# maciejkula/spotlight

Hardware: NVIDIA B200
Metric: interactions/sec (BPR MF, 1Mx100Kx64) (higher is better)
Workload: dtype f32

## Files before the change

### include/spotlight_b200.h

```cpp
#ifndef SPOTLIGHT_B200_H
#define SPOTLIGHT_B200_H

#include <stddef.h>
#include <stdint.h>

#ifdef __cplusplus
extern "C" {
#endif

#define SLB_VERSION 100

#define SLB_OK 0
#define SLB_EINVAL (-1)
#define SLB_ECUDA (-2)
#define SLB_ENOSPC (-3)

#define SLB_LOSS_POINTWISE 0
#define SLB_LOSS_BPR 1
#define SLB_LOSS_HINGE 2
#define SLB_LOSS_ADAPTIVE_HINGE 3

#define SLB_GRAD_DENSE 0
#define SLB_GRAD_COMPACT 1

#define SLB_OPT_NONE 0
#define SLB_OPT_SGD 1
#define SLB_OPT_ADAGRAD 2
#define SLB_OPT_ADAM 3

typedef void* slb_stream_t;

int slb_version(void);
const char* slb_last_error(void);
int slb_sm_count(void);


int slb_mt19937_fill(uint32_t* blocks, int64_t nblocks, slb_stream_t stream);

int slb_mt19937_fill_parallel(uint32_t* blocks, int64_t nblocks, const uint32_t* jump_table,
                              int32_t table_rows, uint32_t* states, slb_stream_t stream);

int64_t slb_mt19937_direct_slots(int64_t nblocks, int32_t j0_log2);
int slb_mt19937_fill_direct(uint32_t* blocks, int64_t nblocks, const uint32_t* jump_table,
                            int32_t table_rows, const uint32_t* direct_table, int32_t direct_rows,
                            int32_t j0_log2, uint32_t* states, int64_t state_slots, slb_stream_t stream);

size_t slb_sample_workspace_bytes(int64_t nwords);

int slb_sample_bounded(const uint32_t* blocks, int64_t nwords, int64_t* cursor,
                       uint32_t rng, int64_t count, int64_t* out,
                       void* workspace, size_t workspace_bytes, slb_stream_t stream);

int slb_sample_bounded_chain(uint32_t* blocks, int64_t nwords, int64_t* cursor,
                             uint32_t rng, int64_t count, int64_t* out,
                             void* workspace, size_t workspace_bytes, slb_stream_t stream);

int slb_host_shuffle_order(uint32_t* key, int32_t* pos, int64_t n, int32_t elem_bytes,
                           void* order_out);

size_t slb_shuffle_workspace_bytes(int64_t n, int64_t nwords);
int slb_shuffle_order(const uint32_t* blocks, int64_t nwords, int64_t* cursor, int64_t first_word,
                      int64_t n, int32_t rounds, int32_t resume, int64_t* order,
                      void* workspace, size_t workspace_bytes, slb_stream_t stream);

int slb_permute_ids(const int64_t* order, int64_t n, const void* users, const void* items,
                    int32_t elem_bytes, int64_t* users_out, int64_t* items_out, slb_stream_t stream);


int slb_embedding_forward(const float* W, int64_t rows, int32_t dim,
                          const int64_t* ids, int64_t n,
                          int32_t hash_count, const uint32_t* seeds ,
                          int64_t padding_idx, float* out, slb_stream_t stream);

int slb_bloom_rows(const int64_t* ids, int64_t n, int32_t hash_count,
                   const uint32_t* seeds , int64_t rows, int64_t padding_idx,
                   int64_t* rows_out, slb_stream_t stream);

size_t slb_embedding_backward_workspace_bytes(int64_t n_terms, int64_t rows);

int slb_embedding_backward(const float* dout, const int64_t* ids, int64_t n,
                           int32_t hash_count, const uint32_t* seeds ,
                           int64_t rows, int32_t dim, int64_t frozen_row,
                           float* dW, void* workspace, size_t workspace_bytes,
                           slb_stream_t stream);

int slb_workspace_init(void* workspace, size_t workspace_bytes, slb_stream_t stream);

int slb_mf_scores(const float* Wu, const float* Wi, const float* bu, const float* bi,
                  int32_t dim, const int64_t* users, const int64_t* items, int64_t n,
                  int32_t user_broadcast, float* scores, slb_stream_t stream);

int slb_mf_scores_backward(const float* gscores, const int64_t* users, const int64_t* items,
                           int64_t n, int32_t user_broadcast, const float* Wu, const float* Wi,
                           int64_t num_users, int64_t num_items, int32_t dim,
                           float* dWu, float* dWi, float* dbu, float* dbi,
                           void* workspace, size_t workspace_bytes, slb_stream_t stream);

int slb_rank_pairs(const float* scores, int64_t n_rows, int64_t n_items, const int64_t* pair_row,
                   const int64_t* pair_item, int64_t n_pairs, float* ranks, slb_stream_t stream);

typedef struct slb_mf_step_args {
    int64_t batch;
    const int64_t* users;
    const int64_t* items;
    const int64_t* negs;
    int32_t loss;
    int32_t n_neg;
    int64_t num_users, num_items;
    int32_t dim;
    float* Wu; float* Wi;
    float* bu; float* bi;
    float* loss_out;
    float* pos_out;
    float* neg_out;
    int32_t grad_mode;
    float* dWu; float* dWi; float* dbu; float* dbi;
    int64_t* urows; float* gWu; float* gbu;
    int64_t* irows; float* gWi; float* gbi;
    int32_t* compact_counts;
    int32_t opt;
    float lr;
    float weight_decay;
    float eps;
    float* state_Wu; float* state_Wi; float* state_bu; float* state_bi;
    int64_t norm_batch;
    int32_t opt_users_only;
    void* workspace; size_t workspace_bytes;
    void* fused_workspace; size_t fused_workspace_bytes;
    slb_stream_t plan_stream;
    float beta1, beta2;
    float one_minus_beta1, one_minus_beta2;
    float* state2_Wu; float* state2_Wi; float* state2_bu; float* state2_bi;
    int32_t* last_u; int32_t* last_i;
    const float* adam_sched;
    int64_t adam_step;
} slb_mf_step_args;

size_t slb_mf_step_workspace_bytes(int64_t batch, int32_t n_neg, int32_t loss,
                                   int64_t num_users, int64_t num_items);
size_t slb_mf_fused_workspace_bytes(int64_t batch, int64_t num_users, int64_t num_items, int32_t dim);
int64_t slb_mf_compact_rows(int64_t batch, int32_t n_neg, int32_t loss, int32_t which );

int slb_mf_train_step(const slb_mf_step_args* args, slb_stream_t stream);

int slb_mf_train_step_phases(const slb_mf_step_args* args, int32_t phases, slb_stream_t stream);

typedef struct slb_mf_bloom_args {
    slb_mf_step_args base;
    int64_t user_rows, item_rows;
    int32_t user_hashes, item_hashes;
    uint32_t user_seeds[24], item_seeds[24];
    int64_t user_padding_idx, item_padding_idx;
    int64_t* pair_ids_u; float* pair_g_u;
    int64_t* pair_ids_i; float* pair_g_i;
} slb_mf_bloom_args;

size_t slb_mf_bloom_workspace_bytes(const slb_mf_bloom_args* args);

size_t slb_bias_sparse_workspace_bytes(int64_t n);
int slb_bias_sparse_apply(const int64_t* ids, const float* g, int64_t n, float* bias, float* state,
                          int32_t opt, float lr, float weight_decay, float eps,
                          void* workspace, size_t workspace_bytes, slb_stream_t stream);
int slb_mf_bloom_train_step(const slb_mf_bloom_args* args, slb_stream_t stream);

int slb_mf_fit_epoch(const slb_mf_step_args* step, const int64_t* users, const int64_t* items,
                     const int64_t* negs, int64_t n, float* losses_out, slb_stream_t stream);

int slb_mf_fit_epoch_events(const slb_mf_step_args* step, const int64_t* users, const int64_t* items,
                            const int64_t* negs, int64_t n, float* losses_out, slb_stream_t stream,
                            const int64_t* wait_steps, void* const* wait_events, int32_t n_waits);

int slb_adam_flush(float* W, float* exp_avg, float* exp_avg_sq, float* bias, float* bias_avg, float* bias_avg_sq,
                   int32_t* last, int64_t rows, int32_t dim, const float* sched, int64_t step,
                   float beta1, float beta2, float one_minus_beta1, float one_minus_beta2, float eps,
                   float weight_decay, slb_stream_t stream);

size_t slb_unique_workspace_bytes(int64_t n, int64_t rows);
int slb_unique_bucket(const int64_t* ids, int64_t n, int64_t rows, int64_t chunk, int32_t nparts,
                      int64_t* uniq , int64_t* inverse ,
                      int64_t* counts_out, void* workspace, size_t workspace_bytes,
                      slb_stream_t stream);

int slb_shard_gather_batch(const int64_t* pos, int64_t m, const int64_t* users, const int64_t* items,
                           const int64_t* negs, int64_t neg_base, int32_t n_neg, int64_t user_lo,
                           int64_t* users_out, int64_t* items_out, int64_t* negs_out, slb_stream_t stream);

int slb_adagrad_dense(float* W, float* state, const float* grad, int64_t n, float lr, float eps,
                      slb_stream_t stream);

size_t slb_loss_workspace_bytes(int64_t n);
int slb_pairwise_loss(int32_t loss, const float* pos, const float* neg, const uint8_t* mask,
                      int64_t n, int32_t n_neg, float* loss_out, float* gpos, float* gneg,
                      void* workspace, size_t workspace_bytes, slb_stream_t stream);

typedef struct slb_seq_step_args {
    int64_t batch;
    int32_t seq_len;
    const int64_t* seqs;
    const int64_t* negs;
    int32_t loss; int32_t n_neg;
    int64_t num_items; int32_t dim;
    float* E; float* bias;
    int32_t n_layers;
    const int32_t* kernel_width; const int32_t* dilation;
    int32_t nonlinearity;
    int32_t residual;
    float* const* conv_w;
    float* const* conv_b;
    float* const* dconv_w;
    float* const* dconv_b;
    float* loss_out; float* pos_out; float* neg_out;
    float* dE; float* dbias;
    const int32_t* norm_count;
    void* workspace; size_t workspace_bytes;
    int32_t opt; float lr; float weight_decay; float eps;
    float* state_E; float* state_bias;
} slb_seq_step_args;

size_t slb_seq_step_workspace_bytes(const slb_seq_step_args* args);
int slb_seq_train_step(const slb_seq_step_args* args, slb_stream_t stream);

int slb_seq_representation(const slb_seq_step_args* args, float* rep_out, slb_stream_t stream);

#ifdef __cplusplus
}
#endif
#endif
```

### spotlight_b200/_lib.py

```python

import ctypes
import os

_HERE = os.path.dirname(os.path.abspath(__file__))
LIB_PATH = os.environ.get('SLB_LIBRARY') or os.path.join(_HERE, 'libspotlight_b200.so')

c_i32, c_i64, c_f32 = ctypes.c_int32, ctypes.c_int64, ctypes.c_float
c_vp, c_sz = ctypes.c_void_p, ctypes.c_size_t

LOSS_KIND = {'pointwise': 0, 'bpr': 1, 'hinge': 2, 'adaptive_hinge': 3}
GRAD_DENSE, GRAD_COMPACT = 0, 1
OPT_NONE, OPT_SGD, OPT_ADAGRAD, OPT_ADAM = 0, 1, 2, 3

EXPORTS = (
    'slb_version', 'slb_last_error', 'slb_sm_count', 'slb_workspace_init',
    'slb_mt19937_fill', 'slb_mt19937_fill_parallel', 'slb_mt19937_direct_slots',
    'slb_mt19937_fill_direct', 'slb_host_shuffle_order',
    'slb_sample_workspace_bytes', 'slb_sample_bounded', 'slb_sample_bounded_chain',
    'slb_shuffle_workspace_bytes', 'slb_shuffle_order', 'slb_permute_ids',
    'slb_embedding_forward', 'slb_bloom_rows',
    'slb_embedding_backward_workspace_bytes', 'slb_embedding_backward',
    'slb_mf_scores', 'slb_mf_scores_backward', 'slb_rank_pairs', 'slb_mf_step_workspace_bytes', 'slb_mf_fused_workspace_bytes', 'slb_mf_compact_rows',
    'slb_mf_train_step', 'slb_mf_train_step_phases', 'slb_mf_fit_epoch', 'slb_mf_fit_epoch_events', 'slb_adam_flush',
    'slb_mf_bloom_workspace_bytes', 'slb_mf_bloom_train_step',
    'slb_bias_sparse_workspace_bytes', 'slb_bias_sparse_apply',
    'slb_unique_workspace_bytes', 'slb_unique_bucket', 'slb_shard_gather_batch', 'slb_adagrad_dense',
    'slb_loss_workspace_bytes', 'slb_pairwise_loss',
    'slb_seq_step_workspace_bytes', 'slb_seq_train_step', 'slb_seq_representation',
)


class MfStepArgs(ctypes.Structure):
    _fields_ = [
        ('batch', c_i64), ('users', c_vp), ('items', c_vp), ('negs', c_vp),
        ('loss', c_i32), ('n_neg', c_i32),
        ('num_users', c_i64), ('num_items', c_i64), ('dim', c_i32),
        ('Wu', c_vp), ('Wi', c_vp), ('bu', c_vp), ('bi', c_vp),
        ('loss_out', c_vp), ('pos_out', c_vp), ('neg_out', c_vp),
        ('grad_mode', c_i32),
        ('dWu', c_vp), ('dWi', c_vp), ('dbu', c_vp), ('dbi', c_vp),
        ('urows', c_vp), ('gWu', c_vp), ('gbu', c_vp),
        ('irows', c_vp), ('gWi', c_vp), ('gbi', c_vp),
        ('compact_counts', c_vp),
        ('opt', c_i32), ('lr', c_f32), ('weight_decay', c_f32), ('eps', c_f32),
        ('state_Wu', c_vp), ('state_Wi', c_vp), ('state_bu', c_vp), ('state_bi', c_vp),
        ('norm_batch', c_i64), ('opt_users_only', c_i32),
        ('workspace', c_vp), ('workspace_bytes', c_sz),
        ('fused_workspace', c_vp), ('fused_workspace_bytes', c_sz), ('plan_stream', c_vp),
        ('beta1', c_f32), ('beta2', c_f32), ('one_minus_beta1', c_f32), ('one_minus_beta2', c_f32),
        ('state2_Wu', c_vp), ('state2_Wi', c_vp), ('state2_bu', c_vp), ('state2_bi', c_vp),
        ('last_u', c_vp), ('last_i', c_vp), ('adam_sched', c_vp), ('adam_step', c_i64),
    ]


class MfBloomArgs(ctypes.Structure):
    _fields_ = [
        ('base', MfStepArgs),
        ('user_rows', c_i64), ('item_rows', c_i64),
        ('user_hashes', c_i32), ('item_hashes', c_i32),
        ('user_seeds', ctypes.c_uint32 * 24), ('item_seeds', ctypes.c_uint32 * 24),
        ('user_padding_idx', c_i64), ('item_padding_idx', c_i64),
        ('pair_ids_u', c_vp), ('pair_g_u', c_vp), ('pair_ids_i', c_vp), ('pair_g_i', c_vp),
    ]


class SeqStepArgs(ctypes.Structure):
    _fields_ = [
        ('batch', c_i64), ('seq_len', c_i32), ('seqs', c_vp), ('negs', c_vp),
        ('loss', c_i32), ('n_neg', c_i32),
        ('num_items', c_i64), ('dim', c_i32),
        ('E', c_vp), ('bias', c_vp),
        ('n_layers', c_i32), ('kernel_width', c_vp), ('dilation', c_vp),
        ('nonlinearity', c_i32), ('residual', c_i32),
        ('conv_w', c_vp), ('conv_b', c_vp), ('dconv_w', c_vp), ('dconv_b', c_vp),
        ('loss_out', c_vp), ('pos_out', c_vp), ('neg_out', c_vp),
        ('dE', c_vp), ('dbias', c_vp),
        ('norm_count', c_vp),
        ('workspace', c_vp), ('workspace_bytes', c_sz),
        ('opt', c_i32), ('lr', c_f32), ('weight_decay', c_f32), ('eps', c_f32),
        ('state_E', c_vp), ('state_bias', c_vp),
    ]


_lib = None


class LibraryError(RuntimeError):
    pass


def _declare(lib):
    P = ctypes.POINTER
    lib.slb_version.restype = c_i32
    lib.slb_last_error.restype = ctypes.c_char_p
    lib.slb_sm_count.restype = c_i32
    lib.slb_workspace_init.argtypes = [c_vp, c_sz, c_vp]
    lib.slb_mt19937_fill.argtypes = [c_vp, c_i64, c_vp]
    lib.slb_mt19937_fill_parallel.argtypes = [c_vp, c_i64, c_vp, c_i32, c_vp, c_vp]
    lib.slb_mt19937_direct_slots.argtypes = [c_i64, c_i32]
    lib.slb_mt19937_direct_slots.restype = c_i64
    lib.slb_mt19937_fill_direct.argtypes = [c_vp, c_i64, c_vp, c_i32, c_vp, c_i32, c_i32, c_vp, c_i64, c_vp]
    lib.slb_sample_bounded_chain.argtypes = [c_vp, c_i64, c_vp, ctypes.c_uint32, c_i64, c_vp, c_vp, c_sz, c_vp]
    lib.slb_host_shuffle_order.argtypes = [c_vp, c_vp, c_i64, c_i32, c_vp]
    lib.slb_shuffle_workspace_bytes.argtypes = [c_i64, c_i64]
    lib.slb_shuffle_workspace_bytes.restype = c_sz
    lib.slb_shuffle_order.argtypes = [c_vp, c_i64, c_vp, c_i64, c_i64, c_i32, c_i32, c_vp, c_vp, c_sz, c_vp]
    lib.slb_permute_ids.argtypes = [c_vp, c_i64, c_vp, c_vp, c_i32, c_vp, c_vp, c_vp]
    lib.slb_sample_workspace_bytes.argtypes = [c_i64]
    lib.slb_sample_workspace_bytes.restype = c_sz
    lib.slb_sample_bounded.argtypes = [c_vp, c_i64, c_vp, ctypes.c_uint32, c_i64, c_vp, c_vp, c_sz, c_vp]
    lib.slb_embedding_forward.argtypes = [c_vp, c_i64, c_i32, c_vp, c_i64, c_i32, c_vp, c_i64, c_vp, c_vp]
    lib.slb_bloom_rows.argtypes = [c_vp, c_i64, c_i32, c_vp, c_i64, c_i64, c_vp, c_vp]
    lib.slb_embedding_backward_workspace_bytes.argtypes = [c_i64, c_i64]
    lib.slb_embedding_backward_workspace_bytes.restype = c_sz
    lib.slb_embedding_backward.argtypes = [c_vp, c_vp, c_i64, c_i32, c_vp, c_i64, c_i32, c_i64,
                                           c_vp, c_vp, c_sz, c_vp]
    lib.slb_mf_scores.argtypes = [c_vp, c_vp, c_vp, c_vp, c_i32, c_vp, c_vp, c_i64, c_i32, c_vp, c_vp]
    lib.slb_mf_scores_backward.argtypes = [c_vp, c_vp, c_vp, c_i64, c_i32, c_vp, c_vp, c_i64, c_i64, c_i32,
                                           c_vp, c_vp, c_vp, c_vp, c_vp, c_sz, c_vp]
    lib.slb_rank_pairs.argtypes = [c_vp, c_i64, c_i64, c_vp, c_vp, c_i64, c_vp, c_vp]
    lib.slb_mf_step_workspace_bytes.argtypes = [c_i64, c_i32, c_i32, c_i64, c_i64]
    lib.slb_mf_step_workspace_bytes.restype = c_sz
    lib.slb_mf_fused_workspace_bytes.argtypes = [c_i64, c_i64, c_i64, c_i32]
    lib.slb_mf_fused_workspace_bytes.restype = c_sz
    lib.slb_mf_compact_rows.argtypes = [c_i64, c_i32, c_i32, c_i32]
    lib.slb_mf_compact_rows.restype = c_i64
    lib.slb_mf_train_step.argtypes = [P(MfStepArgs), c_vp]
    lib.slb_mf_train_step_phases.argtypes = [P(MfStepArgs), c_i32, c_vp]
    lib.slb_mf_bloom_workspace_bytes.argtypes = [P(MfBloomArgs)]
    lib.slb_mf_bloom_workspace_bytes.restype = c_sz
    lib.slb_mf_bloom_train_step.argtypes = [P(MfBloomArgs), c_vp]
    lib.slb_bias_sparse_workspace_bytes.argtypes = [c_i64]
    lib.slb_bias_sparse_workspace_bytes.restype = c_sz
    lib.slb_bias_sparse_apply.argtypes = [c_vp, c_vp, c_i64, c_vp, c_vp, c_i32, c_f32, c_f32, c_f32, c_vp, c_sz, c_vp]
    lib.slb_mf_fit_epoch.argtypes = [P(MfStepArgs), c_vp, c_vp, c_vp, c_i64, c_vp, c_vp]
    lib.slb_mf_fit_epoch_events.argtypes = [P(MfStepArgs), c_vp, c_vp, c_vp, c_i64, c_vp, c_vp, c_vp, c_vp, c_i32]
    lib.slb_adam_flush.argtypes = [c_vp, c_vp, c_vp, c_vp, c_vp, c_vp, c_vp, c_i64, c_i32, c_vp, c_i64,
                                   c_f32, c_f32, c_f32, c_f32, c_f32, c_f32, c_vp]
    lib.slb_unique_workspace_bytes.argtypes = [c_i64, c_i64]
    lib.slb_unique_workspace_bytes.restype = c_sz
    lib.slb_unique_bucket.argtypes = [c_vp, c_i64, c_i64, c_i64, c_i32, c_vp, c_vp, c_vp, c_vp, c_sz, c_vp]
    lib.slb_shard_gather_batch.argtypes = [c_vp, c_i64, c_vp, c_vp, c_vp, c_i64, c_i32, c_i64, c_vp, c_vp, c_vp, c_vp]
    lib.slb_adagrad_dense.argtypes = [c_vp, c_vp, c_vp, c_i64, c_f32, c_f32, c_vp]
    lib.slb_loss_workspace_bytes.argtypes = [c_i64]
    lib.slb_loss_workspace_bytes.restype = c_sz
    lib.slb_pairwise_loss.argtypes = [c_i32, c_vp, c_vp, c_vp, c_i64, c_i32, c_vp, c_vp, c_vp,
                                      c_vp, c_sz, c_vp]
    lib.slb_seq_step_workspace_bytes.argtypes = [P(SeqStepArgs)]
    lib.slb_seq_step_workspace_bytes.restype = c_sz
    lib.slb_seq_train_step.argtypes = [P(SeqStepArgs), c_vp]
    lib.slb_seq_representation.argtypes = [P(SeqStepArgs), c_vp, c_vp]
    for name in EXPORTS:
        fn = getattr(lib, name)
        if fn.restype is ctypes.c_int:
            fn.restype = c_i32


def load():
    global _lib
    if _lib is None:
        if not os.path.exists(LIB_PATH):
            raise LibraryError(
                'spotlight_b200: %s not found. Build it with '
                '`python -c "import __graft_entry__ as g; g.build()"` (needs nvcc, sm_100a). '
                'There is no CPU fallback.' % LIB_PATH)
        lib = ctypes.CDLL(LIB_PATH)
        missing = [n for n in EXPORTS if not hasattr(lib, n)]
        if missing:
            raise LibraryError('spotlight_b200: library lacks symbols %s' % missing)
        _declare(lib)
        if lib.slb_version() != 100:
            raise LibraryError('spotlight_b200: ABI version mismatch')
        _lib = lib
    return _lib


def check(rc, what=''):
    if rc != 0:
        msg = load().slb_last_error().decode('utf-8', 'replace')
        if rc == -1:
            raise ValueError('%s: %s' % (what or 'spotlight_b200', msg))
        raise LibraryError('%s failed (%d): %s' % (what or 'spotlight_b200', rc, msg))
```

### spotlight_b200/csrc/common.cuh

```cuda
#pragma once

#include <cuda_runtime.h>
#include <stdint.h>
#include <stdio.h>

#include "../../include/spotlight_b200.h"

void slb_set_error(const char* fmt, ...);
int slb_sms();

#define SLB_REQUIRE(cond, ...)                 \
    do {                                       \
        if (!(cond)) {                         \
            slb_set_error(__VA_ARGS__);        \
            return SLB_EINVAL;                 \
        }                                      \
    } while (0)

#define SLB_LAUNCH_CHECK(name)                                                   \
    do {                                                                         \
        cudaError_t e__ = cudaGetLastError();                                    \
        if (e__ != cudaSuccess) {                                                \
            slb_set_error("%s: launch failed: %s", name, cudaGetErrorString(e__)); \
            return SLB_ECUDA;                                                    \
        }                                                                        \
    } while (0)

static inline size_t slb_align_up(size_t x, size_t a) { return (x + a - 1) / a * a; }

struct WsCarver {
    char* base;
    size_t off;
    explicit WsCarver(void* p) : base(static_cast<char*>(p)), off(0) {}
    template <typename T>
    T* take(size_t count) {
        off = slb_align_up(off, 256);
        T* p = base ? reinterpret_cast<T*>(base + off) : nullptr;
        off += count * sizeof(T);
        return p;
    }
    size_t bytes() const { return slb_align_up(off, 256); }
};

#ifdef __CUDACC__

__device__ __forceinline__ float4 ldg4(const float* p) {
    return __ldg(reinterpret_cast<const float4*>(p));
}
__device__ __forceinline__ float4 ld4(const float* p) {
    return *reinterpret_cast<const float4*>(p);
}
__device__ __forceinline__ void st4(float* p, float4 v) { *reinterpret_cast<float4*>(p) = v; }

__device__ __forceinline__ float dot4(float4 a, float4 b) {
    return a.x * b.x + a.y * b.y + a.z * b.z + a.w * b.w;
}
__device__ __forceinline__ void fma4(float4& acc, float g, float4 v) {
    acc.x = fmaf(g, v.x, acc.x);
    acc.y = fmaf(g, v.y, acc.y);
    acc.z = fmaf(g, v.z, acc.z);
    acc.w = fmaf(g, v.w, acc.w);
}

template <int LPR>
__device__ __forceinline__ float group_sum(float v, unsigned mask) {
#pragma unroll
    for (int o = LPR / 2; o > 0; o >>= 1) v += __shfl_xor_sync(mask, v, o);
    return v;
}

__device__ __forceinline__ unsigned group_mask(int lpr) {
    const int lane = threadIdx.x & 31;
    const unsigned m = lpr == 32 ? 0xffffffffu : ((1u << lpr) - 1u);
    return m << (lane & ~(lpr - 1));
}

__device__ __forceinline__ float sigmoidf_(float x) { return 1.0f / (1.0f + expf(-x)); }

template <int THREADS>
__device__ __forceinline__ float block_sum(float v, float* smem ) {
#pragma unroll
    for (int o = 16; o > 0; o >>= 1) v += __shfl_down_sync(0xffffffffu, v, o);
    const int w = threadIdx.x >> 5, l = threadIdx.x & 31;
    if (l == 0) smem[w] = v;
    __syncthreads();
    if (w == 0) {
        v = l < THREADS / 32 ? smem[l] : 0.f;
#pragma unroll
        for (int o = 16; o > 0; o >>= 1) v += __shfl_down_sync(0xffffffffu, v, o);
    }
    return v;
}

__device__ __forceinline__ uint32_t murmur3_32(uint32_t k, uint32_t seed) {
    k *= 0xcc9e2d51u;
    k = (k << 15) | (k >> 17);
    k *= 0x1b873593u;
    uint32_t h = seed ^ k;
    h = (h << 13) | (h >> 19);
    h = h * 5u + 0xe6546b64u;
    h ^= 4u;
    h ^= h >> 16;
    h *= 0x85ebca6bu;
    h ^= h >> 13;
    h *= 0xc2b2ae35u;
    h ^= h >> 16;
    return h;
}

__device__ __forceinline__ int64_t bloom_row(int64_t id, uint32_t seed, int64_t rows,
                                             int64_t padding_idx) {
    if (id == padding_idx) return 0;
    const int64_t h = static_cast<int32_t>(murmur3_32(static_cast<uint32_t>(id), seed));
    int64_t m = h % rows;
    if (m < 0) m += rows;
    return m;
}

__device__ __forceinline__ float adagrad_delta(float lr, float g, float s, float eps) {
    const float root = s > 0.f ? s * rsqrtf(s) : 0.f;
    return __fdividef(lr * g, root + eps);
}

struct OptV2 { int32_t opt; float lr, wd, eps; };

__device__ __forceinline__ void row_update(const OptV2& o, float4& w, float4& s, const float4& g0) {
    float gv[4] = {g0.x + o.wd * w.x, g0.y + o.wd * w.y, g0.z + o.wd * w.z, g0.w + o.wd * w.w};
    float wv[4] = {w.x, w.y, w.z, w.w};
    if (o.opt == SLB_OPT_SGD) {
#pragma unroll
        for (int q = 0; q < 4; ++q) wv[q] -= o.lr * gv[q];
    } else {
        float sv[4] = {s.x, s.y, s.z, s.w};
#pragma unroll
        for (int q = 0; q < 4; ++q) {
            sv[q] += gv[q] * gv[q];
            wv[q] -= adagrad_delta(o.lr, gv[q], sv[q], o.eps);
        }
        s = make_float4(sv[0], sv[1], sv[2], sv[3]);
    }
    w = make_float4(wv[0], wv[1], wv[2], wv[3]);
}

__device__ __forceinline__ void bias_update(const OptV2& o, float* bw, float* bs, float g) {
    const float gb = g + o.wd * *bw;
    if (o.opt == SLB_OPT_SGD) {
        *bw -= o.lr * gb;
    } else {
        const float sv = *bs + gb * gb;
        *bs = sv;
        *bw -= adagrad_delta(o.lr, gb, sv, o.eps);
    }
}

#endif
```

### spotlight_b200/csrc/mf.cu

```cuda
#include <stdlib.h>

#include "segindex.cuh"

namespace {

constexpr int MF_THREADS = 256;

struct MfDev {
    int64_t B;
    int64_t NB;
    int64_t T;
    const int64_t* users; const int64_t* items; const int64_t* negs;
    int32_t loss; int32_t n_neg;
    int64_t U, I; int32_t D;
    float* Wu; float* Wi; float* bu; float* bi;
    float* loss_out; float* pos_out; float* neg_out;
    int32_t* t_a; int32_t* t_b; float* t_g;
    float* partial; int32_t* done;
    int32_t* err;
    SegIndex seg;
    int32_t grad_mode;
    float* dWu; float* dWi; float* dbu; float* dbi;
    int64_t* urows; float* gWu; float* gbu;
    int64_t* irows; float* gWi; float* gbi;
    int32_t* compact_counts;
    int32_t opt; float lr, wd, eps;
    float* sWu; float* sWi; float* sbu; float* sbi;
    int32_t no_bias;
    int64_t frozen_a, frozen_b;
};

template <int LPR>
__device__ __forceinline__ float row_dot(const float* __restrict__ a, const float* __restrict__ b,
                                         int D, int gl, unsigned gmask) {
    float acc = 0.f;
    for (int c = gl * 4; c < D; c += LPR * 4) acc += dot4(ldg4(a + c), ldg4(b + c));
    return group_sum<LPR>(acc, gmask);
}

__device__ __forceinline__ void pair_loss(int loss, float p, float n, float& per, float& gp, float& gn) {
    if (loss == SLB_LOSS_BPR) {
        const float s = sigmoidf_(p - n);
        per = 1.0f - s;
        gp = -s * (1.0f - s);
        gn = -gp;
    } else if (loss == SLB_LOSS_POINTWISE) {
        const float sp = sigmoidf_(p), sn = sigmoidf_(n);
        per = (1.0f - sp) + sn;
        gp = -sp * (1.0f - sp);
        gn = sn * (1.0f - sn);
    } else {
        const float z = n - p + 1.0f;
        per = fmaxf(z, 0.0f);
        const float act = z >= 0.0f ? 1.0f : 0.0f;
        gp = -act;
        gn = act;
    }
}

template <int LPR>
__global__ void __launch_bounds__(MF_THREADS) mf_fwd_kernel(MfDev a) {
    __shared__ float sh_red[MF_THREADS / 32];
    const int gl = threadIdx.x & (LPR - 1);
    const unsigned gmask = group_mask(LPR);
    constexpr int GROUPS = MF_THREADS / LPR;
    const int64_t gid = static_cast<int64_t>(blockIdx.x) * GROUPS + threadIdx.x / LPR;
    const int64_t gstride = static_cast<int64_t>(gridDim.x) * GROUPS;
    const float invB = 1.0f / static_cast<float>(a.NB);
    const int D = a.D;
    float lsum = 0.f;
    if (blockIdx.x == 0 && threadIdx.x == 0) a.seg.totals[3] = 0;

    const int64_t iters = (a.B + gstride - 1) / gstride;
    for (int64_t it = 0; it < iters; ++it) {
        const int64_t b = gid + it * gstride;
        const bool valid = b < a.B;
        const int64_t bb = valid ? b : 0;
        const int64_t u = a.users[bb], i = a.items[bb];
        bool bad = u < 0 || u >= a.U || i < 0 || i >= a.I;
        const int64_t uc = bad ? 0 : u, ic = bad ? 0 : i;
        const float* urow = a.Wu + uc * D;
        float p, n;
        int64_t nu, nj;
        if (a.loss != SLB_LOSS_ADAPTIVE_HINGE) {
            int64_t j = a.negs[bb];
            if (j < 0 || j >= a.I) { bad = true; j = 0; }
            const float* qi = a.Wi + ic * D;
            const float* qj = a.Wi + j * D;
            float dp = 0.f, dn = 0.f;
            for (int c = gl * 4; c < D; c += LPR * 4) {
                const float4 u4 = ldg4(urow + c), i4 = ldg4(qi + c), j4 = ldg4(qj + c);
                dp += dot4(u4, i4);
                dn += dot4(u4, j4);
            }
            const float ub = __ldg(a.bu + uc);
            p = group_sum<LPR>(dp, gmask) + ub + __ldg(a.bi + ic);
            n = group_sum<LPR>(dn, gmask) + ub + __ldg(a.bi + j);
            nu = uc; nj = j;
            if (valid && gl == 0 && a.neg_out) a.neg_out[bb] = n;
        } else {
            p = row_dot<LPR>(urow, a.Wi + ic * D, D, gl, gmask) + __ldg(a.bu + uc) + __ldg(a.bi + ic);
            n = -INFINITY; nu = 0; nj = 0;
            for (int k = 0; k < a.n_neg; ++k) {
                const int64_t f = static_cast<int64_t>(k) * a.B + bb;
                int64_t u2 = a.users[f / a.n_neg], j = a.negs[f];
                if (u2 < 0 || u2 >= a.U || j < 0 || j >= a.I) { bad = true; u2 = 0; j = 0; }
                const float nk = row_dot<LPR>(a.Wu + u2 * D, a.Wi + j * D, D, gl, gmask) +
                                 __ldg(a.bu + u2) + __ldg(a.bi + j);
                if (valid && gl == 0 && a.neg_out) a.neg_out[f] = nk;
                if (nk > n || k == 0) { n = nk; nu = u2; nj = j; }
            }
        }
        if (valid && gl == 0) {
            if (bad) atomicExch(a.err, 1);
            float per, gp, gn;
            pair_loss(a.loss, p, n, per, gp, gn);
            lsum += per;
            gp *= invB; gn *= invB;
            if (bad) { gp = 0.f; gn = 0.f; }
            if (a.pos_out) a.pos_out[bb] = p;
            const int32_t t = static_cast<int32_t>(2 * bb);
            a.t_a[t] = static_cast<int32_t>(uc); a.t_b[t] = static_cast<int32_t>(ic); a.t_g[t] = gp;
            a.t_a[t + 1] = static_cast<int32_t>(nu); a.t_b[t + 1] = static_cast<int32_t>(nj); a.t_g[t + 1] = gn;
            if (gp != 0.f) { atomicAdd(a.seg.cnt + uc, 1); atomicAdd(a.seg.cnt + a.U + ic, 1); }
            if (gn != 0.f) { atomicAdd(a.seg.cnt + nu, 1); atomicAdd(a.seg.cnt + a.U + nj, 1); }
        }
    }

    const float bsum = block_sum<MF_THREADS>(lsum, sh_red);
    __shared__ bool is_last;
    if (threadIdx.x == 0) {
        a.partial[blockIdx.x] = bsum;
        __threadfence();
        is_last = atomicAdd(a.done, 1) == static_cast<int>(gridDim.x) - 1;
    }
    __syncthreads();
    if (is_last && threadIdx.x < 32) {
        __threadfence();
        float v = 0.f;
        for (int k = threadIdx.x; k < static_cast<int>(gridDim.x); k += 32)
            v += *reinterpret_cast<volatile float*>(a.partial + k);
#pragma unroll
        for (int o = 16; o > 0; o >>= 1) v += __shfl_down_sync(0xffffffffu, v, o);
        if (threadIdx.x == 0) { *a.loss_out = v * invB; *a.done = 0; }
    }
}

constexpr int MF_TILE_THREADS = 128;

template <int LPR, int LOSS, int TI, bool EX>
__global__ void __launch_bounds__(MF_TILE_THREADS) mf_fwd_tile_kernel(MfDev a) {
    __shared__ float sh_red[MF_TILE_THREADS / 32];
    __shared__ bool is_last;
    constexpr int GPW = 32 / LPR;
    constexpr int ITERS = TI / GPW > 0 ? TI / GPW : 1;
    const int lane = threadIdx.x & 31;
    const int gl = lane & (LPR - 1);
    const int grp = lane / LPR;
    const int D = EX ? LPR * 4 : a.D;
    const float invB = 1.0f / static_cast<float>(a.NB);
    const int64_t ntiles = (a.B + TI - 1) / TI;
    const int64_t wstride = static_cast<int64_t>(gridDim.x) * (MF_TILE_THREADS / 32);
    float lsum = 0.f;
    if (blockIdx.x == 0 && threadIdx.x == 0) a.seg.totals[3] = 0;

    for (int64_t tile = static_cast<int64_t>(blockIdx.x) * (MF_TILE_THREADS / 32) + (threadIdx.x >> 5);
         tile < ntiles; tile += wstride) {
        const int64_t b = tile * TI + lane;
        const bool valid = lane < TI && b < a.B;
        int64_t u64 = 0, i64 = 0, j64 = 0;
        if (valid) { u64 = a.users[b]; i64 = a.items[b]; j64 = a.negs[b]; }
        const bool bad = u64 < 0 || u64 >= a.U || i64 < 0 || i64 >= a.I || j64 < 0 || j64 >= a.I;
        if (bad) { u64 = 0; i64 = 0; j64 = 0; }
        const int u = static_cast<int>(u64), i = static_cast<int>(i64), j = static_cast<int>(j64);
        const float ub = __ldg(a.bu + u), ib = __ldg(a.bi + i), jb = __ldg(a.bi + j);
        float dpm = 0.f, dnm = 0.f;
#pragma unroll 4
        for (int s = 0; s < ITERS; ++s) {
            const int src = (s * GPW + grp) % TI;
            const int uu = __shfl_sync(0xffffffffu, u, src);
            const int ii = __shfl_sync(0xffffffffu, i, src);
            const int jj = __shfl_sync(0xffffffffu, j, src);
            const float* ur = a.Wu + static_cast<int64_t>(uu) * D;
            const float* qi = a.Wi + static_cast<int64_t>(ii) * D;
            const float* qj = a.Wi + static_cast<int64_t>(jj) * D;
            float dp = 0.f, dn = 0.f;
            for (int c = gl * 4; c < D; c += LPR * 4) {
                const float4 u4 = ldg4(ur + c), i4 = ldg4(qi + c), j4 = ldg4(qj + c);
                dp += dot4(u4, i4);
                dn += dot4(u4, j4);
            }
            dp = group_sum<LPR>(dp, 0xffffffffu);
            dn = group_sum<LPR>(dn, 0xffffffffu);
            const float tp = __shfl_sync(0xffffffffu, dp, (lane % GPW) * LPR);
            const float tn = __shfl_sync(0xffffffffu, dn, (lane % GPW) * LPR);
            if (lane / GPW == s) { dpm = tp; dnm = tn; }
        }
        if (valid) {
            const float p = dpm + ub + ib, n = dnm + ub + jb;
            float per, gp, gn;
            pair_loss(LOSS, p, n, per, gp, gn);
            lsum += per;
            gp *= invB; gn *= invB;
            if (bad) { atomicExch(a.err, 1); gp = 0.f; gn = 0.f; }
            if (a.pos_out) a.pos_out[b] = p;
            if (a.neg_out) a.neg_out[b] = n;
            *reinterpret_cast<int2*>(a.t_a + 2 * b) = make_int2(u, u);
            *reinterpret_cast<int2*>(a.t_b + 2 * b) = make_int2(i, j);
            *reinterpret_cast<float2*>(a.t_g + 2 * b) = make_float2(gp, gn);
            const int nu = (gp != 0.f) + (gn != 0.f);
            if (nu) atomicAdd(a.seg.cnt + u, nu);
            if (gp != 0.f) atomicAdd(a.seg.cnt + a.U + i, 1);
            if (gn != 0.f) atomicAdd(a.seg.cnt + a.U + j, 1);
        }
    }
    const float bsum = block_sum<MF_TILE_THREADS>(lsum, sh_red);
    if (threadIdx.x == 0) {
        a.partial[blockIdx.x] = bsum;
        __threadfence();
        is_last = atomicAdd(a.done, 1) == static_cast<int>(gridDim.x) - 1;
    }
    __syncthreads();
    if (is_last && threadIdx.x < 32) {
        __threadfence();
        float v = 0.f;
        for (int k = threadIdx.x; k < static_cast<int>(gridDim.x); k += 32)
            v += *reinterpret_cast<volatile float*>(a.partial + k);
#pragma unroll
        for (int o = 16; o > 0; o >>= 1) v += __shfl_down_sync(0xffffffffu, v, o);
        if (threadIdx.x == 0) { *a.loss_out = v * invB; *a.done = 0; }
    }
}

__device__ __forceinline__ void cswap(int& x, int& y) {
    const int lo = x < y ? x : y, hi = x < y ? y : x;
    x = lo; y = hi;
}

#ifndef GEN_CHUNK
#define GEN_CHUNK 8
#endif
__device__ __forceinline__ void pf_row_l2(const float* row, int D) {
    const char* p = reinterpret_cast<const char*>(row);
    for (int o = 0; o < D * 4; o += 128) asm volatile("prefetch.global.L2 [%0];" ::"l"(p + o));
}

#ifndef BWD_BULK
#define BWD_BULK 0
#endif
#if BWD_BULK
__device__ __forceinline__ uint32_t bulk_smem_u32(const void* p) {
    return static_cast<uint32_t>(__cvta_generic_to_shared(p));
}
__device__ __forceinline__ void bulk_bar_init(uint64_t* bar) {
    asm volatile("mbarrier.init.shared::cta.b64 [%0], 1;" ::"r"(bulk_smem_u32(bar)));
    asm volatile("fence.mbarrier_init.release.cluster;" ::: "memory");
}
__device__ __forceinline__ void bulk_bar_expect(uint64_t* bar, uint32_t bytes) {
    asm volatile("mbarrier.arrive.expect_tx.shared::cta.b64 _, [%0], %1;" ::"r"(bulk_smem_u32(bar)), "r"(bytes)
                 : "memory");
}
__device__ __forceinline__ void bulk_g2s(void* dst, const void* src, uint32_t bytes, uint64_t* bar) {
    asm volatile("cp.async.bulk.shared::cluster.global.mbarrier::complete_tx::bytes [%0], [%1], %2, [%3];"
                 ::"r"(bulk_smem_u32(dst)), "l"(src), "r"(bytes), "r"(bulk_smem_u32(bar)) : "memory");
}
__device__ __forceinline__ void bulk_bar_wait(uint64_t* bar, uint32_t parity) {
    for (int spin = 0; spin < (1 << 26); ++spin) {
        uint32_t ok;
        asm volatile("{\n\t.reg .pred p;\n\t"
                     "mbarrier.try_wait.parity.shared::cta.b64 p, [%1], %2;\n\t"
                     "selp.u32 %0, 1, 0, p;\n\t}"
                     : "=r"(ok) : "r"(bulk_smem_u32(bar)), "r"(parity) : "memory");
        if (ok) return;
    }
    __trap();
}
#endif

#ifndef BWD_MINB
#define BWD_MINB 6
#endif
#ifndef BWD_MINB1
#define BWD_MINB1 BWD_MINB
#endif
#ifndef BWD_FAST
#define BWD_FAST 4
#endif
template <int LPR, int MODE, int TI, bool EX>
__global__ void __launch_bounds__(MF_TILE_THREADS, MODE == 1 ? BWD_MINB1 : BWD_MINB) mf_bwd_tile_kernel(MfDev a) {
    constexpr int GPW = 32 / LPR;
    constexpr int ITERS = TI / GPW > 0 ? TI / GPW : 1;
    constexpr int WARPS = MF_TILE_THREADS / 32;
    constexpr int CAP = seg_sort_cap(LPR);
    __shared__ int32_t sh_all[WARPS * GPW * 4 * CAP];
    const int lane = threadIdx.x & 31;
    const int gl = lane & (LPR - 1);
    const int grp = lane / LPR;
    const unsigned gmask = group_mask(LPR);
    int32_t* sh = sh_all + ((threadIdx.x >> 5) * GPW + grp) * 4 * CAP;
    const int D = EX ? LPR * 4 : a.D;
#if defined(BWD_OPT_CT)
    a.opt = BWD_OPT_CT;
    a.wd = 0.f;
#endif
#if BWD_BULK
    constexpr bool BULK = MODE == 2 && EX && TI == 32;
    constexpr int RB = LPR * 16;
    extern __shared__ __align__(128) unsigned char bulk_rows[];
    __shared__ uint64_t bulk_bar[WARPS];
    unsigned char* my_rows = bulk_rows + (threadIdx.x >> 5) * (TI * 2 * RB);
    uint64_t* my_bar = &bulk_bar[threadIdx.x >> 5];
    uint32_t bulk_phase = 0;
    if (BULK) {
        if (lane == 0) bulk_bar_init(my_bar);
        __syncwarp();
    }
#endif
    const int nseg = a.seg.totals[0];
    const int nsegA = a.seg.totals[2];
    if (MODE != 2 && blockIdx.x == 0 && threadIdx.x == 0 && a.compact_counts) {
        a.compact_counts[0] = nsegA;
        a.compact_counts[1] = nseg - nsegA;
    }
    const int seg_lo = MODE == 1 ? nsegA : 0;
    const int seg_hi = MODE == 2 ? nsegA : nseg;
    const int32_t* __restrict__ t_a = a.t_a;
    const int32_t* __restrict__ t_b = a.t_b;
    const float* __restrict__ t_g = a.t_g;
    const int32_t* __restrict__ members = a.seg.members;
    const int ntiles = (seg_hi - seg_lo + TI - 1) / TI;
    const int wstride = gridDim.x * WARPS;

    for (int tile = blockIdx.x * WARPS + (threadIdx.x >> 5); tile < ntiles; tile += wstride) {
        const int sidx = seg_lo + tile * TI + lane;
        const bool valid = lane < TI && sidx < seg_hi;
        int start = 0, len = 0, row = 0;
        int p[BWD_FAST] = {};
        float g[BWD_FAST] = {};
#if BWD_BULK
        if (valid) {
            start = a.seg.seg_start[sidx];
            len = a.seg.seg_start[sidx + 1] - start;
            row = a.seg.seg_row[sidx];
        }
        if (BULK) {
            const bool stage = valid && len <= CAP && row != a.frozen_a;
            const unsigned who = __ballot_sync(0xffffffffu, stage);
            const uint32_t per = a.opt == SLB_OPT_ADAGRAD ? 2u * RB : 1u * RB;
            if (lane == 0) bulk_bar_expect(my_bar, __popc(who) * per);
            __syncwarp();
            if (stage) {
                bulk_g2s(my_rows + lane * 2 * RB, a.Wu + static_cast<int64_t>(row) * D, RB, my_bar);
                if (a.opt == SLB_OPT_ADAGRAD)
                    bulk_g2s(my_rows + lane * 2 * RB + RB, a.sWu + static_cast<int64_t>(row) * D, RB, my_bar);
            }
        }
#endif
        if (valid) {
            const bool isA = sidx < nsegA;
#if !BWD_BULK
            start = a.seg.seg_start[sidx];
            len = a.seg.seg_start[sidx + 1] - start;
            row = a.seg.seg_row[sidx];
#endif
            if (len <= BWD_FAST) {
                int m[BWD_FAST];
#pragma unroll
                for (int k = 0; k < BWD_FAST; ++k) m[k] = k < len ? members[start + k] : 0x7fffffff;
                cswap(m[0], m[1]);
                if (BWD_FAST == 4) { cswap(m[BWD_FAST - 2], m[BWD_FAST - 1]); cswap(m[0], m[BWD_FAST - 2]); cswap(m[1], m[BWD_FAST - 1]); cswap(m[1], m[BWD_FAST - 2]); }
                const int32_t* pidx = isA ? t_b : t_a;
#pragma unroll
                for (int k = 0; k < BWD_FAST; ++k)
                    if (k < len) { g[k] = t_g[m[k]]; p[k] = pidx[m[k]]; }
            }
        }
#if BWD_BULK
        if (BULK) { bulk_bar_wait(my_bar, bulk_phase); bulk_phase ^= 1u; }
#endif
        for (int it = 0; it < ITERS; ++it) {
            const int src = it * GPW + grp;
            const int s_len = __shfl_sync(0xffffffffu, len, src & 31);
            const int s_row = __shfl_sync(0xffffffffu, row, src & 31);
            const int s_start = __shfl_sync(0xffffffffu, start, src & 31);
            int sp[BWD_FAST];
            float sg[BWD_FAST];
#pragma unroll
            for (int k = 0; k < BWD_FAST; ++k) {
                sp[k] = __shfl_sync(0xffffffffu, p[k], src & 31);
                sg[k] = __shfl_sync(0xffffffffu, g[k], src & 31);
            }
            const int s = seg_lo + tile * TI + src;
            if (src >= TI || s >= seg_hi) continue;
            const bool sA = s < nsegA;
            const float* ptab = sA ? a.Wi : a.Wu;
            const int64_t orow = sA ? s_row : s_row - a.U;
            if (orow == (sA ? a.frozen_a : a.frozen_b)) {
                if (MODE != 2 && gl == 0 && a.grad_mode == SLB_GRAD_COMPACT) {
                    if (sA) a.urows[s] = -1; else a.irows[s - nsegA] = -1;
                }
                continue;
            }
            if (s_len > CAP) continue;
            float* out = nullptr;
            if (MODE != 2) {
                if (a.grad_mode == SLB_GRAD_DENSE) out = (sA ? a.dWu : a.dWi) + orow * D;
                else out = sA ? a.gWu + static_cast<int64_t>(s) * D : a.gWi + static_cast<int64_t>(s - nsegA) * D;
            }
            float* wrow = MODE == 2 ? a.Wu + orow * D : nullptr;
            float* srow = (MODE == 2 && a.opt == SLB_OPT_ADAGRAD) ? a.sWu + orow * D : nullptr;
            float bacc = 0.f;

            int n_gen = 0;
            if (s_len > BWD_FAST && s_len <= CAP) {
                int32_t* in = sh;
                int32_t* srt = sh + CAP;
                float* pg = reinterpret_cast<float*>(sh + 2 * CAP);
                int32_t* pp = sh + 3 * CAP;
                for (int i = gl; i < s_len; i += LPR) in[i] = members[s_start + i];
                __syncwarp(gmask);
                for (int i = gl; i < s_len; i += LPR) {
                    const int32_t m = in[i];
                    int r = 0;
                    for (int j = 0; j < s_len; ++j) r += in[j] < m;
                    srt[r] = m;
                }
                __syncwarp(gmask);
                const int32_t* pidx = sA ? t_b : t_a;
                for (int i = gl; i < s_len; i += LPR) {
                    const int32_t pr = pidx[srt[i]];
                    pg[i] = t_g[srt[i]];
                    pp[i] = pr;
                    if (!sA) pf_row_l2(ptab + static_cast<int64_t>(pr) * D, D);
                }
                __syncwarp(gmask);
                n_gen = s_len;
            }

            for (int c = gl * 4; c < D; c += LPR * 4) {
                float4 acc = make_float4(0.f, 0.f, 0.f, 0.f);
                float b2 = 0.f;
                float4 w4 = make_float4(0.f, 0.f, 0.f, 0.f), s4 = w4;
#if BWD_BULK
                if (BULK) {
                    const unsigned char* staged = my_rows + src * 2 * RB + c * 4;
                    w4 = *reinterpret_cast<const float4*>(staged);
                    if (srow) s4 = *reinterpret_cast<const float4*>(staged + RB);
                } else
#endif
                if (MODE == 2) { w4 = ld4(wrow + c); if (srow) s4 = ld4(srow + c); }
                if (s_len <= BWD_FAST) {
                    float4 v[BWD_FAST];
#pragma unroll
                    for (int k = 0; k < BWD_FAST; ++k)
                        if (k < s_len) v[k] = ldg4(ptab + static_cast<int64_t>(sp[k]) * D + c);
#pragma unroll
                    for (int k = 0; k < BWD_FAST; ++k)
                        if (k < s_len) { fma4(acc, sg[k], v[k]); b2 += sg[k]; }
                } else if (n_gen) {
                    const float* pg = reinterpret_cast<const float*>(sh + 2 * CAP);
                    const int32_t* pp = sh + 3 * CAP;
                    int i = 0;
                    for (; i + GEN_CHUNK <= n_gen; i += GEN_CHUNK) {
                        float4 v[GEN_CHUNK];
#pragma unroll
                        for (int k = 0; k < GEN_CHUNK; ++k) v[k] = ldg4(ptab + static_cast<int64_t>(pp[i + k]) * D + c);
#pragma unroll
                        for (int k = 0; k < GEN_CHUNK; ++k) { fma4(acc, pg[i + k], v[k]); b2 += pg[i + k]; }
                    }
                    for (; i < n_gen; ++i) {
                        fma4(acc, pg[i], ldg4(ptab + static_cast<int64_t>(pp[i]) * D + c));
                        b2 += pg[i];
                    }
                }
                bacc = b2;
                if (MODE == 2) {
                    float gv[4] = {acc.x + a.wd * w4.x, acc.y + a.wd * w4.y, acc.z + a.wd * w4.z, acc.w + a.wd * w4.w};
                    float wv[4] = {w4.x, w4.y, w4.z, w4.w};
                    if (a.opt == SLB_OPT_SGD) {
#pragma unroll
                        for (int q = 0; q < 4; ++q) wv[q] -= a.lr * gv[q];
                    } else {
                        float sv[4] = {s4.x, s4.y, s4.z, s4.w};
#pragma unroll
                        for (int q = 0; q < 4; ++q) {
                            sv[q] += gv[q] * gv[q];
                            wv[q] -= adagrad_delta(a.lr, gv[q], sv[q], a.eps);
                        }
                        st4(srow + c, make_float4(sv[0], sv[1], sv[2], sv[3]));
                    }
                    st4(wrow + c, make_float4(wv[0], wv[1], wv[2], wv[3]));
                } else {
                    st4(out + c, acc);
                }
            }
            if (n_gen) __syncwarp(gmask);
            if (gl == 0 && MODE != 2 && a.grad_mode == SLB_GRAD_COMPACT) {
                if (sA) a.urows[s] = orow; else a.irows[s - nsegA] = orow;
            }
            if (gl == 0 && !a.no_bias) {
                if (MODE == 2) {
                    float* bw = a.bu + orow;
                    const float gb = bacc + a.wd * *bw;
                    if (a.opt == SLB_OPT_SGD) {
                        *bw -= a.lr * gb;
                    } else {
                        float* bs = a.sbu + orow;
                        const float sv = *bs + gb * gb;
                        *bs = sv;
                        *bw -= adagrad_delta(a.lr, gb, sv, a.eps);
                    }
                } else if (a.grad_mode == SLB_GRAD_DENSE) {
                    if (sA) a.dbu[orow] = bacc; else a.dbi[orow] = bacc;
                } else {
                    if (sA) a.gbu[s] = bacc; else a.gbi[s - nsegA] = bacc;
                }
            }
        }
#if BWD_BULK
        if (BULK) __syncwarp();
#endif
    }
}

template <int LPR, int MODE>
__global__ void __launch_bounds__(256) mf_bwd_long_kernel(MfDev a) {
    constexpr int GROUPS = 256 / LPR;
    extern __shared__ float sh_part[];
    const int gl = threadIdx.x & (LPR - 1);
    const int gq = threadIdx.x / LPR;
    const int D = a.D;
    const int PS = D + 4;
    const int nlong = a.seg.totals[3];
    const int nsegA = a.seg.totals[2];
    const int32_t* __restrict__ members = a.seg.members;
    for (int li = blockIdx.x; li < nlong; li += gridDim.x) {
        const int s = a.seg.long_list[li];
        const bool sA = s < nsegA;
        if ((MODE == 1 && sA) || (MODE == 2 && !sA)) continue;
        const int start = a.seg.seg_start[s];
        const int len = a.seg.seg_start[s + 1] - start;
        const int row = a.seg.seg_row[s];
        const int64_t orow = sA ? row : row - a.U;
        if (orow == (sA ? a.frozen_a : a.frozen_b)) {
            if (MODE != 2 && threadIdx.x == 0 && a.grad_mode == SLB_GRAD_COMPACT) {
                if (sA) a.urows[s] = -1; else a.irows[s - nsegA] = -1;
            }
            continue;
        }
        const float* ptab = sA ? a.Wi : a.Wu;
        const int32_t* pidx = sA ? a.t_b : a.t_a;
        const int chunk = (len + GROUPS - 1) / GROUPS;
        const int lo = min(gq * chunk, len), hi = min(lo + chunk, len);
        for (int c0 = 0; c0 < D; c0 += LPR * 4) {
            const int c = c0 + gl * 4;
            float4 acc = make_float4(0.f, 0.f, 0.f, 0.f);
            float b2 = 0.f;
            int i = lo;
            for (; i + 4 <= hi; i += 4) {
                int t[4]; float g[4]; float4 v[4];
#pragma unroll
                for (int k = 0; k < 4; ++k) t[k] = members[start + i + k];
#pragma unroll
                for (int k = 0; k < 4; ++k) {
                    g[k] = a.t_g[t[k]];
                    v[k] = c < D ? ldg4(ptab + static_cast<int64_t>(pidx[t[k]]) * D + c) : make_float4(0, 0, 0, 0);
                }
#pragma unroll
                for (int k = 0; k < 4; ++k) { fma4(acc, g[k], v[k]); b2 += g[k]; }
            }
            for (; i < hi; ++i) {
                const int t = members[start + i];
                const float g = a.t_g[t];
                if (c < D) fma4(acc, g, ldg4(ptab + static_cast<int64_t>(pidx[t]) * D + c));
                b2 += g;
            }
            if (c < D) st4(sh_part + gq * PS + c, acc);
            if (gl == 0 && c0 == 0) sh_part[gq * PS + D] = b2;
        }
        __syncthreads();
        if (gq == 0) {
            float bacc = 0.f;
            for (int q = 0; q < GROUPS; ++q) bacc += sh_part[q * PS + D];
            for (int c = gl * 4; c < D; c += LPR * 4) {
                float4 acc = make_float4(0.f, 0.f, 0.f, 0.f);
                for (int q = 0; q < GROUPS; ++q) {
                    const float4 p = ld4(sh_part + q * PS + c);
                    acc.x += p.x; acc.y += p.y; acc.z += p.z; acc.w += p.w;
                }
                if (MODE == 2) {
                    float* wrow = a.Wu + orow * D;
                    float4 w4 = ld4(wrow + c);
                    float gv[4] = {acc.x + a.wd * w4.x, acc.y + a.wd * w4.y, acc.z + a.wd * w4.z, acc.w + a.wd * w4.w};
                    float wv[4] = {w4.x, w4.y, w4.z, w4.w};
                    if (a.opt == SLB_OPT_SGD) {
#pragma unroll
                        for (int q = 0; q < 4; ++q) wv[q] -= a.lr * gv[q];
                    } else {
                        float* srow = a.sWu + orow * D;
                        float4 s4 = ld4(srow + c);
                        float sv[4] = {s4.x, s4.y, s4.z, s4.w};
#pragma unroll
                        for (int q = 0; q < 4; ++q) { sv[q] += gv[q] * gv[q]; wv[q] -= adagrad_delta(a.lr, gv[q], sv[q], a.eps); }
                        st4(srow + c, make_float4(sv[0], sv[1], sv[2], sv[3]));
                    }
                    st4(wrow + c, make_float4(wv[0], wv[1], wv[2], wv[3]));
                } else {
                    float* out;
                    if (a.grad_mode == SLB_GRAD_DENSE) out = (sA ? a.dWu : a.dWi) + orow * D;
                    else out = sA ? a.gWu + static_cast<int64_t>(s) * D : a.gWi + static_cast<int64_t>(s - nsegA) * D;
                    st4(out + c, acc);
                }
            }
            if (gl == 0 && MODE != 2 && a.grad_mode == SLB_GRAD_COMPACT) {
                if (sA) a.urows[s] = orow; else a.irows[s - nsegA] = orow;
            }
            if (gl == 0 && !a.no_bias) {
                if (MODE == 2) {
                    float* bw = a.bu + orow;
                    const float gb = bacc + a.wd * *bw;
                    if (a.opt == SLB_OPT_SGD) {
                        *bw -= a.lr * gb;
                    } else {
                        float* bs = a.sbu + orow;
                        const float sv = *bs + gb * gb;
                        *bs = sv;
                        *bw -= adagrad_delta(a.lr, gb, sv, a.eps);
                    }
                } else if (a.grad_mode == SLB_GRAD_DENSE) {
                    if (sA) a.dbu[orow] = bacc; else a.dbi[orow] = bacc;
                } else {
                    if (sA) a.gbu[s] = bacc; else a.gbi[s - nsegA] = bacc;
                }
            }
        }
        __syncthreads();
    }
}

__global__ void __launch_bounds__(256) mf_fill_kernel(MfDev a) {
    seg_rearm(a.seg);
    const int64_t T = a.T;
    const int64_t nth = static_cast<int64_t>(gridDim.x) * blockDim.x;
    for (int64_t t = static_cast<int64_t>(blockIdx.x) * blockDim.x + threadIdx.x; t < T; t += nth) {
        if (a.t_g[t] != 0.f) {
            seg_place(a.seg, a.t_a[t], static_cast<int32_t>(t));
            seg_place(a.seg, a.U + a.t_b[t], static_cast<int32_t>(t));
        }
    }
}

template <int LPR, int ITEMS_ONLY>
__global__ void __launch_bounds__(MF_THREADS) mf_apply_kernel(MfDev a) {
    constexpr int GROUPS = MF_THREADS / LPR;
    const int gl = threadIdx.x & (LPR - 1);
    const int gib = threadIdx.x / LPR;
    const int D = a.D;
    const int nseg = a.seg.totals[0];
    const int nsegA = a.seg.totals[2];
    for (int64_t s = (ITEMS_ONLY ? nsegA : 0) + static_cast<int64_t>(blockIdx.x) * GROUPS + gib; s < nseg;
         s += static_cast<int64_t>(gridDim.x) * GROUPS) {
        const bool isA = s < nsegA;
        const int64_t k = isA ? s : s - nsegA;
        const int64_t row = isA ? a.urows[k] : a.irows[k];
        if (row < 0) continue;
        float* W = (isA ? a.Wu : a.Wi) + row * D;
        const float* G = (isA ? a.gWu : a.gWi) + k * D;
        float* S = a.opt == SLB_OPT_ADAGRAD ? (isA ? a.sWu : a.sWi) + row * D : nullptr;
        for (int c = gl * 4; c < D; c += LPR * 4) {
            float4 w = ld4(W + c);
            const float4 g0 = ld4(G + c);
            float gv[4] = {g0.x + a.wd * w.x, g0.y + a.wd * w.y, g0.z + a.wd * w.z, g0.w + a.wd * w.w};
            float wv[4] = {w.x, w.y, w.z, w.w};
            if (a.opt == SLB_OPT_SGD) {
#pragma unroll
                for (int q = 0; q < 4; ++q) wv[q] -= a.lr * gv[q];
            } else {
                float4 st = ld4(S + c);
                float sv[4] = {st.x, st.y, st.z, st.w};
#pragma unroll
                for (int q = 0; q < 4; ++q) {
                    sv[q] += gv[q] * gv[q];
                    wv[q] -= adagrad_delta(a.lr, gv[q], sv[q], a.eps);
                }
                st4(S + c, make_float4(sv[0], sv[1], sv[2], sv[3]));
            }
            st4(W + c, make_float4(wv[0], wv[1], wv[2], wv[3]));
        }
        if (gl == 0 && !a.no_bias) {
            float* bw = (isA ? a.bu : a.bi) + row;
            float g = (isA ? a.gbu : a.gbi)[k] + a.wd * *bw;
            if (a.opt == SLB_OPT_SGD) {
                *bw -= a.lr * g;
            } else {
                float* bs = (isA ? a.sbu : a.sbi) + row;
                const float sv = *bs + g * g;
                *bs = sv;
                *bw -= adagrad_delta(a.lr, g, sv, a.eps);
            }
        }
    }
}

constexpr int MF_MAX_GRID = 148 * 16;

#include "mf_v2.cuh"
#include "mf_adam.cuh"

template <int LPR>
__global__ void __launch_bounds__(MF_THREADS)
mf_scores_kernel(const float* __restrict__ Wu, const float* __restrict__ Wi,
                 const float* __restrict__ bu, const float* __restrict__ bi, int D,
                 const int64_t* __restrict__ users, const int64_t* __restrict__ items, int64_t n,
                 int user_broadcast, float* __restrict__ scores) {
    const int gl = threadIdx.x & (LPR - 1);
    const unsigned gmask = group_mask(LPR);
    constexpr int GROUPS = MF_THREADS / LPR;
    const int64_t gid = static_cast<int64_t>(blockIdx.x) * GROUPS + threadIdx.x / LPR;
    const int64_t gstride = static_cast<int64_t>(gridDim.x) * GROUPS;
    const int64_t iters = (n + gstride - 1) / gstride;
    for (int64_t it = 0; it < iters; ++it) {
        const int64_t b = gid + it * gstride;
        const bool valid = b < n;
        const int64_t bb = valid ? b : 0;
        const int64_t u = users[user_broadcast ? 0 : bb], i = items[bb];
        const float p = row_dot<LPR>(Wu + u * D, Wi + i * D, D, gl, gmask) + __ldg(bu + u) + __ldg(bi + i);
        if (valid && gl == 0) scores[bb] = p;
    }
}

__global__ void __launch_bounds__(256)
mf_terms_kernel(MfDev a, const float* __restrict__ gscores, int user_broadcast) {
    const int64_t nth = static_cast<int64_t>(gridDim.x) * blockDim.x;
    if (blockIdx.x == 0 && threadIdx.x == 0) a.seg.totals[3] = 0;
    for (int64_t t = static_cast<int64_t>(blockIdx.x) * blockDim.x + threadIdx.x; t < a.T; t += nth) {
        int64_t u = a.users[user_broadcast ? 0 : t], i = a.items[t];
        float g = gscores[t];
        if (u < 0 || u >= a.U || i < 0 || i >= a.I) { atomicExch(a.err, 1); u = 0; i = 0; g = 0.f; }
        a.t_a[t] = static_cast<int32_t>(u); a.t_b[t] = static_cast<int32_t>(i); a.t_g[t] = g;
        if (g != 0.f) { atomicAdd(a.seg.cnt + u, 1); atomicAdd(a.seg.cnt + a.U + i, 1); }
    }
}

struct BloomSpec {
    int Hu, Hi;
    int64_t pad_u, pad_i;
    uint32_t su[24], si[24];
    int64_t num_users, num_items;
    int64_t* ids_u2; int64_t* ids_i2;
    float* g_u2; float* g_i2;
};

__device__ __forceinline__ int64_t hashed_row(int64_t id, int k, int H, const uint32_t* seeds,
                                              int64_t rows, int64_t pad) {
    return H == 0 ? id : bloom_row(id, seeds[k], rows, pad);
}

template <int LPR>
__device__ __forceinline__ float bloom_dot(const MfDev& a, const BloomSpec& h, int64_t u, int64_t i,
                                           int gl, unsigned gmask) {
    const int D = a.D;
    const int nu = h.Hu ? h.Hu : 1, ni = h.Hi ? h.Hi : 1;
    float acc = 0.f;
    for (int c = gl * 4; c < D; c += LPR * 4) {
        float4 us = make_float4(0, 0, 0, 0), is = make_float4(0, 0, 0, 0);
        for (int k = 0; k < nu; ++k) {
            const float4 v = ldg4(a.Wu + hashed_row(u, k, h.Hu, h.su, a.U, h.pad_u) * D + c);
            us.x += v.x; us.y += v.y; us.z += v.z; us.w += v.w;
        }
        for (int k = 0; k < ni; ++k) {
            const float4 v = ldg4(a.Wi + hashed_row(i, k, h.Hi, h.si, a.I, h.pad_i) * D + c);
            is.x += v.x; is.y += v.y; is.z += v.z; is.w += v.w;
        }
        acc += dot4(us, is);
    }
    return group_sum<LPR>(acc, gmask);
}

template <int LPR>
__global__ void __launch_bounds__(MF_THREADS) mf_fwd_bloom_kernel(MfDev a, const __grid_constant__ BloomSpec h) {
    __shared__ float sh_red[MF_THREADS / 32];
    __shared__ bool is_last;
    const int gl = threadIdx.x & (LPR - 1);
    const unsigned gmask = group_mask(LPR);
    constexpr int GROUPS = MF_THREADS / LPR;
    const int64_t gid = static_cast<int64_t>(blockIdx.x) * GROUPS + threadIdx.x / LPR;
    const int64_t gstride = static_cast<int64_t>(gridDim.x) * GROUPS;
    const float invB = 1.0f / static_cast<float>(a.NB);
    const int nu = h.Hu ? h.Hu : 1, ni = h.Hi ? h.Hi : 1;
    const int pairs = nu * ni;
    float lsum = 0.f;
    if (blockIdx.x == 0 && threadIdx.x == 0) a.seg.totals[3] = 0;
    const int64_t iters = (a.B + gstride - 1) / gstride;
    for (int64_t it = 0; it < iters; ++it) {
        const int64_t b = gid + it * gstride;
        const bool valid = b < a.B;
        const int64_t bb = valid ? b : 0;
        int64_t u = a.users[bb], i = a.items[bb];
        bool bad = u < 0 || u >= h.num_users || i < 0 || i >= h.num_items;
        if (bad) { u = 0; i = 0; }
        const float p = bloom_dot<LPR>(a, h, u, i, gl, gmask) + __ldg(a.bu + u) + __ldg(a.bi + i);
        float n = -INFINITY;
        int64_t nuid = u, njid = 0;
        for (int k = 0; k < a.n_neg; ++k) {
            const int64_t f = static_cast<int64_t>(k) * a.B + bb;
            int64_t u2 = a.loss == SLB_LOSS_ADAPTIVE_HINGE ? a.users[f / a.n_neg] : u;
            int64_t j = a.negs[f];
            if (u2 < 0 || u2 >= h.num_users || j < 0 || j >= h.num_items) { bad = true; u2 = 0; j = 0; }
            const float nk = bloom_dot<LPR>(a, h, u2, j, gl, gmask) + __ldg(a.bu + u2) + __ldg(a.bi + j);
            if (valid && gl == 0 && a.neg_out) a.neg_out[f] = nk;
            if (k == 0 || nk > n) { n = nk; nuid = u2; njid = j; }
        }
        if (valid && gl == 0) {
            if (bad) atomicExch(a.err, 1);
            float per, gp, gn;
            pair_loss(a.loss, p, n, per, gp, gn);
            lsum += per;
            gp *= invB; gn *= invB;
            if (bad) { gp = 0.f; gn = 0.f; }
            if (a.pos_out) a.pos_out[bb] = p;
            if (nuid == u) {
                h.ids_u2[bb] = u; h.g_u2[bb] = gp + gn;
                h.ids_u2[a.B + bb] = u; h.g_u2[a.B + bb] = 0.f;
            } else {
                h.ids_u2[bb] = u; h.g_u2[bb] = gp;
                h.ids_u2[a.B + bb] = nuid; h.g_u2[a.B + bb] = gn;
            }
            h.ids_i2[bb] = i; h.g_i2[bb] = gp;
            h.ids_i2[a.B + bb] = njid; h.g_i2[a.B + bb] = gn;
            const int64_t t0 = bb * 2 * pairs;
            for (int side = 0; side < 2; ++side) {
                const float g = side ? gn : gp;
                const int64_t uu = side ? nuid : u, ii = side ? njid : i;
                for (int ku = 0; ku < nu; ++ku) {
                    const int32_t ra = static_cast<int32_t>(hashed_row(uu, ku, h.Hu, h.su, a.U, h.pad_u));
                    for (int ki = 0; ki < ni; ++ki) {
                        const int32_t rb = static_cast<int32_t>(hashed_row(ii, ki, h.Hi, h.si, a.I, h.pad_i));
                        const int64_t t = t0 + side * pairs + ku * ni + ki;
                        a.t_a[t] = ra; a.t_b[t] = rb; a.t_g[t] = g;
                        if (g != 0.f) { atomicAdd(a.seg.cnt + ra, 1); atomicAdd(a.seg.cnt + a.U + rb, 1); }
                    }
                }
            }
        }
    }
    const float bsum = block_sum<MF_THREADS>(lsum, sh_red);
    if (threadIdx.x == 0) {
        a.partial[blockIdx.x] = bsum;
        __threadfence();
        is_last = atomicAdd(a.done, 1) == static_cast<int>(gridDim.x) - 1;
    }
    __syncthreads();
    if (is_last && threadIdx.x < 32) {
        __threadfence();
        float v = 0.f;
        for (int k = threadIdx.x; k < static_cast<int>(gridDim.x); k += 32)
            v += *reinterpret_cast<volatile float*>(a.partial + k);
#pragma unroll
        for (int o = 16; o > 0; o >>= 1) v += __shfl_down_sync(0xffffffffu, v, o);
        if (threadIdx.x == 0) { *a.loss_out = v * invB; *a.done = 0; }
    }
}

struct MfLayout {
    int32_t* t_a; int32_t* t_b; float* t_g; float* partial; int32_t* done; int32_t* err;
    SegIndex seg;
    size_t bytes;
};

MfLayout mf_layout(void* base, int64_t B, int64_t U, int64_t I) {
    WsCarver ws(base);
    MfLayout l;
    l.done = ws.take<int32_t>(8);
    l.err = l.done + 4;
    l.seg = seg_index_carve(ws, U + I, 4 * B);
    l.t_a = ws.take<int32_t>(2 * B);
    l.t_b = ws.take<int32_t>(2 * B);
    l.t_g = ws.take<float>(2 * B);
    l.partial = ws.take<float>(MF_MAX_GRID);
    l.bytes = ws.bytes();
    return l;
}

int lpr_for_dim(int D) {
    int l = D / 4;
    if (l >= 32) return 32;
    int p = 1;
    while (p < l) p <<= 1;
    return p;
}

#define DISPATCH_LPR(lpr, KERNEL, grid, block, stream, ...)                                   \
    switch (lpr) {                                                                           \
        case 1: KERNEL<1><<<grid, block, 0, stream>>>(__VA_ARGS__); break;                   \
        case 2: KERNEL<2><<<grid, block, 0, stream>>>(__VA_ARGS__); break;                   \
        case 4: KERNEL<4><<<grid, block, 0, stream>>>(__VA_ARGS__); break;                   \
        case 8: KERNEL<8><<<grid, block, 0, stream>>>(__VA_ARGS__); break;                   \
        case 16: KERNEL<16><<<grid, block, 0, stream>>>(__VA_ARGS__); break;                 \
        default: KERNEL<32><<<grid, block, 0, stream>>>(__VA_ARGS__); break;                 \
    }

#define DISPATCH_LPR2(lpr, KERNEL, P2, grid, block, stream, ...)                               \
    switch (lpr) {                                                                           \
        case 1: KERNEL<1, P2><<<grid, block, 0, stream>>>(__VA_ARGS__); break;               \
        case 2: KERNEL<2, P2><<<grid, block, 0, stream>>>(__VA_ARGS__); break;               \
        case 4: KERNEL<4, P2><<<grid, block, 0, stream>>>(__VA_ARGS__); break;               \
        case 8: KERNEL<8, P2><<<grid, block, 0, stream>>>(__VA_ARGS__); break;               \
        case 16: KERNEL<16, P2><<<grid, block, 0, stream>>>(__VA_ARGS__); break;             \
        default: KERNEL<32, P2><<<grid, block, 0, stream>>>(__VA_ARGS__); break;             \
    }

#define DISPATCH_LPR3_EX(L, KERNEL, P2, P3, grid, block, stream, a)                              \
    if ((a).D == (L) * 4) KERNEL<L, P2, P3, true><<<grid, block, 0, stream>>>(a);                \
    else KERNEL<L, P2, P3, false><<<grid, block, 0, stream>>>(a);
#define DISPATCH_LPR3(lpr, KERNEL, P2, P3, grid, block, stream, a)                               \
    switch (lpr) {                                                                               \
        case 1: KERNEL<1, P2, P3, false><<<grid, block, 0, stream>>>(a); break;                  \
        case 2: KERNEL<2, P2, P3, false><<<grid, block, 0, stream>>>(a); break;                  \
        case 4: KERNEL<4, P2, P3, false><<<grid, block, 0, stream>>>(a); break;                  \
        case 8: DISPATCH_LPR3_EX(8, KERNEL, P2, P3, grid, block, stream, a) break;               \
        case 16: DISPATCH_LPR3_EX(16, KERNEL, P2, P3, grid, block, stream, a) break;             \
        default: DISPATCH_LPR3_EX(32, KERNEL, P2, P3, grid, block, stream, a) break;             \
    }

template <int MODE>
void launch_long(int lpr, cudaStream_t st, const MfDev& a) {
    const size_t smem = static_cast<size_t>(256 / lpr) * (a.D + 4) * sizeof(float);
    switch (lpr) {
        case 1: mf_bwd_long_kernel<1, MODE><<<SEG_LONG_CTAS * 4, 256, smem, st>>>(a); break;
        case 2: mf_bwd_long_kernel<2, MODE><<<SEG_LONG_CTAS * 4, 256, smem, st>>>(a); break;
        case 4: mf_bwd_long_kernel<4, MODE><<<SEG_LONG_CTAS * 4, 256, smem, st>>>(a); break;
        case 8: mf_bwd_long_kernel<8, MODE><<<SEG_LONG_CTAS * 4, 256, smem, st>>>(a); break;
        case 16: mf_bwd_long_kernel<16, MODE><<<SEG_LONG_CTAS * 4, 256, smem, st>>>(a); break;
        default: mf_bwd_long_kernel<32, MODE><<<SEG_LONG_CTAS * 4, 256, smem, st>>>(a); break;
    }
}

bool v2_eligible(const slb_mf_step_args* x);

int validate(const slb_mf_step_args* x) {
    SLB_REQUIRE(x != nullptr, "mf_train_step: null args");
    SLB_REQUIRE(x->batch > 0, "mf_train_step: batch must be > 0");
    SLB_REQUIRE(x->dim >= 4 && x->dim % 4 == 0, "mf_train_step: dim must be a positive multiple of 4 (got %d)", x->dim);
    SLB_REQUIRE(x->loss >= 0 && x->loss <= 3, "mf_train_step: bad loss kind %d", x->loss);
    SLB_REQUIRE(x->n_neg >= 1, "mf_train_step: n_neg must be >= 1");
    SLB_REQUIRE(x->loss == SLB_LOSS_ADAPTIVE_HINGE || x->n_neg == 1, "mf_train_step: n_neg > 1 only for adaptive hinge");
    SLB_REQUIRE(x->num_users > 0 && x->num_items > 0, "mf_train_step: empty tables");
    SLB_REQUIRE(x->num_users + x->num_items < (1ll << 31) - SEG_SCAN_TILE, "mf_train_step: num_users + num_items must be < 2^31");
    SLB_REQUIRE(x->batch * 4 < (1ll << 31), "mf_train_step: batch too large");
    SLB_REQUIRE(x->users && x->items && x->negs && x->Wu && x->Wi && x->bu && x->bi && x->loss_out,
                "mf_train_step: null pointer");
    SLB_REQUIRE(x->workspace != nullptr, "mf_train_step: null workspace");
    if (x->grad_mode == SLB_GRAD_DENSE) {
        if (x->opt != SLB_OPT_NONE) {
            SLB_REQUIRE(x->opt_users_only, "mf_train_step: a fully fused optimizer needs compact grads");
            SLB_REQUIRE(x->dWi && x->dbi, "mf_train_step: users-only optimizer needs dWi/dbi for the item side");
        } else {
            SLB_REQUIRE(x->dWu && x->dWi && x->dbu && x->dbi, "mf_train_step: dense mode needs dWu/dWi/dbu/dbi");
        }
    } else {
        SLB_REQUIRE(x->grad_mode == SLB_GRAD_COMPACT, "mf_train_step: bad grad_mode");
        SLB_REQUIRE(v2_eligible(x) || (x->urows && x->gWu && x->gbu && x->irows && x->gWi && x->gbi && x->compact_counts),
                    "mf_train_step: compact mode needs urows/gWu/gbu/irows/gWi/gbi/compact_counts");
    }
    SLB_REQUIRE(x->opt >= SLB_OPT_NONE && x->opt <= SLB_OPT_ADAM, "mf_train_step: bad optimizer");
    if (x->opt == SLB_OPT_ADAM) {
        SLB_REQUIRE(x->grad_mode == SLB_GRAD_COMPACT && !x->opt_users_only, "mf_train_step: fused Adam needs compact grads");
        SLB_REQUIRE(x->state_Wu && x->state_Wi && x->state_bu && x->state_bi && x->state2_Wu && x->state2_Wi &&
                    x->state2_bu && x->state2_bi && x->last_u && x->last_i && x->adam_sched && x->adam_step >= 1,
                    "mf_train_step: fused Adam needs exp_avg / exp_avg_sq / last / schedule and adam_step >= 1");
    }
    if (x->opt == SLB_OPT_ADAGRAD) {
        SLB_REQUIRE(x->state_Wu && x->state_bu, "mf_train_step: adagrad needs state");
        SLB_REQUIRE(x->opt_users_only || (x->state_Wi && x->state_bi), "mf_train_step: adagrad needs item state");
    }
#if defined(BWD_OPT_CT)
    SLB_REQUIRE(x->opt == SLB_OPT_NONE || (x->opt == BWD_OPT_CT && x->weight_decay == 0.f),
                "mf_train_step: this build was compiled with -DBWD_OPT_CT=%d and weight_decay 0", BWD_OPT_CT);
#endif
    const size_t need = slb_mf_step_workspace_bytes(x->batch, x->n_neg, x->loss, x->num_users, x->num_items);
    if (x->workspace_bytes < need) {
        slb_set_error("mf_train_step: workspace too small (%zu < %zu)", x->workspace_bytes, need);
        return SLB_ENOSPC;
    }
    return SLB_OK;
}

int launch_step(const slb_mf_step_args* x, const int64_t* users, const int64_t* items,
                const int64_t* negs, int64_t B, float* loss_out, cudaStream_t st,
                int phases = 0x1f, int64_t step_idx = 0) {
    MfLayout l = mf_layout(x->workspace, x->batch, x->num_users, x->num_items);
    MfDev a;
    a.B = B; a.NB = x->norm_batch > 0 ? x->norm_batch : B; a.T = 2 * B; a.users = users; a.items = items; a.negs = negs;
    a.loss = x->loss; a.n_neg = x->n_neg;
    a.U = x->num_users; a.I = x->num_items; a.D = x->dim;
    a.Wu = x->Wu; a.Wi = x->Wi; a.bu = x->bu; a.bi = x->bi;
    a.loss_out = loss_out; a.pos_out = x->pos_out; a.neg_out = x->neg_out;
    a.t_a = l.t_a; a.t_b = l.t_b; a.t_g = l.t_g; a.partial = l.partial; a.done = l.done; a.err = l.err;
    a.seg = l.seg;
    a.seg.long_cap = seg_sort_cap(lpr_for_dim(x->dim));
    a.no_bias = 0; a.frozen_a = -1; a.frozen_b = -1;
    a.grad_mode = x->grad_mode;
    a.dWu = x->dWu; a.dWi = x->dWi; a.dbu = x->dbu; a.dbi = x->dbi;
    a.urows = x->urows; a.gWu = x->gWu; a.gbu = x->gbu;
    a.irows = x->irows; a.gWi = x->gWi; a.gbi = x->gbi;
    a.compact_counts = x->compact_counts;
    a.opt = x->opt; a.lr = x->lr; a.wd = x->weight_decay; a.eps = x->eps;
    a.sWu = x->state_Wu; a.sWi = x->state_Wi; a.sbu = x->state_bu; a.sbi = x->state_bi;

    const int lpr = lpr_for_dim(x->dim);
    const int groups = MF_THREADS / lpr;
    const int sms = slb_sms();
    int64_t want = (B + groups - 1) / groups;
    int grid = static_cast<int>(want < static_cast<int64_t>(sms) * 8 ? want : static_cast<int64_t>(sms) * 8);
    if (grid < 1) grid = 1;
    if (grid > MF_MAX_GRID) grid = MF_MAX_GRID;
    if ((phases & 1) && x->opt == SLB_OPT_ADAM) {
        AdamDev o = {x->beta1, x->beta2, x->one_minus_beta1, x->one_minus_beta2, x->eps, x->weight_decay, x->adam_sched,
                     static_cast<int32_t>(x->adam_step + step_idx)};
        const int64_t refs = (2 + x->n_neg) * B;
        const int64_t pw = (refs + groups - 1) / groups;
        const int pgrid = static_cast<int>(pw < static_cast<int64_t>(sms) * 8 ? (pw < 1 ? 1 : pw) : static_cast<int64_t>(sms) * 8);
        DISPATCH_LPR(lpr, mf_adam_prepass_kernel, pgrid, MF_THREADS, st, a, o, x->state2_Wu, x->state2_Wi,
                     x->state2_bu, x->state2_bi, x->last_u, x->last_i);
        SLB_LAUNCH_CHECK("mf_adam_prepass_kernel");
    }
    if (phases & 1) {
        if (x->loss == SLB_LOSS_ADAPTIVE_HINGE) {
            DISPATCH_LPR(lpr, mf_fwd_kernel, grid, MF_THREADS, st, a);
        } else {
            const bool small = B < static_cast<int64_t>(sms) * 36 * 32;
            const int ti = small ? 8 : 32;
            int64_t tw = ((B + ti - 1) / ti + 3) / 4;
            int tgrid = static_cast<int>(tw < MF_MAX_GRID ? tw : MF_MAX_GRID);
#define FWD_TILE(L)                                                                             \
    if (small) { DISPATCH_LPR3(lpr, mf_fwd_tile_kernel, L, 8, tgrid, MF_TILE_THREADS, st, a); } \
    else { DISPATCH_LPR3(lpr, mf_fwd_tile_kernel, L, 32, tgrid, MF_TILE_THREADS, st, a); }
            switch (x->loss) {
                case SLB_LOSS_POINTWISE: FWD_TILE(SLB_LOSS_POINTWISE); break;
                case SLB_LOSS_BPR: FWD_TILE(SLB_LOSS_BPR); break;
                default: FWD_TILE(SLB_LOSS_HINGE); break;
            }
        }
        SLB_LAUNCH_CHECK("mf_fwd_kernel");
    }
    if (phases & 2) {
        seg_scan_launch(a.seg, a.U, st);
        SLB_LAUNCH_CHECK("seg_scan_kernel");
    }
    int fgrid = static_cast<int>((2 * B + 255) / 256);
    if (fgrid > sms * 8) fgrid = sms * 8;
    if (phases & 4) {
        mf_fill_kernel<<<fgrid, 256, 0, st>>>(a);
        SLB_LAUNCH_CHECK("mf_fill_kernel");
        seg_sort_long_kernel<<<SEG_LONG_CTAS, 256, 0, st>>>(a.seg);
        SLB_LAUNCH_CHECK("seg_sort_long_kernel");
    }
    int64_t bwant = (2 * B + groups - 1) / groups;
    int bgrid = static_cast<int>(bwant < static_cast<int64_t>(sms) * 8 ? bwant : static_cast<int64_t>(sms) * 8);
    const bool bsmall = 2 * B < static_cast<int64_t>(sms) * 24 * 32;
    const int bti = bsmall ? 8 : 32;
    const int64_t tw = ((2 * B + bti - 1) / bti + 3) / 4;
    const int tgrid = static_cast<int>(tw < static_cast<int64_t>(sms) * 16 ? tw : static_cast<int64_t>(sms) * 16);
    const int blpr = lpr;
#define BWD_TILE(MODE)                                                                               \
    if (bsmall) { DISPATCH_LPR3(blpr, mf_bwd_tile_kernel, MODE, 8, tgrid, MF_TILE_THREADS, st, a); } \
    else { DISPATCH_LPR3(blpr, mf_bwd_tile_kernel, MODE, 32, tgrid, MF_TILE_THREADS, st, a); }
    if (x->opt == SLB_OPT_NONE || x->opt == SLB_OPT_ADAM) {
        if (phases & 8) {
            BWD_TILE(0);
            SLB_LAUNCH_CHECK("mf_bwd_tile_kernel");
            launch_long<0>(lpr, st, a);
            SLB_LAUNCH_CHECK("mf_bwd_long_kernel");
        }
        if (x->opt == SLB_OPT_ADAM && (phases & 16)) {
            AdamDev o = {x->beta1, x->beta2, x->one_minus_beta1, x->one_minus_beta2, x->eps, x->weight_decay, x->adam_sched,
                         static_cast<int32_t>(x->adam_step + step_idx)};
            DISPATCH_LPR(lpr, mf_adam_apply_kernel, bgrid, MF_THREADS, st, a, o, x->state2_Wu, x->state2_Wi,
                         x->state2_bu, x->state2_bi, x->last_u, x->last_i);
            SLB_LAUNCH_CHECK("mf_adam_apply_kernel");
        }
    } else {
        if (phases & 8) {
            BWD_TILE(1);
            SLB_LAUNCH_CHECK("mf_bwd_tile_kernel<items>");
            launch_long<1>(lpr, st, a);
            SLB_LAUNCH_CHECK("mf_bwd_long_kernel<items>");
#if BWD_BULK
            if (lpr == 16 && a.D == 64 && !bsmall) {
                auto kern = mf_bwd_tile_kernel<16, 2, 32, true>;
                constexpr int BULK_SMEM = (MF_TILE_THREADS / 32) * 32 * 2 * 256;
                static bool configured = false;
                if (!configured) {
                    cudaFuncSetAttribute(kern, cudaFuncAttributeMaxDynamicSharedMemorySize, BULK_SMEM);
                    configured = true;
                }
                kern<<<tgrid, MF_TILE_THREADS, BULK_SMEM, st>>>(a);
            } else
#endif
            { BWD_TILE(2); }
            SLB_LAUNCH_CHECK("mf_bwd_tile_kernel<users+opt>");
            launch_long<2>(lpr, st, a);
            SLB_LAUNCH_CHECK("mf_bwd_long_kernel<users+opt>");
        }
        if ((phases & 16) && !x->opt_users_only) {
            DISPATCH_LPR2(lpr, mf_apply_kernel, 1, bgrid, MF_THREADS, st, a);
            SLB_LAUNCH_CHECK("mf_apply_kernel<items>");
        }
    }
    return SLB_OK;
}


struct V2Layout {
    PlanDev plan[2];
    StepV2 st;
    size_t bytes;
};

V2Layout v2_layout(void* base, int64_t B, int64_t U, int64_t I, int D) {
    WsCarver ws(base);
    V2Layout l;
    const int64_t R = U + I;
    const int64_t Rpad = (R + SEG_SCAN_TILE - 1) / SEG_SCAN_TILE * SEG_SCAN_TILE;
    l.st.done = ws.take<int32_t>(8);
    int32_t* cnt[2] = {ws.take<int32_t>(Rpad), ws.take<int32_t>(Rpad)};
    for (int k = 0; k < 2; ++k) {
        PlanDev& p = l.plan[k];
        SegIndex& s = p.seg;
        s.R = R;
        s.Rpad = Rpad;
        s.ntiles = s.Rpad / SEG_SCAN_TILE;
        s.Tmax = 3 * B;
        s.cnt = cnt[k];
        s.off = ws.take<int32_t>(s.Rpad);
        s.sid = ws.take<int32_t>(s.Rpad);
        s.status = ws.take<unsigned long long>(s.ntiles);
        s.ticket = ws.take<int32_t>(8);
        s.totals = s.ticket + 4;
        s.seg_row = ws.take<int32_t>(3 * B + 1);
        s.seg_start = ws.take<int32_t>(3 * B + 2);
        s.long_list = ws.take<int32_t>(3 * B / 16 + 2);
        s.members = nullptr; s.long_tmp = nullptr; s.long_bits = nullptr; s.long_words = 0;
        s.long_cap = 0;
        p.mu = ws.take<URec>(B + 1);
        p.mi = ws.take<IRec>(2 * B + 1);
        p.mu_tmp = ws.take<URec>(B + 1);
        p.mi_tmp = ws.take<IRec>(2 * B + 1);
        p.words = (2 * B + 31) / 32;
        p.bits = ws.take<uint32_t>(static_cast<size_t>(SEG_LONG_CTAS) * 2 * p.words);
        p.B = B; p.U = U; p.I = I;
        p.err = nullptr; p.users = nullptr; p.items = nullptr; p.negs = nullptr;
    }
    l.st.t_g = ws.take<float>(2 * B);
    l.st.stash = ws.take<float>(static_cast<size_t>(B) * D);
    l.st.partial = ws.take<float>(MF_MAX_GRID);
    l.st.partial_long = ws.take<float>(SEG_LONG_CTAS * 4);
    l.bytes = ws.bytes();
    return l;
}

bool v2_dim_ok(int D) { return D == 8 || D == 16 || D == 32 || D == 64 || D == 128; }

bool v2_eligible(const slb_mf_step_args* x) {
    if (x->fused_workspace == nullptr || x->loss == SLB_LOSS_ADAPTIVE_HINGE || x->opt == SLB_OPT_NONE ||
        x->opt == SLB_OPT_ADAM ||
        !v2_dim_ok(x->dim) || x->pos_out != nullptr || x->neg_out != nullptr)
        return false;
    if (x->opt_users_only) return x->grad_mode == SLB_GRAD_DENSE && x->dWi != nullptr && x->dbi != nullptr;
    return x->grad_mode == SLB_GRAD_COMPACT;
}

int v2_launch_plan(const slb_mf_step_args* x, PlanDev p, int32_t* err, const int64_t* users, const int64_t* items,
                   const int64_t* negs, int64_t B, cudaStream_t st) {
    p.B = B; p.users = users; p.items = items; p.negs = negs; p.err = err;
    p.seg.long_cap = seg_sort_cap(lpr_for_dim(x->dim));
    const int sms = slb_sms();
    int g = static_cast<int>((B + 255) / 256);
    if (g > sms * 8) g = sms * 8;
    plan_count_kernel<<<g, 256, 0, st>>>(p);
    SLB_LAUNCH_CHECK("plan_count_kernel");
    seg_scan_launch(p.seg, p.U, st);
    SLB_LAUNCH_CHECK("seg_scan_kernel");
    plan_fill_kernel<<<g, 256, 0, st>>>(p);
    SLB_LAUNCH_CHECK("plan_fill_kernel");
    int64_t tiles = ((3 * B + 31) / 32 + 3) / 4;
    int sg = static_cast<int>(tiles < static_cast<int64_t>(sms) * 16 ? tiles : static_cast<int64_t>(sms) * 16);
    plan_sort_kernel<<<sg, 128, 0, st>>>(p, p.seg.long_cap);
    SLB_LAUNCH_CHECK("plan_sort_kernel");
    plan_sort_long_kernel<<<SEG_LONG_CTAS, 256, 0, st>>>(p);
    SLB_LAUNCH_CHECK("plan_sort_long_kernel");
    return SLB_OK;
}

MfDev v2_dev(const slb_mf_step_args* x, int64_t B, float* loss_out) {
    MfDev a = {};
    a.B = B; a.NB = x->norm_batch > 0 ? x->norm_batch : B; a.T = 2 * B;
    a.loss = x->loss; a.n_neg = 1;
    a.U = x->num_users; a.I = x->num_items; a.D = x->dim;
    a.Wu = x->Wu; a.Wi = x->Wi; a.bu = x->bu; a.bi = x->bi;
    a.loss_out = loss_out;
    a.opt = x->opt; a.lr = x->lr; a.wd = x->weight_decay; a.eps = x->eps;
    a.sWu = x->state_Wu; a.sWi = x->state_Wi; a.sbu = x->state_bu; a.sbi = x->state_bi;
    a.frozen_a = -1; a.frozen_b = -1;
    if (x->opt_users_only) { a.dWi = x->dWi; a.dbi = x->dbi; }
    return a;
}

template <int LPR, int LOSS>
void v2_user_launch(const MfDev& a, const PlanDev& p, const StepV2& v, bool small, int grid, cudaStream_t st) {
    const size_t smem = static_cast<size_t>(256 / LPR) * (LPR * 4 + 4) * sizeof(float);
    mf_user_long_kernel<LPR, LOSS><<<SEG_LONG_CTAS * 4, 256, smem, st>>>(a, p, v);
    if (small) mf_user_kernel<LPR, 1, LOSS, 8><<<grid, MF_TILE_THREADS, 0, st>>>(a, p, v, SEG_LONG_CTAS * 4);
    else if (V2_UVPL == 2 && LPR >= 16) {
        mf_user_kernel<LPR / 2, 2, LOSS, 32><<<grid, MF_TILE_THREADS, 0, st>>>(a, p, v, SEG_LONG_CTAS * 4);
    } else mf_user_kernel<LPR, 1, LOSS, 32><<<grid, MF_TILE_THREADS, 0, st>>>(a, p, v, SEG_LONG_CTAS * 4);
}

template <int LPR>
void v2_user_dispatch(const MfDev& a, const PlanDev& p, const StepV2& v, bool small, int grid, cudaStream_t st) {
    switch (a.loss) {
        case SLB_LOSS_POINTWISE: v2_user_launch<LPR, SLB_LOSS_POINTWISE>(a, p, v, small, grid, st); break;
        case SLB_LOSS_BPR: v2_user_launch<LPR, SLB_LOSS_BPR>(a, p, v, small, grid, st); break;
        default: v2_user_launch<LPR, SLB_LOSS_HINGE>(a, p, v, small, grid, st); break;
    }
}

template <int LPR>
void v2_item_launch(const MfDev& a, const PlanDev& p, const StepV2& v, bool small, int grid, cudaStream_t st) {
    const size_t smem = static_cast<size_t>(256 / LPR) * (LPR * 4 + 4) * sizeof(float);
    mf_item_long_kernel<LPR><<<SEG_LONG_CTAS * 4, 256, smem, st>>>(a, p, v);
    if (small) mf_item_kernel<LPR, 8><<<grid, MF_TILE_THREADS, 0, st>>>(a, p, v);
    else mf_item_kernel<LPR, 32><<<grid, MF_TILE_THREADS, 0, st>>>(a, p, v);
}

int v2_launch_step(const slb_mf_step_args* x, const V2Layout& l, int slot, int32_t* err, const int64_t* users,
                   const int64_t* items, const int64_t* negs, int64_t B, float* loss_out, cudaStream_t st,
                   int phases) {
    if (phases & 1) {
        const int rc = v2_launch_plan(x, l.plan[slot], err, users, items, negs, B, st);
        if (rc != SLB_OK) return rc;
    }
    PlanDev p = l.plan[slot];
    p.B = B; p.users = users; p.items = items; p.negs = negs; p.err = err;
    p.seg.long_cap = seg_sort_cap(lpr_for_dim(x->dim));
    const MfDev a = v2_dev(x, B, loss_out);
    const int sms = slb_sms();
    const int lpr = x->dim / 4;
    if (phases & 2) {
        const bool small = B < static_cast<int64_t>(sms) * 24 * 32;
        const int64_t tw = ((B + (small ? 8 : 32) - 1) / (small ? 8 : 32) + 3) / 4;
        const int grid = static_cast<int>(tw < MF_MAX_GRID ? (tw < 1 ? 1 : tw) : MF_MAX_GRID);
        switch (lpr) {
            case 2: v2_user_dispatch<2>(a, p, l.st, small, grid, st); break;
            case 4: v2_user_dispatch<4>(a, p, l.st, small, grid, st); break;
            case 8: v2_user_dispatch<8>(a, p, l.st, small, grid, st); break;
            case 16: v2_user_dispatch<16>(a, p, l.st, small, grid, st); break;
            default: v2_user_dispatch<32>(a, p, l.st, small, grid, st); break;
        }
        SLB_LAUNCH_CHECK("mf_user_kernel");
    }
    if (phases & 4) {
        const bool small = 2 * B < static_cast<int64_t>(sms) * 24 * 32;
        const int64_t tw = ((2 * B + (small ? 8 : 32) - 1) / (small ? 8 : 32) + 3) / 4;
        const int grid = static_cast<int>(tw < static_cast<int64_t>(sms) * 16 ? (tw < 1 ? 1 : tw) : static_cast<int64_t>(sms) * 16);
        switch (lpr) {
            case 2: v2_item_launch<2>(a, p, l.st, small, grid, st); break;
            case 4: v2_item_launch<4>(a, p, l.st, small, grid, st); break;
            case 8: v2_item_launch<8>(a, p, l.st, small, grid, st); break;
            case 16: v2_item_launch<16>(a, p, l.st, small, grid, st); break;
            default: v2_item_launch<32>(a, p, l.st, small, grid, st); break;
        }
        SLB_LAUNCH_CHECK("mf_item_kernel");
    }
    return SLB_OK;
}

int v2_check_ws(const slb_mf_step_args* x) {
    const size_t need = v2_layout(nullptr, x->batch, x->num_users, x->num_items, x->dim).bytes;
    if (x->fused_workspace_bytes < need) {
        slb_set_error("mf_train_step: fused workspace too small (%zu < %zu)", x->fused_workspace_bytes, need);
        return SLB_ENOSPC;
    }
    return SLB_OK;
}

}

extern "C" {

size_t slb_mf_step_workspace_bytes(int64_t batch, int32_t n_neg, int32_t loss,
                                   int64_t num_users, int64_t num_items) {
    (void)n_neg; (void)loss;
    return mf_layout(nullptr, batch, num_users, num_items).bytes;
}

int64_t slb_mf_compact_rows(int64_t batch, int32_t n_neg, int32_t loss, int32_t which) {
    (void)n_neg; (void)loss; (void)which;
    return 2 * batch;
}

size_t slb_mf_fused_workspace_bytes(int64_t batch, int64_t num_users, int64_t num_items, int32_t dim) {
    if (batch <= 0 || !v2_dim_ok(dim)) return 0;
    return v2_layout(nullptr, batch, num_users, num_items, dim).bytes;
}

int slb_mf_train_step(const slb_mf_step_args* x, slb_stream_t stream) {
    const int rc = validate(x);
    if (rc != SLB_OK) return rc;
    if (v2_eligible(x)) {
        const int r2 = v2_check_ws(x);
        if (r2 != SLB_OK) return r2;
        const V2Layout l = v2_layout(x->fused_workspace, x->batch, x->num_users, x->num_items, x->dim);
        MfLayout old = mf_layout(x->workspace, x->batch, x->num_users, x->num_items);
        return v2_launch_step(x, l, 0, old.err, x->users, x->items, x->negs, x->batch, x->loss_out,
                              static_cast<cudaStream_t>(stream), 7);
    }
    return launch_step(x, x->users, x->items, x->negs, x->batch, x->loss_out,
                       static_cast<cudaStream_t>(stream));
}

int slb_mf_train_step_phases(const slb_mf_step_args* x, int32_t phases, slb_stream_t stream) {
    const int rc = validate(x);
    if (rc != SLB_OK) return rc;
    if (v2_eligible(x)) {
        const int r2 = v2_check_ws(x);
        if (r2 != SLB_OK) return r2;
        const V2Layout l = v2_layout(x->fused_workspace, x->batch, x->num_users, x->num_items, x->dim);
        MfLayout old = mf_layout(x->workspace, x->batch, x->num_users, x->num_items);
        return v2_launch_step(x, l, (phases >> 8) & 1, old.err, x->users, x->items, x->negs, x->batch, x->loss_out,
                              static_cast<cudaStream_t>(stream), phases & 7);
    }
    return launch_step(x, x->users, x->items, x->negs, x->batch, x->loss_out,
                       static_cast<cudaStream_t>(stream), phases);
}

static int fit_epoch_impl(const slb_mf_step_args* x, const int64_t* users, const int64_t* items,
                          const int64_t* negs, int64_t n, float* losses_out, slb_stream_t stream,
                          const int64_t* wait_steps, void* const* wait_events, int32_t n_waits) {
    slb_mf_step_args tmp = *x;
    tmp.users = users; tmp.items = items; tmp.negs = negs; tmp.loss_out = losses_out;
    const int rc = validate(&tmp);
    if (rc != SLB_OK) return rc;
    SLB_REQUIRE(x->grad_mode == SLB_GRAD_COMPACT && x->opt != SLB_OPT_NONE,
                "mf_fit_epoch: needs compact grads and a fused optimizer");
    SLB_REQUIRE(n > 0, "mf_fit_epoch: n must be > 0");
    cudaStream_t main_st = static_cast<cudaStream_t>(stream);
    if (v2_eligible(&tmp)) {
        const int r2 = v2_check_ws(&tmp);
        if (r2 != SLB_OK) return r2;
        const V2Layout l = v2_layout(x->fused_workspace, x->batch, x->num_users, x->num_items, x->dim);
        MfLayout old = mf_layout(x->workspace, x->batch, x->num_users, x->num_items);
        cudaStream_t plan_st = x->plan_stream ? static_cast<cudaStream_t>(x->plan_stream) : main_st;
        const bool two = plan_st != main_st;
        const int64_t nsteps = (n + x->batch - 1) / x->batch;
        cudaEvent_t ev_plan[2] = {nullptr, nullptr}, ev_done[2] = {nullptr, nullptr}, ev_in = nullptr;
        int rc2 = SLB_OK;
        if (two) {
            bool ok = cudaEventCreateWithFlags(&ev_in, cudaEventDisableTiming) == cudaSuccess;
            for (int k = 0; k < 2 && ok; ++k)
                ok = cudaEventCreateWithFlags(&ev_plan[k], cudaEventDisableTiming) == cudaSuccess &&
                     cudaEventCreateWithFlags(&ev_done[k], cudaEventDisableTiming) == cudaSuccess;
            if (!ok) { slb_set_error("mf_fit_epoch: cannot create events"); rc2 = SLB_ECUDA; }
            if (rc2 == SLB_OK) {
                cudaEventRecord(ev_in, main_st);
                cudaStreamWaitEvent(plan_st, ev_in, 0);
            }
        }
        int next_wait = 0;
        auto plan_of = [&](int64_t k) {
            const int64_t lo = k * x->batch;
            const int64_t B = n - lo < x->batch ? n - lo : x->batch;
            const int slot = static_cast<int>(k & 1);
            while (next_wait < n_waits && wait_steps[next_wait] <= k) {
                cudaStreamWaitEvent(plan_st, static_cast<cudaEvent_t>(wait_events[next_wait]), 0);
                ++next_wait;
            }
            if (two && k >= 2) cudaStreamWaitEvent(plan_st, ev_done[slot], 0);
            const int r = v2_launch_plan(&tmp, l.plan[slot], old.err, users + lo, items + lo, negs + lo, B, plan_st);
            if (two) cudaEventRecord(ev_plan[slot], plan_st);
            return r;
        };
        if (rc2 == SLB_OK) rc2 = plan_of(0);
        for (int64_t k = 0; k < nsteps && rc2 == SLB_OK; ++k) {
            const int64_t lo = k * x->batch;
            const int64_t B = n - lo < x->batch ? n - lo : x->batch;
            const int slot = static_cast<int>(k & 1);
            if (k + 1 < nsteps) rc2 = plan_of(k + 1);
            if (rc2 != SLB_OK) break;
            if (two) cudaStreamWaitEvent(main_st, ev_plan[slot], 0);
            rc2 = v2_launch_step(&tmp, l, slot, old.err, users + lo, items + lo, negs + lo, B, losses_out + k,
                                 main_st, 6);
            if (two) cudaEventRecord(ev_done[slot], main_st);
        }
        if (two) {
            if (ev_in) { cudaEventRecord(ev_in, main_st); cudaStreamWaitEvent(plan_st, ev_in, 0); }
            for (int k = 0; k < 2; ++k) {
                if (ev_plan[k]) cudaEventDestroy(ev_plan[k]);
                if (ev_done[k]) cudaEventDestroy(ev_done[k]);
            }
            if (ev_in) cudaEventDestroy(ev_in);
        }
        return rc2;
    }
    int64_t step = 0;
    int next_wait = 0;
    for (int64_t lo = 0; lo < n; lo += x->batch, ++step) {
        const int64_t B = n - lo < x->batch ? n - lo : x->batch;
        while (next_wait < n_waits && wait_steps[next_wait] <= step) {
            cudaStreamWaitEvent(main_st, static_cast<cudaEvent_t>(wait_events[next_wait]), 0);
            ++next_wait;
        }
        const int64_t* ng = negs + lo * x->n_neg;
        const int r = launch_step(x, users + lo, items + lo, ng, B, losses_out + step, main_st, 0x1f, step);
        if (r != SLB_OK) return r;
    }
    return SLB_OK;
}

int slb_mf_fit_epoch(const slb_mf_step_args* x, const int64_t* users, const int64_t* items,
                     const int64_t* negs, int64_t n, float* losses_out, slb_stream_t stream) {
    return fit_epoch_impl(x, users, items, negs, n, losses_out, stream, nullptr, nullptr, 0);
}

int slb_mf_fit_epoch_events(const slb_mf_step_args* x, const int64_t* users, const int64_t* items,
                            const int64_t* negs, int64_t n, float* losses_out, slb_stream_t stream,
                            const int64_t* wait_steps, void* const* wait_events, int32_t n_waits) {
    SLB_REQUIRE(n_waits == 0 || (wait_steps && wait_events), "mf_fit_epoch_events: null wait list");
    for (int32_t k = 1; k < n_waits; ++k)
        SLB_REQUIRE(wait_steps[k] >= wait_steps[k - 1], "mf_fit_epoch_events: wait_steps must ascend");
    return fit_epoch_impl(x, users, items, negs, n, losses_out, stream, wait_steps, wait_events, n_waits);
}

int slb_adam_flush(float* W, float* exp_avg, float* exp_avg_sq, float* bias, float* bias_avg, float* bias_avg_sq,
                   int32_t* last, int64_t rows, int32_t dim, const float* sched, int64_t step,
                   float beta1, float beta2, float one_minus_beta1, float one_minus_beta2, float eps,
                   float weight_decay, slb_stream_t stream) {
    SLB_REQUIRE(W && exp_avg && exp_avg_sq && bias && bias_avg && bias_avg_sq && last && sched, "adam_flush: null pointer");
    SLB_REQUIRE(rows > 0 && dim >= 4 && dim % 4 == 0 && step >= 0 && step < (1ll << 31), "adam_flush: bad sizes");
    if (step == 0) return SLB_OK;
    AdamDev o = {beta1, beta2, one_minus_beta1, one_minus_beta2, eps, weight_decay, sched, static_cast<int32_t>(step)};
    const int lpr = lpr_for_dim(dim);
    const int groups = MF_THREADS / lpr;
    const int64_t want = (rows + groups - 1) / groups;
    const int sms = slb_sms();
    const int grid = static_cast<int>(want < static_cast<int64_t>(sms) * 16 ? want : static_cast<int64_t>(sms) * 16);
    cudaStream_t st = static_cast<cudaStream_t>(stream);
    DISPATCH_LPR(lpr, adam_flush_kernel, grid, MF_THREADS, st, W, exp_avg, exp_avg_sq, bias, bias_avg, bias_avg_sq,
                 last, rows, dim, o);
    SLB_LAUNCH_CHECK("adam_flush_kernel");
    return SLB_OK;
}

int slb_mf_scores(const float* Wu, const float* Wi, const float* bu, const float* bi,
                  int32_t dim, const int64_t* users, const int64_t* items, int64_t n,
                  int32_t user_broadcast, float* scores, slb_stream_t stream) {
    SLB_REQUIRE(dim >= 4 && dim % 4 == 0, "mf_scores: dim must be a positive multiple of 4 (got %d)", dim);
    SLB_REQUIRE(Wu && Wi && bu && bi && users && items && scores, "mf_scores: null pointer");
    if (n <= 0) return SLB_OK;
    const int lpr = lpr_for_dim(dim);
    const int groups = MF_THREADS / lpr;
    const int sms = slb_sms();
    int64_t want = (n + groups - 1) / groups;
    int grid = static_cast<int>(want < static_cast<int64_t>(sms) * 8 ? want : static_cast<int64_t>(sms) * 8);
    cudaStream_t st = static_cast<cudaStream_t>(stream);
    DISPATCH_LPR(lpr, mf_scores_kernel, grid, MF_THREADS, st, Wu, Wi, bu, bi, dim, users, items, n,
                 user_broadcast, scores);
    SLB_LAUNCH_CHECK("mf_scores_kernel");
    return SLB_OK;
}

int slb_mf_scores_backward(const float* gscores, const int64_t* users, const int64_t* items,
                           int64_t n, int32_t user_broadcast, const float* Wu, const float* Wi,
                           int64_t num_users, int64_t num_items, int32_t dim,
                           float* dWu, float* dWi, float* dbu, float* dbi,
                           void* workspace, size_t workspace_bytes, slb_stream_t stream) {
    SLB_REQUIRE(dim >= 4 && dim % 4 == 0, "mf_scores_backward: dim must be a positive multiple of 4 (got %d)", dim);
    SLB_REQUIRE(gscores && users && items && Wu && Wi && dWu && dWi && dbu && dbi && workspace,
                "mf_scores_backward: null pointer");
    SLB_REQUIRE(num_users + num_items < (1ll << 31) - SEG_SCAN_TILE && n * 2 < (1ll << 31), "mf_scores_backward: too large");
    if (n <= 0) return SLB_OK;
    const int64_t Bcap = (n + 1) / 2;
    MfLayout l = mf_layout(workspace, Bcap, num_users, num_items);
    if (workspace_bytes < l.bytes) {
        slb_set_error("mf_scores_backward: workspace too small (%zu < %zu)", workspace_bytes, l.bytes);
        return SLB_ENOSPC;
    }
    MfDev a = {};
    a.B = n; a.NB = n; a.T = n; a.users = users; a.items = items;
    a.U = num_users; a.I = num_items; a.D = dim;
    a.Wu = const_cast<float*>(Wu); a.Wi = const_cast<float*>(Wi);
    a.t_a = l.t_a; a.t_b = l.t_b; a.t_g = l.t_g; a.partial = l.partial; a.done = l.done; a.err = l.err;
    a.seg = l.seg;
    a.seg.long_cap = seg_sort_cap(lpr_for_dim(dim));
    a.no_bias = 0; a.frozen_a = -1; a.frozen_b = -1;
    a.grad_mode = SLB_GRAD_DENSE;
    a.dWu = dWu; a.dWi = dWi; a.dbu = dbu; a.dbi = dbi;
    cudaStream_t st = static_cast<cudaStream_t>(stream);
    const int sms = slb_sms();
    int g1 = static_cast<int>((n + 255) / 256);
    if (g1 > sms * 8) g1 = sms * 8;
    mf_terms_kernel<<<g1, 256, 0, st>>>(a, gscores, user_broadcast);
    SLB_LAUNCH_CHECK("mf_terms_kernel");
    seg_scan_launch(a.seg, a.U, st);
    SLB_LAUNCH_CHECK("seg_scan_kernel");
    mf_fill_kernel<<<g1, 256, 0, st>>>(a);
    SLB_LAUNCH_CHECK("mf_fill_kernel");
    seg_sort_long_kernel<<<SEG_LONG_CTAS, 256, 0, st>>>(a.seg);
    SLB_LAUNCH_CHECK("seg_sort_long_kernel");
    const int lpr = lpr_for_dim(dim);
    int64_t tw = ((n + 31) / 32 + 3) / 4;
    int tgrid = static_cast<int>(tw < static_cast<int64_t>(sms) * 16 ? tw : static_cast<int64_t>(sms) * 16);
    DISPATCH_LPR3(lpr, mf_bwd_tile_kernel, 0, 32, tgrid, MF_TILE_THREADS, st, a);
    SLB_LAUNCH_CHECK("mf_bwd_tile_kernel");
    launch_long<0>(lpr, st, a);
    SLB_LAUNCH_CHECK("mf_bwd_long_kernel");
    return SLB_OK;
}

}

namespace {

struct BiasSparse {
    SegIndex seg;
    const int64_t* ids; const float* g; int64_t n; int64_t mask;
    float* b; float* sb;
    int32_t opt; float lr, wd, eps;
};

__global__ void __launch_bounds__(256) bias_count_kernel(BiasSparse p) {
    const int64_t nth = static_cast<int64_t>(gridDim.x) * blockDim.x;
    for (int64_t k = static_cast<int64_t>(blockIdx.x) * blockDim.x + threadIdx.x; k < p.n; k += nth)
        if (p.g[k] != 0.f) atomicAdd(p.seg.cnt + (p.ids[k] & p.mask), 1);
}

__global__ void __launch_bounds__(256) bias_fill_kernel(BiasSparse p) {
    const int64_t nth = static_cast<int64_t>(gridDim.x) * blockDim.x;
    for (int64_t k = static_cast<int64_t>(blockIdx.x) * blockDim.x + threadIdx.x; k < p.n; k += nth)
        if (p.g[k] != 0.f) seg_place(p.seg, p.ids[k] & p.mask, static_cast<int32_t>(k));
}

__global__ void __launch_bounds__(256) bias_apply_kernel(BiasSparse p) {
    const int nseg = p.seg.totals[0];
    const OptV2 o = {p.opt, p.lr, p.wd, p.eps};
    const int nth = gridDim.x * blockDim.x;
    for (int s = blockIdx.x * blockDim.x + threadIdx.x; s < nseg; s += nth) {
        const int start = p.seg.seg_start[s], len = p.seg.seg_start[s + 1] - start;
        int64_t last_id = -1;
        for (;;) {
            int64_t cur = INT64_MAX;
            for (int m = 0; m < len; ++m) {
                const int64_t id = p.ids[p.seg.members[start + m]];
                if (id > last_id && id < cur) cur = id;
            }
            if (cur == INT64_MAX) break;
            float acc = 0.f;
            int prev = -1;
            for (;;) {
                int best = INT32_MAX;
                for (int m = 0; m < len; ++m) {
                    const int k = p.seg.members[start + m];
                    if (k > prev && k < best && p.ids[k] == cur) best = k;
                }
                if (best == INT32_MAX) break;
                acc += p.g[best];
                prev = best;
            }
            bias_update(o, p.b + cur, p.sb ? p.sb + cur : nullptr, acc);
            last_id = cur;
        }
    }
}

size_t bias_sparse_bytes(int64_t n) {
    int64_t nb = 4096;
    while (nb < 2 * n) nb <<= 1;
    WsCarver ws(nullptr);
    seg_index_carve(ws, nb, n);
    return ws.bytes();
}

int bias_sparse_apply(void* wsp, const int64_t* ids, const float* g, int64_t n, float* b, float* sb,
                      int32_t opt, float lr, float wd, float eps, cudaStream_t st) {
    int64_t nb = 4096;
    while (nb < 2 * n) nb <<= 1;
    WsCarver ws(wsp);
    BiasSparse p;
    p.seg = seg_index_carve(ws, nb, n);
    p.ids = ids; p.g = g; p.n = n; p.mask = nb - 1; p.b = b; p.sb = sb;
    p.opt = opt; p.lr = lr; p.wd = wd; p.eps = eps;
    const int sms = slb_sms();
    int grid = static_cast<int>((n + 255) / 256);
    if (grid > sms * 8) grid = sms * 8;
    bias_count_kernel<<<grid, 256, 0, st>>>(p);
    SLB_LAUNCH_CHECK("bias_count_kernel");
    seg_scan_launch(p.seg, p.seg.Rpad, st);
    SLB_LAUNCH_CHECK("seg_scan_kernel");
    bias_fill_kernel<<<grid, 256, 0, st>>>(p);
    SLB_LAUNCH_CHECK("bias_fill_kernel");
    bias_apply_kernel<<<grid, 256, 0, st>>>(p);
    SLB_LAUNCH_CHECK("bias_apply_kernel");
    return SLB_OK;
}

}

struct BloomLayout {
    int32_t* t_a; int32_t* t_b; float* t_g; float* partial; int32_t* done; int32_t* err;
    SegIndex seg;
    int64_t* ids_u2; int64_t* ids_i2; float* g_u2; float* g_i2;
    void* ws_u; size_t ws_u_bytes; void* ws_i; size_t ws_i_bytes;
    int64_t* irows; float* gWi; int32_t* compact_counts; void* bws_u; void* bws_i;
    size_t bytes;
};

static BloomLayout bloom_layout(void* base, const slb_mf_bloom_args* x) {
    const int nu = x->user_hashes ? x->user_hashes : 1, ni = x->item_hashes ? x->item_hashes : 1;
    const int64_t B = x->base.batch, T = 2 * B * nu * ni;
    WsCarver ws(base);
    BloomLayout l;
    l.done = ws.take<int32_t>(8);
    l.err = l.done + 4;
    l.seg = seg_index_carve(ws, x->user_rows + x->item_rows, 2 * T);
    l.t_a = ws.take<int32_t>(T);
    l.t_b = ws.take<int32_t>(T);
    l.t_g = ws.take<float>(T);
    l.partial = ws.take<float>(MF_MAX_GRID);
    l.ids_u2 = ws.take<int64_t>(2 * B);
    l.ids_i2 = ws.take<int64_t>(2 * B);
    l.g_u2 = ws.take<float>(2 * B);
    l.g_i2 = ws.take<float>(2 * B);
    l.irows = nullptr; l.gWi = nullptr; l.compact_counts = nullptr; l.bws_u = nullptr; l.bws_i = nullptr;
    l.ws_u = nullptr; l.ws_i = nullptr; l.ws_u_bytes = 0; l.ws_i_bytes = 0;
    if (x->base.opt == SLB_OPT_NONE) {
        l.ws_u_bytes = slb_embedding_backward_workspace_bytes(2 * B, x->base.num_users);
        l.ws_u = ws.take<char>(l.ws_u_bytes);
        l.ws_i_bytes = slb_embedding_backward_workspace_bytes(2 * B, x->base.num_items);
        l.ws_i = ws.take<char>(l.ws_i_bytes);
    } else {
        l.bws_u = ws.take<char>(bias_sparse_bytes(2 * B));
        l.bws_i = ws.take<char>(bias_sparse_bytes(2 * B));
        const int64_t irow_cap = T < x->item_rows ? T : x->item_rows;
        l.irows = ws.take<int64_t>(irow_cap + 1);
        l.gWi = ws.take<float>(static_cast<size_t>(irow_cap + 1) * x->base.dim);
        l.compact_counts = ws.take<int32_t>(4);
    }
    l.bytes = ws.bytes();
    return l;
}

extern "C" {

size_t slb_mf_bloom_workspace_bytes(const slb_mf_bloom_args* x) {
    if (!x || x->base.batch <= 0) return 0;
    return bloom_layout(nullptr, x).bytes;
}

int slb_mf_bloom_train_step(const slb_mf_bloom_args* x, slb_stream_t stream) {
    SLB_REQUIRE(x != nullptr, "mf_bloom_train_step: null args");
    const slb_mf_step_args& b = x->base;
    SLB_REQUIRE(b.batch > 0 && b.dim >= 4 && b.dim % 4 == 0, "mf_bloom_train_step: bad batch / dim");
    SLB_REQUIRE(b.loss >= 0 && b.loss <= 3 && b.n_neg >= 1, "mf_bloom_train_step: bad loss / n_neg");
    SLB_REQUIRE(b.loss == SLB_LOSS_ADAPTIVE_HINGE || b.n_neg == 1, "mf_bloom_train_step: n_neg > 1 only for adaptive hinge");
    const bool fused = b.opt != SLB_OPT_NONE;
    SLB_REQUIRE(fused ? (b.opt == SLB_OPT_SGD || b.opt == SLB_OPT_ADAGRAD) : b.grad_mode == SLB_GRAD_DENSE,
                "mf_bloom_train_step: dense gradients, or a fused SGD / Adagrad optimizer");
    SLB_REQUIRE(!fused || b.opt == SLB_OPT_SGD || (b.state_Wu && b.state_Wi && b.state_bu && b.state_bi),
                "mf_bloom_train_step: adagrad needs state");
    SLB_REQUIRE(x->user_hashes >= 0 && x->user_hashes <= 24 && x->item_hashes >= 0 && x->item_hashes <= 24,
                "mf_bloom_train_step: at most 24 hash functions");
    SLB_REQUIRE(x->user_rows > 0 && x->item_rows > 0 && b.num_users > 0 && b.num_items > 0, "mf_bloom_train_step: empty tables");
    SLB_REQUIRE(x->user_hashes > 0 || x->user_rows == b.num_users, "mf_bloom_train_step: plain user table must have num_users rows");
    SLB_REQUIRE(x->item_hashes > 0 || x->item_rows == b.num_items, "mf_bloom_train_step: plain item table must have num_items rows");
    const bool pairs_u = x->pair_ids_u && x->pair_g_u, pairs_i = x->pair_ids_i && x->pair_g_i;
    SLB_REQUIRE(b.users && b.items && b.negs && b.Wu && b.Wi && b.bu && b.bi && b.loss_out && b.workspace &&
                (fused || (b.dWu && b.dWi && (b.dbu || pairs_u) && (b.dbi || pairs_i))), "mf_bloom_train_step: null pointer");
    const int nu = x->user_hashes ? x->user_hashes : 1, ni = x->item_hashes ? x->item_hashes : 1;
    const int64_t B = b.batch, T = 2 * B * nu * ni;
    SLB_REQUIRE(x->user_rows + x->item_rows < (1ll << 31) - SEG_SCAN_TILE && 2 * T < (1ll << 31),
                "mf_bloom_train_step: too large");
    BloomLayout l = bloom_layout(b.workspace, x);
    if (b.workspace_bytes < l.bytes) {
        slb_set_error("mf_bloom_train_step: workspace too small (%zu < %zu)", b.workspace_bytes, l.bytes);
        return SLB_ENOSPC;
    }
    cudaStream_t st = static_cast<cudaStream_t>(stream);
    MfDev a = {};
    a.B = B; a.NB = b.norm_batch > 0 ? b.norm_batch : B; a.T = T;
    a.users = b.users; a.items = b.items; a.negs = b.negs; a.loss = b.loss; a.n_neg = b.n_neg;
    a.U = x->user_rows; a.I = x->item_rows; a.D = b.dim;
    a.Wu = b.Wu; a.Wi = b.Wi; a.bu = b.bu; a.bi = b.bi;
    a.loss_out = b.loss_out; a.pos_out = b.pos_out; a.neg_out = b.neg_out;
    a.t_a = l.t_a; a.t_b = l.t_b; a.t_g = l.t_g; a.partial = l.partial; a.done = l.done; a.err = l.err;
    a.seg = l.seg;
    const int lpr = lpr_for_dim(b.dim);
    a.seg.long_cap = seg_sort_cap(lpr);
    a.grad_mode = fused ? SLB_GRAD_COMPACT : SLB_GRAD_DENSE;
    a.dWu = b.dWu; a.dWi = b.dWi; a.dbu = b.dbu; a.dbi = b.dbi;
    a.irows = l.irows; a.gWi = l.gWi; a.compact_counts = l.compact_counts;
    a.opt = b.opt; a.lr = b.lr; a.wd = b.weight_decay; a.eps = b.eps;
    a.sWu = b.state_Wu; a.sWi = b.state_Wi; a.sbu = b.state_bu; a.sbi = b.state_bi;
    a.no_bias = 1;
    a.frozen_a = x->user_hashes ? x->user_padding_idx : -1;
    a.frozen_b = x->item_hashes ? x->item_padding_idx : -1;
    BloomSpec h = {};
    h.Hu = x->user_hashes; h.Hi = x->item_hashes;
    h.pad_u = x->user_padding_idx; h.pad_i = x->item_padding_idx;
    for (int k = 0; k < 24; ++k) { h.su[k] = x->user_seeds[k]; h.si[k] = x->item_seeds[k]; }
    h.num_users = b.num_users; h.num_items = b.num_items;
    h.ids_u2 = l.ids_u2; h.ids_i2 = l.ids_i2; h.g_u2 = l.g_u2; h.g_i2 = l.g_i2;
    if (!fused && pairs_u) { h.ids_u2 = x->pair_ids_u; h.g_u2 = x->pair_g_u; }
    if (!fused && pairs_i) { h.ids_i2 = x->pair_ids_i; h.g_i2 = x->pair_g_i; }

    const int groups = MF_THREADS / lpr;
    const int sms = slb_sms();
    int64_t want = (B + groups - 1) / groups;
    int grid = static_cast<int>(want < static_cast<int64_t>(sms) * 8 ? want : static_cast<int64_t>(sms) * 8);
    if (grid > MF_MAX_GRID) grid = MF_MAX_GRID;
    switch (lpr) {
        case 1: mf_fwd_bloom_kernel<1><<<grid, MF_THREADS, 0, st>>>(a, h); break;
        case 2: mf_fwd_bloom_kernel<2><<<grid, MF_THREADS, 0, st>>>(a, h); break;
        case 4: mf_fwd_bloom_kernel<4><<<grid, MF_THREADS, 0, st>>>(a, h); break;
        case 8: mf_fwd_bloom_kernel<8><<<grid, MF_THREADS, 0, st>>>(a, h); break;
        case 16: mf_fwd_bloom_kernel<16><<<grid, MF_THREADS, 0, st>>>(a, h); break;
        default: mf_fwd_bloom_kernel<32><<<grid, MF_THREADS, 0, st>>>(a, h); break;
    }
    SLB_LAUNCH_CHECK("mf_fwd_bloom_kernel");
    seg_scan_launch(a.seg, a.U, st);
    SLB_LAUNCH_CHECK("seg_scan_kernel");
    int fgrid = static_cast<int>((T + 255) / 256);
    if (fgrid > sms * 8) fgrid = sms * 8;
    mf_fill_kernel<<<fgrid, 256, 0, st>>>(a);
    SLB_LAUNCH_CHECK("mf_fill_kernel");
    seg_sort_long_kernel<<<SEG_LONG_CTAS, 256, 0, st>>>(a.seg);
    SLB_LAUNCH_CHECK("seg_sort_long_kernel");
    const int64_t tw = ((2 * T + 31) / 32 + 3) / 4;
    const int tgrid = static_cast<int>(tw < static_cast<int64_t>(sms) * 16 ? tw : static_cast<int64_t>(sms) * 16);
    if (fused) {
        DISPATCH_LPR3(lpr, mf_bwd_tile_kernel, 1, 32, tgrid, MF_TILE_THREADS, st, a);
        SLB_LAUNCH_CHECK("mf_bwd_tile_kernel<items>");
        launch_long<1>(lpr, st, a);
        DISPATCH_LPR3(lpr, mf_bwd_tile_kernel, 2, 32, tgrid, MF_TILE_THREADS, st, a);
        SLB_LAUNCH_CHECK("mf_bwd_tile_kernel<users+opt>");
        launch_long<2>(lpr, st, a);
        const int64_t aw = (2 * T + groups - 1) / groups;
        const int agrid = static_cast<int>(aw < static_cast<int64_t>(sms) * 8 ? aw : static_cast<int64_t>(sms) * 8);
        DISPATCH_LPR2(lpr, mf_apply_kernel, 1, agrid, MF_THREADS, st, a);
        SLB_LAUNCH_CHECK("mf_apply_kernel<items>");
        int rcb = bias_sparse_apply(l.bws_u, l.ids_u2, l.g_u2, 2 * B, b.bu, b.state_bu, b.opt, b.lr, b.weight_decay, b.eps, st);
        if (rcb != SLB_OK) return rcb;
        return bias_sparse_apply(l.bws_i, l.ids_i2, l.g_i2, 2 * B, b.bi, b.state_bi, b.opt, b.lr, b.weight_decay, b.eps, st);
    }
    DISPATCH_LPR3(lpr, mf_bwd_tile_kernel, 0, 32, tgrid, MF_TILE_THREADS, st, a);
    SLB_LAUNCH_CHECK("mf_bwd_tile_kernel");
    launch_long<0>(lpr, st, a);
    SLB_LAUNCH_CHECK("mf_bwd_long_kernel");
    int rc = SLB_OK;
    if (!pairs_u)
        rc = slb_embedding_backward(l.g_u2, l.ids_u2, 2 * B, 0, nullptr, b.num_users, 1, -1, b.dbu, l.ws_u,
                                    l.ws_u_bytes, stream);
    if (rc != SLB_OK) return rc;
    if (!pairs_i)
        rc = slb_embedding_backward(l.g_i2, l.ids_i2, 2 * B, 0, nullptr, b.num_items, 1, -1, b.dbi, l.ws_i,
                                    l.ws_i_bytes, stream);
    return rc;
}

size_t slb_bias_sparse_workspace_bytes(int64_t n) { return n > 0 ? bias_sparse_bytes(n) : 0; }

int slb_bias_sparse_apply(const int64_t* ids, const float* g, int64_t n, float* bias, float* state,
                          int32_t opt, float lr, float weight_decay, float eps,
                          void* workspace, size_t workspace_bytes, slb_stream_t stream) {
    if (n <= 0) return SLB_OK;
    SLB_REQUIRE(ids && g && bias && workspace, "bias_sparse_apply: null pointer");
    SLB_REQUIRE(opt == SLB_OPT_SGD || (opt == SLB_OPT_ADAGRAD && state), "bias_sparse_apply: SGD, or Adagrad with state");
    SLB_REQUIRE(n < (1ll << 30), "bias_sparse_apply: too many pairs");
    if (workspace_bytes < bias_sparse_bytes(n)) {
        slb_set_error("bias_sparse_apply: workspace too small");
        return SLB_ENOSPC;
    }
    return bias_sparse_apply(workspace, ids, g, n, bias, state, opt, lr, weight_decay, eps,
                             static_cast<cudaStream_t>(stream));
}

}
```

### spotlight_b200/csrc/mf_v2.cuh

```cuda
#pragma once

struct __align__(16) URec { int32_t b, i, j, pad; };
struct __align__(8) IRec { int32_t t, useg; };

struct PlanDev {
    SegIndex seg;
    URec* mu;
    IRec* mi;
    URec* mu_tmp;
    IRec* mi_tmp;
    uint32_t* bits;
    int64_t words;
    int32_t* err;
    int64_t B, U, I;
    const int64_t* users; const int64_t* items; const int64_t* negs;
};

struct StepV2 {
    float* t_g;
    float* stash;
    float* partial;
    float* partial_long;
    int32_t* done;
};


__global__ void __launch_bounds__(256) plan_count_kernel(PlanDev p) {
    const int64_t nth = static_cast<int64_t>(gridDim.x) * blockDim.x;
    if (blockIdx.x == 0 && threadIdx.x == 0) p.seg.totals[3] = 0;
    for (int64_t b = static_cast<int64_t>(blockIdx.x) * blockDim.x + threadIdx.x; b < p.B; b += nth) {
        const int64_t u = p.users[b], i = p.items[b], j = p.negs[b];
        if (u < 0 || u >= p.U || i < 0 || i >= p.I || j < 0 || j >= p.I) { atomicExch(p.err, 1); continue; }
        atomicAdd(p.seg.cnt + u, 1);
        atomicAdd(p.seg.cnt + p.U + i, 1);
        atomicAdd(p.seg.cnt + p.U + j, 1);
    }
}

__global__ void __launch_bounds__(256) plan_fill_kernel(PlanDev p) {
    const int64_t nth = static_cast<int64_t>(gridDim.x) * blockDim.x;
    const int ubase = p.seg.seg_start[p.seg.totals[2]];
    for (int64_t b = static_cast<int64_t>(blockIdx.x) * blockDim.x + threadIdx.x; b < p.B; b += nth) {
        const int64_t u = p.users[b], i = p.items[b], j = p.negs[b];
        if (u < 0 || u >= p.U || i < 0 || i >= p.I || j < 0 || j >= p.I) continue;
        const int su = p.seg.off[u] + atomicSub(p.seg.cnt + u, 1) - 1;
        URec r;
        r.b = static_cast<int32_t>(b); r.i = static_cast<int32_t>(i); r.j = static_cast<int32_t>(j); r.pad = 0;
        p.mu[su] = r;
        const int useg = p.seg.sid[u];
        const int si = p.seg.off[p.U + i] + atomicSub(p.seg.cnt + p.U + i, 1) - 1 - ubase;
        const int sj = p.seg.off[p.U + j] + atomicSub(p.seg.cnt + p.U + j, 1) - 1 - ubase;
        IRec a; a.t = static_cast<int32_t>(2 * b); a.useg = useg;
        IRec c; c.t = static_cast<int32_t>(2 * b + 1); c.useg = useg;
        p.mi[si] = a;
        p.mi[sj] = c;
    }
}

__device__ __forceinline__ int rec_key(const URec& r) { return r.b; }
__device__ __forceinline__ int rec_key(const IRec& r) { return r.t; }

constexpr int PLAN_SORT_SMALL = 16;

__device__ __forceinline__ URec rec_shfl_xor(const URec& r, int j) {
    URec o;
    o.b = __shfl_xor_sync(0xffffffffu, r.b, j); o.i = __shfl_xor_sync(0xffffffffu, r.i, j);
    o.j = __shfl_xor_sync(0xffffffffu, r.j, j); o.pad = 0;
    return o;
}
__device__ __forceinline__ IRec rec_shfl_xor(const IRec& r, int j) {
    IRec o;
    o.t = __shfl_xor_sync(0xffffffffu, r.t, j); o.useg = __shfl_xor_sync(0xffffffffu, r.useg, j);
    return o;
}
__device__ __forceinline__ void rec_set_key(URec& r, int k) { r.b = k; r.i = 0; r.j = 0; r.pad = 0; }
__device__ __forceinline__ void rec_set_key(IRec& r, int k) { r.t = k; r.useg = 0; }

template <typename Rec>
__device__ __forceinline__ void plan_sort_tile(Rec* base, int start, int len, int cap, Rec* tmp_base) {
    const int lane = threadIdx.x & 31;
    if (len == 2) {
        const Rec x = base[start], y = base[start + 1];
        if (rec_key(x) > rec_key(y)) { base[start] = y; base[start + 1] = x; }
    }
    unsigned net = __ballot_sync(0xffffffffu, len > 2 && len <= PLAN_SORT_SMALL);
    const int half = lane >> 4, lid = lane & 15;
    while (net) {
        const int s0 = __ffs(net) - 1;
        net &= net - 1;
        int s1 = -1;
        if (net) { s1 = __ffs(net) - 1; net &= net - 1; }
        const int mine = half == 0 ? s0 : s1;
        const int m_start = __shfl_sync(0xffffffffu, start, mine < 0 ? 0 : mine);
        const int t_len = __shfl_sync(0xffffffffu, len, mine < 0 ? 0 : mine);
        const int m_len = mine < 0 ? 0 : t_len;
        Rec v;
        if (lid < m_len) v = base[m_start + lid];
        else rec_set_key(v, 0x7fffffff);
#pragma unroll
        for (int k = 2; k <= 16; k <<= 1) {
#pragma unroll
            for (int j = k >> 1; j > 0; j >>= 1) {
                const Rec o = rec_shfl_xor(v, j);
                const bool keep_min = ((lid & j) == 0) == ((lid & k) == 0);
                const bool other_smaller = rec_key(o) < rec_key(v);
                if (keep_min == other_smaller) v = o;
            }
        }
        if (lid < m_len) base[m_start + lid] = v;
    }
    unsigned med = __ballot_sync(0xffffffffu, len > PLAN_SORT_SMALL && len <= cap);
    while (med) {
        const int src = __ffs(med) - 1;
        med &= med - 1;
        const int s_start = __shfl_sync(0xffffffffu, start, src);
        const int s_len = __shfl_sync(0xffffffffu, len, src);
        for (int i = lane; i < s_len; i += 32) {
            const Rec x = base[s_start + i];
            int r = 0;
            for (int m = 0; m < s_len; ++m) r += rec_key(base[s_start + m]) < rec_key(x);
            tmp_base[s_start + r] = x;
        }
        __syncwarp();
        for (int i = lane; i < s_len; i += 32) base[s_start + i] = tmp_base[s_start + i];
        __syncwarp();
    }
}

__global__ void __launch_bounds__(128) plan_sort_kernel(PlanDev p, int cap) {
    const int nseg = p.seg.totals[0], nsegA = p.seg.totals[2];
    const int ubase = p.seg.seg_start[nsegA];
    const int lane = threadIdx.x & 31;
    const int ntiles = (nseg + 31) / 32;
    for (int tile = blockIdx.x * 4 + (threadIdx.x >> 5); tile < ntiles; tile += gridDim.x * 4) {
        const int s = tile * 32 + lane;
        int start = 0, len = 0;
        if (s < nseg) { start = p.seg.seg_start[s]; len = p.seg.seg_start[s + 1] - start; }
        plan_sort_tile<URec>(p.mu, start, (s < nsegA) ? len : 0, cap, p.mu_tmp);
        plan_sort_tile<IRec>(p.mi, start - ubase, (s >= nsegA && s < nseg) ? len : 0, cap, p.mi_tmp);
    }
}

template <typename Rec>
__device__ void plan_sort_long_one(Rec* base, Rec* tmp, int start, int len, uint32_t* bits, uint32_t* pre,
                                   int W, uint32_t* sh_scan) {
    const int per = (W + 255) / 256;
    for (int w = threadIdx.x; w < W; w += 256) bits[w] = 0u;
    __syncthreads();
    for (int i = threadIdx.x; i < len; i += 256) {
        const int t = rec_key(base[start + i]);
        atomicOr(bits + (t >> 5), 1u << (t & 31));
    }
    __syncthreads();
    const int lo = threadIdx.x * per, hi = lo + per < W ? lo + per : W;
    uint32_t sum = 0;
    for (int w = lo; w < hi; ++w) sum += __popc(bits[w]);
    sh_scan[threadIdx.x] = sum;
    __syncthreads();
    for (int o = 1; o < 256; o <<= 1) {
        const uint32_t v = threadIdx.x >= o ? sh_scan[threadIdx.x - o] : 0u;
        __syncthreads();
        sh_scan[threadIdx.x] += v;
        __syncthreads();
    }
    uint32_t run = sh_scan[threadIdx.x] - sum;
    for (int w = lo; w < hi; ++w) { pre[w] = run; run += __popc(bits[w]); }
    __syncthreads();
    for (int i = threadIdx.x; i < len; i += 256) {
        const Rec x = base[start + i];
        const int t = rec_key(x);
        const uint32_t r = pre[t >> 5] + __popc(bits[t >> 5] & ((1u << (t & 31)) - 1u));
        tmp[start + r] = x;
    }
    __syncthreads();
    for (int i = threadIdx.x; i < len; i += 256) base[start + i] = tmp[start + i];
    __syncthreads();
}

__global__ void __launch_bounds__(256) plan_sort_long_kernel(PlanDev p) {
    __shared__ uint32_t sh_scan[256];
    const int nlong = p.seg.totals[3];
    const int nsegA = p.seg.totals[2];
    const int ubase = p.seg.seg_start[nsegA];
    uint32_t* bits = p.bits + static_cast<size_t>(blockIdx.x) * 2 * p.words;
    uint32_t* pre = bits + p.words;
    for (int li = blockIdx.x; li < nlong; li += gridDim.x) {
        const int s = p.seg.long_list[li];
        const int start = p.seg.seg_start[s];
        const int len = p.seg.seg_start[s + 1] - start;
        if (s < nsegA) plan_sort_long_one<URec>(p.mu, p.mu_tmp, start, len, bits, pre, static_cast<int>((p.B + 31) / 32), sh_scan);
        else plan_sort_long_one<IRec>(p.mi, p.mi_tmp, start - ubase, len, bits, pre, static_cast<int>((2 * p.B + 31) / 32), sh_scan);
    }
}



#ifndef V2_UMINB
#define V2_UMINB 8
#endif
#ifndef V2_UMINB2
#define V2_UMINB2 6
#endif
#ifndef V2_UVPL
#define V2_UVPL 2
#endif
#ifndef V2_UPF
#define V2_UPF 0
#endif

template <int VPL>
struct RowV { float4 v[VPL]; };

template <int LPR, int VPL>
__device__ __forceinline__ RowV<VPL> row_ldg(const float* row, int gl) {
    RowV<VPL> r;
#pragma unroll
    for (int q = 0; q < VPL; ++q) r.v[q] = ldg4(row + gl * 4 + q * LPR * 4);
    return r;
}
template <int LPR, int VPL>
__device__ __forceinline__ RowV<VPL> row_ldcs(const float* row, int gl) {
    RowV<VPL> r;
#pragma unroll
    for (int q = 0; q < VPL; ++q) r.v[q] = __ldcs(reinterpret_cast<const float4*>(row + gl * 4 + q * LPR * 4));
    return r;
}
template <int VPL>
__device__ __forceinline__ RowV<VPL> row_zero() {
    RowV<VPL> r;
#pragma unroll
    for (int q = 0; q < VPL; ++q) r.v[q] = make_float4(0.f, 0.f, 0.f, 0.f);
    return r;
}

template <int LPR, int VPL, int LOSS, bool FULL>
__device__ __forceinline__ void user_member(const RowV<VPL>& w, float ub, const RowV<VPL>& qi, const RowV<VPL>& qj,
                                            float bi_, float bj_, int b, float invB, unsigned gmask, int gl,
                                            float* t_g, RowV<VPL>& acc, float& bacc, bool& nz, float& lsum) {
    float dp = 0.f, dn = 0.f;
#pragma unroll
    for (int q = 0; q < VPL; ++q) { dp += dot4(w.v[q], qi.v[q]); dn += dot4(w.v[q], qj.v[q]); }
    dp = group_sum<LPR>(dp, FULL ? 0xffffffffu : gmask);
    dn = group_sum<LPR>(dn, FULL ? 0xffffffffu : gmask);
    float per, gp, gn;
    pair_loss(LOSS, dp + ub + bi_, dn + ub + bj_, per, gp, gn);
    gp *= invB; gn *= invB;
    if (gl == 0) {
        lsum += per;
        *reinterpret_cast<float2*>(t_g + 2 * static_cast<int64_t>(b)) = make_float2(gp, gn);
    }
#pragma unroll
    for (int q = 0; q < VPL; ++q) { fma4(acc.v[q], gp, qi.v[q]); fma4(acc.v[q], gn, qj.v[q]); }
    bacc += gp + gn;
    nz = nz || gp != 0.f || gn != 0.f;
}

template <int LPR, int VPL>
__device__ __forceinline__ void user_finish(const MfDev& a, const OptV2& o, float* stash_row, float* wrow, float* srow,
                                            RowV<VPL> w, RowV<VPL> s, const RowV<VPL>& acc, float bacc, bool nz,
                                            int row, int gl) {
#pragma unroll
    for (int q = 0; q < VPL; ++q) st4(stash_row + gl * 4 + q * LPR * 4, w.v[q]);
    if (nz) {
#pragma unroll
        for (int q = 0; q < VPL; ++q) {
            row_update(o, w.v[q], s.v[q], acc.v[q]);
            __stcs(reinterpret_cast<float4*>(wrow + gl * 4 + q * LPR * 4), w.v[q]);
            if (srow) __stcs(reinterpret_cast<float4*>(srow + gl * 4 + q * LPR * 4), s.v[q]);
        }
        if (gl == 0) bias_update(o, a.bu + row, a.sbu ? a.sbu + row : nullptr, bacc);
    }
}

template <int LPR, int VPL, int LOSS, int TI>
__global__ void __launch_bounds__(MF_TILE_THREADS, (VPL == 1 ? V2_UMINB : V2_UMINB2)) mf_user_kernel(MfDev a, PlanDev p, StepV2 v, int n_long_partials) {
    constexpr int D = LPR * 4 * VPL;
    constexpr int GPW = 32 / LPR;
    constexpr int WARPS = MF_TILE_THREADS / 32;
    __shared__ float sh_red[WARPS];
    __shared__ int sh_inv[WARPS][32];
    __shared__ bool is_last;
    const int lane = threadIdx.x & 31;
    const int warp = threadIdx.x >> 5;
    const int gl = lane & (LPR - 1);
    const int grp = lane / LPR;
    const unsigned gmask = group_mask(LPR);
    const unsigned below = (1u << lane) - 1u;
    const float invB = 1.0f / static_cast<float>(a.NB);
    const OptV2 o = {a.opt, a.lr, a.wd, a.eps};
    const int nsegA = p.seg.totals[2];
    const int ntiles = (nsegA + TI - 1) / TI;
    const int wstride = gridDim.x * WARPS;
    const int cap = p.seg.long_cap;
    const bool adagrad = a.opt == SLB_OPT_ADAGRAD;
    float lsum = 0.f;

    for (int tile = blockIdx.x * WARPS + warp; tile < ntiles; tile += wstride) {
        const int sidx = tile * TI + lane;
        const bool valid = lane < TI && sidx < nsegA;
        int start = 0, len = 0, row = 0;
        int4 r0 = make_int4(0, 0, 0, 0), r1 = r0;
        if (valid) {
            start = p.seg.seg_start[sidx];
            len = p.seg.seg_start[sidx + 1] - start;
            row = p.seg.seg_row[sidx];
            r0 = __ldg(reinterpret_cast<const int4*>(p.mu + start));
            if (len == 2) r1 = __ldg(reinterpret_cast<const int4*>(p.mu + start + 1));
#if V2_UPF
            pf_row_l2(a.Wu + static_cast<int64_t>(row) * D, D);
            if (adagrad) pf_row_l2(a.sWu + static_cast<int64_t>(row) * D, D);
#endif
        }
        const unsigned m1 = __ballot_sync(0xffffffffu, len == 1);
        const unsigned m2 = __ballot_sync(0xffffffffu, len == 2);
        const unsigned m3 = __ballot_sync(0xffffffffu, len > 2);
        const int n1 = __popc(m1), n2 = __popc(m2), n3 = __popc(m3);
        int pos;
        if (len == 1) pos = __popc(m1 & below);
        else if (len == 2) pos = n1 + __popc(m2 & below);
        else if (len > 2) pos = n1 + n2 + __popc(m3 & below);
        else pos = n1 + n2 + n3 + __popc(~(m1 | m2 | m3) & below);
        __syncwarp();
        sh_inv[warp][pos] = lane;
        __syncwarp();
        const int nvalid = n1 + n2 + n3;

        for (int q0 = 0; q0 < nvalid; q0 += GPW) {
            const int q = q0 + grp;
            const int src = sh_inv[warp][q & 31];
            const int s_len = __shfl_sync(0xffffffffu, len, src);
            const int s_row = __shfl_sync(0xffffffffu, row, src);
            const int b0 = __shfl_sync(0xffffffffu, r0.x, src);
            const int i0 = __shfl_sync(0xffffffffu, r0.y, src);
            const int j0 = __shfl_sync(0xffffffffu, r0.z, src);
            const int s = tile * TI + src;
            float* wrow = a.Wu + static_cast<int64_t>(s_row) * D;
            float* srow = adagrad ? a.sWu + static_cast<int64_t>(s_row) * D : nullptr;
            float* stash_row = v.stash + static_cast<int64_t>(s) * D;
            RowV<VPL> acc = row_zero<VPL>();
            float bacc = 0.f;
            bool nz = false;
            if (q0 + GPW <= n1) {
                const RowV<VPL> w = row_ldcs<LPR, VPL>(wrow, gl);
                RowV<VPL> st_ = row_zero<VPL>();
                if (adagrad) st_ = row_ldcs<LPR, VPL>(srow, gl);
                const RowV<VPL> qi = row_ldg<LPR, VPL>(a.Wi + static_cast<int64_t>(i0) * D, gl);
                const RowV<VPL> qj = row_ldg<LPR, VPL>(a.Wi + static_cast<int64_t>(j0) * D, gl);
                const float ub = a.bu[s_row], bi_ = __ldg(a.bi + i0), bj_ = __ldg(a.bi + j0);
                user_member<LPR, VPL, LOSS, true>(w, ub, qi, qj, bi_, bj_, b0, invB, gmask, gl, v.t_g, acc, bacc, nz, lsum);
                user_finish<LPR, VPL>(a, o, stash_row, wrow, srow, w, st_, acc, bacc, nz, s_row, gl);
            } else if (q0 >= n1 && q0 + GPW <= n1 + n2) {
                const int b1 = __shfl_sync(0xffffffffu, r1.x, src);
                const int i1 = __shfl_sync(0xffffffffu, r1.y, src);
                const int j1 = __shfl_sync(0xffffffffu, r1.z, src);
                const RowV<VPL> w = row_ldcs<LPR, VPL>(wrow, gl);
                RowV<VPL> st_ = row_zero<VPL>();
                if (adagrad) st_ = row_ldcs<LPR, VPL>(srow, gl);
                const RowV<VPL> qi0 = row_ldg<LPR, VPL>(a.Wi + static_cast<int64_t>(i0) * D, gl);
                const RowV<VPL> qj0 = row_ldg<LPR, VPL>(a.Wi + static_cast<int64_t>(j0) * D, gl);
                const float ub = a.bu[s_row];
                const float bi0 = __ldg(a.bi + i0), bj0 = __ldg(a.bi + j0), bi1 = __ldg(a.bi + i1), bj1 = __ldg(a.bi + j1);
                user_member<LPR, VPL, LOSS, true>(w, ub, qi0, qj0, bi0, bj0, b0, invB, gmask, gl, v.t_g, acc, bacc, nz, lsum);
                const RowV<VPL> qi1 = row_ldg<LPR, VPL>(a.Wi + static_cast<int64_t>(i1) * D, gl);
                const RowV<VPL> qj1 = row_ldg<LPR, VPL>(a.Wi + static_cast<int64_t>(j1) * D, gl);
                user_member<LPR, VPL, LOSS, true>(w, ub, qi1, qj1, bi1, bj1, b1, invB, gmask, gl, v.t_g, acc, bacc, nz, lsum);
                user_finish<LPR, VPL>(a, o, stash_row, wrow, srow, w, st_, acc, bacc, nz, s_row, gl);
            } else {
                const int s_start = __shfl_sync(0xffffffffu, start, src);
                if (q >= nvalid || s_len > cap) continue;
                const RowV<VPL> w = row_ldcs<LPR, VPL>(wrow, gl);
                RowV<VPL> st_ = row_zero<VPL>();
                if (adagrad) st_ = row_ldcs<LPR, VPL>(srow, gl);
                const float ub = a.bu[s_row];
                for (int k = 0; k < s_len; ++k) {
                    const int4 r = __ldg(reinterpret_cast<const int4*>(p.mu + s_start + k));
                    const RowV<VPL> qi = row_ldg<LPR, VPL>(a.Wi + static_cast<int64_t>(r.y) * D, gl);
                    const RowV<VPL> qj = row_ldg<LPR, VPL>(a.Wi + static_cast<int64_t>(r.z) * D, gl);
                    user_member<LPR, VPL, LOSS, false>(w, ub, qi, qj, __ldg(a.bi + r.y), __ldg(a.bi + r.z), r.x, invB, gmask,
                                                       gl, v.t_g, acc, bacc, nz, lsum);
                }
                user_finish<LPR, VPL>(a, o, stash_row, wrow, srow, w, st_, acc, bacc, nz, s_row, gl);
            }
        }
    }

    const float bsum = block_sum<MF_TILE_THREADS>(lsum, sh_red);
    if (threadIdx.x == 0) {
        v.partial[blockIdx.x] = bsum;
        __threadfence();
        is_last = atomicAdd(v.done, 1) == static_cast<int>(gridDim.x) - 1;
    }
    __syncthreads();
    if (is_last && threadIdx.x < 32) {
        __threadfence();
        float t = 0.f;
        for (int k = threadIdx.x; k < static_cast<int>(gridDim.x); k += 32)
            t += *reinterpret_cast<volatile float*>(v.partial + k);
        for (int k = threadIdx.x; k < n_long_partials; k += 32)
            t += *reinterpret_cast<volatile float*>(v.partial_long + k);
#pragma unroll
        for (int off = 16; off > 0; off >>= 1) t += __shfl_down_sync(0xffffffffu, t, off);
        if (threadIdx.x == 0) { *a.loss_out = t * invB; *v.done = 0; }
    }
}

template <int LPR, int LOSS>
__global__ void __launch_bounds__(256) mf_user_long_kernel(MfDev a, PlanDev p, StepV2 v) {
    constexpr int D = LPR * 4;
    constexpr int GROUPS = 256 / LPR;
    constexpr int PS = D + 4;
    extern __shared__ float sh_part[];
    __shared__ float sh_red[8];
    const int gl = threadIdx.x & (LPR - 1);
    const int gq = threadIdx.x / LPR;
    const int c = gl * 4;
    const unsigned gmask = group_mask(LPR);
    const float invB = 1.0f / static_cast<float>(a.NB);
    const OptV2 o = {a.opt, a.lr, a.wd, a.eps};
    const int nlong = p.seg.totals[3];
    const int nsegA = p.seg.totals[2];
    float lsum = 0.f;
    for (int li = blockIdx.x; li < nlong; li += gridDim.x) {
        const int s = p.seg.long_list[li];
        if (s >= nsegA) continue;
        const int start = p.seg.seg_start[s];
        const int len = p.seg.seg_start[s + 1] - start;
        const int row = p.seg.seg_row[s];
        float* wrow = a.Wu + static_cast<int64_t>(row) * D + c;
        const float4 w4 = ld4(wrow);
        const float ub = a.bu[row];
        const int chunk = (len + GROUPS - 1) / GROUPS;
        const int lo = min(gq * chunk, len), hi = min(lo + chunk, len);
        float4 acc = make_float4(0.f, 0.f, 0.f, 0.f);
        float bacc = 0.f, nzf = 0.f;
        for (int k = lo; k < hi; ++k) {
            const int4 r0 = __ldg(reinterpret_cast<const int4*>(p.mu + start + k));
            const float4 a0 = ldg4(a.Wi + static_cast<int64_t>(r0.y) * D + c), b0 = ldg4(a.Wi + static_cast<int64_t>(r0.z) * D + c);
            const float dp = group_sum<LPR>(dot4(w4, a0), gmask);
            const float dn = group_sum<LPR>(dot4(w4, b0), gmask);
            float per, gp, gn;
            pair_loss(LOSS, dp + ub + __ldg(a.bi + r0.y), dn + ub + __ldg(a.bi + r0.z), per, gp, gn);
            gp *= invB; gn *= invB;
            if (gl == 0) {
                lsum += per;
                *reinterpret_cast<float2*>(v.t_g + 2 * static_cast<int64_t>(r0.x)) = make_float2(gp, gn);
            }
            fma4(acc, gp, a0);
            fma4(acc, gn, b0);
            bacc += gp + gn;
            if (gp != 0.f || gn != 0.f) nzf = 1.f;
        }
        st4(sh_part + gq * PS + c, acc);
        if (gl == 0) { sh_part[gq * PS + D] = bacc; sh_part[gq * PS + D + 1] = nzf; }
        __syncthreads();
        if (gq == 0) {
            float4 tot = make_float4(0.f, 0.f, 0.f, 0.f);
            float bt = 0.f, nzt = 0.f;
            for (int q = 0; q < GROUPS; ++q) {
                const float4 x = ld4(sh_part + q * PS + c);
                tot.x += x.x; tot.y += x.y; tot.z += x.z; tot.w += x.w;
                bt += sh_part[q * PS + D];
                nzt += sh_part[q * PS + D + 1];
            }
            st4(v.stash + static_cast<int64_t>(s) * D + c, w4);
            if (nzt != 0.f) {
                float4 wn = w4, s4 = make_float4(0.f, 0.f, 0.f, 0.f);
                float* srow = a.opt == SLB_OPT_ADAGRAD ? a.sWu + static_cast<int64_t>(row) * D + c : nullptr;
                if (srow) s4 = ld4(srow);
                row_update(o, wn, s4, tot);
                st4(wrow, wn);
                if (srow) st4(srow, s4);
                if (gl == 0) bias_update(o, a.bu + row, a.sbu ? a.sbu + row : nullptr, bt);
            }
        }
        __syncthreads();
    }
    const float bsum = block_sum<256>(lsum, sh_red);
    if (threadIdx.x == 0) v.partial_long[blockIdx.x] = bsum;
}


#ifndef V2_IFAST
#define V2_IFAST 4
#endif
#ifndef V2_IMINB
#define V2_IMINB 6
#endif
#ifndef V2_ICHUNK
#define V2_ICHUNK 8
#endif

template <int LPR, int TI>
__global__ void __launch_bounds__(MF_TILE_THREADS, V2_IMINB) mf_item_kernel(MfDev a, PlanDev p, StepV2 v) {
    constexpr int D = LPR * 4;
    constexpr int GPW = 32 / LPR;
    constexpr int ITERS = TI / GPW > 0 ? TI / GPW : 1;
    constexpr int WARPS = MF_TILE_THREADS / 32;
    constexpr int CAP = seg_sort_cap(LPR);
    __shared__ int32_t sh_all[WARPS * GPW * 2 * CAP];
    const int lane = threadIdx.x & 31;
    const int gl = lane & (LPR - 1);
    const int grp = lane / LPR;
    const int c = gl * 4;
    const unsigned gmask = group_mask(LPR);
    int32_t* sh = sh_all + ((threadIdx.x >> 5) * GPW + grp) * 2 * CAP;
    const OptV2 o = {a.opt, a.lr, a.wd, a.eps};
    const int nseg = p.seg.totals[0];
    const int nsegA = p.seg.totals[2];
    const int ubase = p.seg.seg_start[nsegA];
    const int ntiles = (nseg - nsegA + TI - 1) / TI;
    const int wstride = gridDim.x * WARPS;
    const float* __restrict__ t_g = v.t_g;

    for (int tile = blockIdx.x * WARPS + (threadIdx.x >> 5); tile < ntiles; tile += wstride) {
        const int sidx = nsegA + tile * TI + lane;
        const bool valid = lane < TI && sidx < nseg;
        int start = 0, len = 0, row = 0;
        int pu[V2_IFAST] = {};
        float pg[V2_IFAST] = {};
        if (valid) {
            start = p.seg.seg_start[sidx] - ubase;
            len = p.seg.seg_start[sidx + 1] - ubase - start;
            row = p.seg.seg_row[sidx] - static_cast<int>(a.U);
            if (len <= V2_IFAST) {
#pragma unroll
                for (int k = 0; k < V2_IFAST; ++k)
                    if (k < len) {
                        const int2 r = __ldg(reinterpret_cast<const int2*>(p.mi + start + k));
                        pu[k] = r.y;
                        pg[k] = t_g[r.x];
                    }
            }
        }
        for (int it = 0; it < ITERS; ++it) {
            const int src = it * GPW + grp;
            const int s_len = __shfl_sync(0xffffffffu, len, src & 31);
            const int s_row = __shfl_sync(0xffffffffu, row, src & 31);
            const int s_start = __shfl_sync(0xffffffffu, start, src & 31);
            int su[V2_IFAST];
            float sg[V2_IFAST];
#pragma unroll
            for (int k = 0; k < V2_IFAST; ++k) {
                su[k] = __shfl_sync(0xffffffffu, pu[k], src & 31);
                sg[k] = __shfl_sync(0xffffffffu, pg[k], src & 31);
            }
            const int s = nsegA + tile * TI + src;
            if (src >= TI || s >= nseg) continue;
            if (s_len > CAP) continue;
            float4 acc = make_float4(0.f, 0.f, 0.f, 0.f);
            float bacc = 0.f;
            bool nz = false;
            if (s_len <= V2_IFAST) {
                float4 x[V2_IFAST];
#pragma unroll
                for (int k = 0; k < V2_IFAST; ++k)
                    if (k < s_len) x[k] = ld4(v.stash + static_cast<int64_t>(su[k]) * D + c);
#pragma unroll
                for (int k = 0; k < V2_IFAST; ++k)
                    if (k < s_len) { fma4(acc, sg[k], x[k]); bacc += sg[k]; nz = nz || sg[k] != 0.f; }
            } else {
                float* lg = reinterpret_cast<float*>(sh);
                int32_t* lu = sh + CAP;
                for (int i = gl; i < s_len; i += LPR) {
                    const int2 r = __ldg(reinterpret_cast<const int2*>(p.mi + s_start + i));
                    lg[i] = t_g[r.x];
                    lu[i] = r.y;
                    pf_row_l2(v.stash + static_cast<int64_t>(r.y) * D, D);
                }
                __syncwarp(gmask);
                int i = 0;
                for (; i + V2_ICHUNK <= s_len; i += V2_ICHUNK) {
                    float4 x[V2_ICHUNK];
#pragma unroll
                    for (int k = 0; k < V2_ICHUNK; ++k) x[k] = ld4(v.stash + static_cast<int64_t>(lu[i + k]) * D + c);
#pragma unroll
                    for (int k = 0; k < V2_ICHUNK; ++k) { fma4(acc, lg[i + k], x[k]); bacc += lg[i + k]; nz = nz || lg[i + k] != 0.f; }
                }
                for (; i < s_len; ++i) {
                    fma4(acc, lg[i], ld4(v.stash + static_cast<int64_t>(lu[i]) * D + c));
                    bacc += lg[i];
                    nz = nz || lg[i] != 0.f;
                }
                __syncwarp(gmask);
            }
            if (a.dWi) {
                st4(a.dWi + static_cast<int64_t>(s_row) * D + c, acc);
                if (gl == 0) a.dbi[s_row] = bacc;
            } else if (nz) {
                float* wrow = a.Wi + static_cast<int64_t>(s_row) * D + c;
                float* srow = a.opt == SLB_OPT_ADAGRAD ? a.sWi + static_cast<int64_t>(s_row) * D + c : nullptr;
                float4 w4 = ld4(wrow);
                float4 s4 = make_float4(0.f, 0.f, 0.f, 0.f);
                if (srow) s4 = ld4(srow);
                row_update(o, w4, s4, acc);
                st4(wrow, w4);
                if (srow) st4(srow, s4);
                if (gl == 0) bias_update(o, a.bi + s_row, a.sbi ? a.sbi + s_row : nullptr, bacc);
            }
        }
    }
}

template <int LPR>
__global__ void __launch_bounds__(256) mf_item_long_kernel(MfDev a, PlanDev p, StepV2 v) {
    constexpr int D = LPR * 4;
    constexpr int GROUPS = 256 / LPR;
    constexpr int PS = D + 4;
    extern __shared__ float sh_part[];
    const int gl = threadIdx.x & (LPR - 1);
    const int gq = threadIdx.x / LPR;
    const int c = gl * 4;
    const OptV2 o = {a.opt, a.lr, a.wd, a.eps};
    const int nlong = p.seg.totals[3];
    const int nsegA = p.seg.totals[2];
    const int ubase = p.seg.seg_start[nsegA];
    for (int li = blockIdx.x; li < nlong; li += gridDim.x) {
        const int s = p.seg.long_list[li];
        if (s < nsegA) continue;
        const int start = p.seg.seg_start[s] - ubase;
        const int len = p.seg.seg_start[s + 1] - ubase - start;
        const int row = p.seg.seg_row[s] - static_cast<int>(a.U);
        const int chunk = (len + GROUPS - 1) / GROUPS;
        const int lo = min(gq * chunk, len), hi = min(lo + chunk, len);
        float4 acc = make_float4(0.f, 0.f, 0.f, 0.f);
        float bacc = 0.f, nzf = 0.f;
        int i = lo;
        for (; i + 4 <= hi; i += 4) {
            int2 r[4]; float g[4]; float4 x[4];
#pragma unroll
            for (int k = 0; k < 4; ++k) r[k] = __ldg(reinterpret_cast<const int2*>(p.mi + start + i + k));
#pragma unroll
            for (int k = 0; k < 4; ++k) { g[k] = v.t_g[r[k].x]; x[k] = ld4(v.stash + static_cast<int64_t>(r[k].y) * D + c); }
#pragma unroll
            for (int k = 0; k < 4; ++k) { fma4(acc, g[k], x[k]); bacc += g[k]; if (g[k] != 0.f) nzf = 1.f; }
        }
        for (; i < hi; ++i) {
            const int2 r = __ldg(reinterpret_cast<const int2*>(p.mi + start + i));
            const float g = v.t_g[r.x];
            fma4(acc, g, ld4(v.stash + static_cast<int64_t>(r.y) * D + c));
            bacc += g;
            if (g != 0.f) nzf = 1.f;
        }
        st4(sh_part + gq * PS + c, acc);
        if (gl == 0) { sh_part[gq * PS + D] = bacc; sh_part[gq * PS + D + 1] = nzf; }
        __syncthreads();
        if (gq == 0) {
            float4 tot = make_float4(0.f, 0.f, 0.f, 0.f);
            float bt = 0.f, nzt = 0.f;
            for (int q = 0; q < GROUPS; ++q) {
                const float4 x = ld4(sh_part + q * PS + c);
                tot.x += x.x; tot.y += x.y; tot.z += x.z; tot.w += x.w;
                bt += sh_part[q * PS + D];
                nzt += sh_part[q * PS + D + 1];
            }
            if (a.dWi) {
                st4(a.dWi + static_cast<int64_t>(row) * D + c, tot);
                if (gl == 0) a.dbi[row] = bt;
            } else if (nzt != 0.f) {
                float* wrow = a.Wi + static_cast<int64_t>(row) * D + c;
                float* srow = a.opt == SLB_OPT_ADAGRAD ? a.sWi + static_cast<int64_t>(row) * D + c : nullptr;
                float4 w4 = ld4(wrow), s4 = make_float4(0.f, 0.f, 0.f, 0.f);
                if (srow) s4 = ld4(srow);
                row_update(o, w4, s4, tot);
                st4(wrow, w4);
                if (srow) st4(srow, s4);
                if (gl == 0) bias_update(o, a.bi + row, a.sbi ? a.sbi + row : nullptr, bt);
            }
        }
        __syncthreads();
    }
}
```

### spotlight_b200/factorization/implicit.py

```python

import ctypes
import os

import numpy as np
import torch
import torch.optim as optim

from spotlight_b200 import _lib, ops
from spotlight_b200.factorization._components import _predict_process_ids
from spotlight_b200.factorization.representations import BilinearNet
from spotlight_b200.helpers import _repr_model
from spotlight_b200.losses import adaptive_hinge_loss, bpr_loss, hinge_loss, pointwise_loss
from spotlight_b200.rng import (SHUFFLE_DEVICE_MAX, permute_ids, shuffle_begin, shuffle_end,
                                shuffled_order_device)
from spotlight_b200.sampling import sample_items
from spotlight_b200.torch_utils import cpu, gpu, minibatch, set_seed, shuffled_order

_SIDE_STREAMS = {}


def _side_stream(device):
    key = torch.device(device).index
    if key not in _SIDE_STREAMS:
        _SIDE_STREAMS[key] = torch.cuda.Stream(device=device, priority=-1)
    return _SIDE_STREAMS[key]


_PLAN_STREAMS = {}


def _plan_stream(device):
    key = torch.device(device).index
    if key not in _PLAN_STREAMS:
        _PLAN_STREAMS[key] = torch.cuda.Stream(device=device, priority=-1)
    return _PLAN_STREAMS[key]


def _to_device_ids(ids, device):
    return _to_device_narrow(ids, device).long()


def _to_device_narrow(ids, device):
    arr = np.ascontiguousarray(ids)
    if arr.dtype not in (np.int32, np.int64):
        arr = arr.astype(np.int64)
    host = torch.from_numpy(arr)
    return host.to(device, non_blocking=host.is_pinned())


PLANNED_STEP = True

DEVICE_SHUFFLE_MIN = 1 << 17

_NO_CPU = ('spotlight_b200 runs the fit() hot path in sm_100a CUDA kernels and has no CPU '
           'route; construct the model with use_cuda=True.')


class ImplicitFactorizationModel(object):

    def __init__(self, loss='pointwise', embedding_dim=32, n_iter=10, batch_size=256, l2=0.0,
                 learning_rate=1e-2, optimizer_func=None, use_cuda=False, representation=None,
                 sparse=False, random_state=None, num_negative_samples=5):

        assert loss in ('pointwise', 'bpr', 'hinge', 'adaptive_hinge')

        self._loss = loss
        self._embedding_dim = embedding_dim
        self._n_iter = n_iter
        self._learning_rate = learning_rate
        self._batch_size = batch_size
        self._l2 = l2
        self._use_cuda = use_cuda
        self._representation = representation
        self._sparse = sparse
        self._optimizer_func = optimizer_func
        self._random_state = random_state or np.random.RandomState()
        self._num_negative_samples = num_negative_samples

        self._num_users = None
        self._num_items = None
        self._net = None
        self._optimizer = None
        self._loss_func = None

        set_seed(self._random_state.randint(-10**8, 10**8), cuda=self._use_cuda)

    def __repr__(self):
        return _repr_model(self)

    @property
    def _initialized(self):
        return self._net is not None

    def _initialize(self, interactions):
        if not self._use_cuda:
            raise RuntimeError(_NO_CPU)
        (self._num_users, self._num_items) = (interactions.num_users, interactions.num_items)

        if self._representation is not None:
            self._net = gpu(self._representation, self._use_cuda)
        else:
            self._net = gpu(BilinearNet(self._num_users, self._num_items, self._embedding_dim,
                                        sparse=self._sparse), self._use_cuda)

        if self._optimizer_func is None:
            if isinstance(self._net, BilinearNet) and self._net.plain_tables() and not self._sparse:
                from spotlight_b200.optim import FusedAdam
                self._optimizer = FusedAdam(self._net.parameters(), weight_decay=self._l2,
                                            lr=self._learning_rate)
            else:
                self._optimizer = optim.Adam(self._net.parameters(), weight_decay=self._l2,
                                             lr=self._learning_rate)
        else:
            self._optimizer = self._optimizer_func(self._net.parameters())

        self._loss_func = {'pointwise': pointwise_loss, 'bpr': bpr_loss, 'hinge': hinge_loss,
                           'adaptive_hinge': adaptive_hinge_loss}[self._loss]

    def _check_input(self, user_ids, item_ids, allow_items_none=False):
        user_id_max = user_ids if isinstance(user_ids, int) else user_ids.max()
        if user_id_max >= self._num_users:
            raise ValueError('Maximum user id greater than number of users in model.')
        if allow_items_none and item_ids is None:
            return
        item_id_max = item_ids if isinstance(item_ids, int) else item_ids.max()
        if item_id_max >= self._num_items:
            raise ValueError('Maximum item id greater than number of items in model.')


    def _route(self):
        net = self._net
        fusable = isinstance(net, BilinearNet) and net.plain_tables()
        if fusable and getattr(self._optimizer, 'fused_kind', None) is not None:
            return 'epoch'
        if fusable and not self._sparse:
            return 'fused'
        if isinstance(net, BilinearNet) and not self._sparse and net.fused_spec() is not None:
            return 'bloom'
        return 'generic'

    def _n_neg(self):
        return self._num_negative_samples if self._loss == 'adaptive_hinge' else 1

    def _device(self):
        return next(self._net.parameters()).device

    def _epoch_negatives(self, n_interactions):
        return sample_items(self._num_items, n_interactions * self._n_neg(),
                            random_state=self._random_state, device=self._device())

    def fit(self, interactions, verbose=False):
        user_ids = interactions.user_ids
        item_ids = interactions.item_ids

        if not self._initialized:
            self._initialize(interactions)
        if not self._use_cuda:
            raise RuntimeError(_NO_CPU)

        route = self._route()
        device = self._device()
        n = len(user_ids)
        on_device = DEVICE_SHUFFLE_MIN <= n <= SHUFFLE_DEVICE_MAX and \
            self._random_state.get_state()[0] == 'MT19937'
        main = torch.cuda.current_stream(device)
        pending = (shuffle_begin(n, self._random_state, device), main) if on_device and self._n_iter > 0 \
            else None
        copy_stream = _side_stream(device)
        with torch.cuda.stream(copy_stream):
            users_dev = _to_device_narrow(user_ids, device)
            items_dev = _to_device_narrow(item_ids, device)
        torch.cuda.current_stream(device).wait_stream(copy_stream)
        users_dev.record_stream(torch.cuda.current_stream(device))
        items_dev.record_stream(torch.cuda.current_stream(device))
        if users_dev.dtype != items_dev.dtype:
            users_dev, items_dev = users_dev.long(), items_dev.long()
        if n:
            umax, imax, umin, imin = torch.stack([users_dev.max(), items_dev.max(), users_dev.min(),
                                                  items_dev.min()]).tolist()
            self._check_input(int(umax), int(imax))
            if umin < 0 or imin < 0:
                raise IndexError('index out of range in self: negative user or item id')

        for epoch_num in range(self._n_iter):
            if pending is not None:
                handle, stream = pending
                with torch.cuda.stream(stream):
                    order_dev = shuffle_end(handle)
                if stream is not main:
                    main.wait_stream(stream)
                    order_dev.record_stream(main)
                pending = None
            elif on_device:
                order_dev = shuffled_order_device(n, self._random_state, device)
            else:
                order = shuffled_order(n, self._random_state)
                order_dev = torch.from_numpy(order).to(device).long()
            user_ids_tensor, item_ids_tensor = permute_ids(order_dev, users_dev, items_dev)
            del order_dev

            if route == 'epoch':
                def next_permutation(last=epoch_num + 1 >= self._n_iter):
                    nonlocal pending
                    if on_device and not last:
                        side = _side_stream(device)
                        with torch.cuda.stream(side):
                            pending = (shuffle_begin(n, self._random_state, device), side)
                epoch_loss = self._run_epoch_device(user_ids_tensor, item_ids_tensor,
                                                    after_sampling=next_permutation)
            elif route == 'bloom' and getattr(self._optimizer, 'fused_kind', None) in (_lib.OPT_SGD, _lib.OPT_ADAGRAD):
                negatives = self._epoch_negatives(len(user_ids))
                epoch_loss = self._fit_epoch_bloom_fused(user_ids_tensor, item_ids_tensor, negatives)
            else:
                negatives = self._epoch_negatives(len(user_ids))
                epoch_loss = self._fit_epoch_autograd(user_ids_tensor, item_ids_tensor, negatives,
                                                      fused=route)

            if verbose:
                print('Epoch {}: loss {}'.format(epoch_num, epoch_loss))

            if np.isnan(epoch_loss) or epoch_loss == 0.0:
                raise ValueError('Degenerate epoch loss: {}'.format(epoch_loss))
        if hasattr(self._optimizer, 'flush'):
            self._optimizer.flush()

    def _run_epoch_device(self, users, items, chunk_batches=48, after_sampling=None):
        n, B, n_neg = users.numel(), int(self._batch_size), self._n_neg()
        dev = users.device
        main = torch.cuda.current_stream(dev)
        side = _side_stream(dev)
        chunk = max(1, int(chunk_batches)) * B

        negs_all = torch.empty(n * n_neg, dtype=torch.int64, device=dev)
        side.wait_stream(main)
        from spotlight_b200 import rng as _rng
        with torch.cuda.stream(side):
            _rng.reserve(self._num_items, min(chunk, n) * n_neg, dev)
            stream = _rng.DeviceStream(self._random_state, dev)
        waits = []
        lo = 0
        with torch.cuda.stream(side):
            while lo < n:
                cur = min(chunk, n - lo)
                stream.draw(self._num_items, cur * n_neg, out=negs_all[lo * n_neg:(lo + cur) * n_neg])
                ev = torch.cuda.Event()
                ev.record(side)
                waits.append((lo // B, ev))
                lo += cur
        losses = self._fit_epoch_pipeline(users, items, negs_all, sync=False, waits=waits)
        with torch.cuda.stream(side):
            stream.finish()
        if after_sampling is not None:
            after_sampling()
        host = losses.cpu().numpy().astype(np.float64)
        ws = ops.workspace('mf%d_%d' % (self._num_users, self._num_items), 0, dev)
        if ops.workspace_error_flag(ws):
            raise ValueError('ids out of range reached the device kernels')
        return float(host.sum() / len(host))

    def _fit_epoch_pipeline(self, users, items, negatives, sync=True, waits=()):
        net, opt = self._net, self._optimizer
        lib = _lib.load()
        n, B, n_neg = users.numel(), int(self._batch_size), self._n_neg()
        Wu, Wi = net.user_embeddings.weight, net.item_embeddings.weight
        bu, bi = net.user_biases.weight, net.item_biases.weight
        dev = Wu.device
        with torch.no_grad():
            a = ops.mf_step_args(Wu, Wi, bu, bi, users, items, negatives, self._loss, n_neg,
                                 batch=min(B, n))
            a.grad_mode = _lib.GRAD_COMPACT
            fused_need = 0
            if self._loss != 'adaptive_hinge' and PLANNED_STEP and opt.fused_kind != _lib.OPT_ADAM:
                fused_need = lib.slb_mf_fused_workspace_bytes(a.batch, a.num_users, a.num_items, a.dim)
            if fused_need:
                fws = ops.workspace('mfv2_%d_%d_%d' % (a.num_users, a.num_items, a.dim),
                                    fused_need, dev)
                a.fused_workspace, a.fused_workspace_bytes = fws.data_ptr(), fws.numel()
                if not os.environ.get('SLB_PLAN_SAME_STREAM'):
                    a.plan_stream = _plan_stream(dev).cuda_stream
                keep = (fws,)
            else:
                rows = lib.slb_mf_compact_rows(a.batch, n_neg, a.loss, 0)
                D = a.dim
                urows = torch.empty(rows, dtype=torch.int64, device=dev)
                irows = torch.empty(rows, dtype=torch.int64, device=dev)
                gWu = torch.empty((rows, D), dtype=torch.float32, device=dev)
                gWi = torch.empty((rows, D), dtype=torch.float32, device=dev)
                gbu = torch.empty(rows, dtype=torch.float32, device=dev)
                gbi = torch.empty(rows, dtype=torch.float32, device=dev)
                counts = torch.zeros(2, dtype=torch.int32, device=dev)
                a.urows, a.gWu, a.gbu = urows.data_ptr(), gWu.data_ptr(), gbu.data_ptr()
                a.irows, a.gWi, a.gbi = irows.data_ptr(), gWi.data_ptr(), gbi.data_ptr()
                a.compact_counts = counts.data_ptr()
                keep = (urows, irows, gWu, gWi, gbu, gbi, counts)
            hp = opt.fused_hparams()
            a.opt, a.lr, a.weight_decay, a.eps = opt.fused_kind, hp['lr'], hp['weight_decay'], hp['eps']
            n_steps = (n + B - 1) // B
            if opt.fused_kind == _lib.OPT_ADAGRAD:
                states = [opt.fused_state(p) for p in (Wu, Wi, bu, bi)]
                a.state_Wu, a.state_Wi, a.state_bu, a.state_bi = [s.data_ptr() for s in states]
            elif opt.fused_kind == _lib.OPT_ADAM:
                states = [opt.fused_states(p) for p in (Wu, Wi, bu, bi)]
                a.state_Wu, a.state_Wi, a.state_bu, a.state_bi = [s[0].data_ptr() for s in states]
                a.state2_Wu, a.state2_Wi, a.state2_bu, a.state2_bi = [s[1].data_ptr() for s in states]
                a.last_u, a.last_i = states[0][2].data_ptr(), states[1][2].data_ptr()
                a.beta1, a.beta2 = hp['beta1'], hp['beta2']
                a.one_minus_beta1, a.one_minus_beta2 = 1.0 - hp['beta1'], 1.0 - hp['beta2']
                sched = opt.schedule(opt.steps_taken + n_steps, dev)
                a.adam_sched, a.adam_step = sched.data_ptr(), opt.steps_taken + 1
                opt.advance(n_steps)
            need = lib.slb_mf_step_workspace_bytes(a.batch, n_neg, a.loss, a.num_users, a.num_items)
            ws = ops.workspace('mf%d_%d' % (a.num_users, a.num_items), need, dev)
            a.workspace, a.workspace_bytes = ws.data_ptr(), ws.numel()
            n_steps = (n + B - 1) // B
            losses = torch.empty(n_steps, dtype=torch.float32, device=dev)
            w_steps = (ctypes.c_int64 * max(1, len(waits)))(*[int(k) for k, _ in waits])
            w_events = (ctypes.c_void_p * max(1, len(waits)))(*[ev.cuda_event for _, ev in waits])
            rc = lib.slb_mf_fit_epoch_events(ctypes.byref(a), ops._ptr(users), ops._ptr(items),
                                             ops._ptr(negatives), n, ops._ptr(losses), ops._stream(),
                                             w_steps, w_events, len(waits))
            _lib.check(rc, 'mf_fit_epoch')
            if not sync:
                return losses
            host = losses.cpu().numpy().astype(np.float64)
            if ops.workspace_error_flag(ws):
                raise ValueError('ids out of range reached the device kernels')
        return float(host.sum() / n_steps)

    def _fit_epoch_bloom_fused(self, users, items, negatives):
        net, opt = self._net, self._optimizer
        spec = net.fused_spec()
        n_neg = self._n_neg()
        hp = opt.fused_hparams()
        params = (spec['Wu'], spec['Wi'], net.user_biases.weight, net.item_biases.weight)
        states = [opt.fused_state(p) for p in params] if opt.fused_kind == _lib.OPT_ADAGRAD else None
        losses = []
        lo = 0
        for batch_user, batch_item in minibatch(users, items, batch_size=self._batch_size):
            B = batch_user.numel()
            batch_neg = negatives[lo * n_neg:(lo + B) * n_neg]
            lo += B
            losses.append(ops.mf_bloom_train_step_inplace(
                *params, batch_user, batch_item, batch_neg, self._loss, n_neg, spec['user_seeds'],
                spec['item_seeds'], spec['user_pad'], spec['item_pad'], opt.fused_kind, hp['lr'], states,
                hp['weight_decay'], hp['eps']))
        host = torch.stack(losses).cpu().numpy().astype(np.float64)
        return float(host.sum() / len(host))

    def _fit_epoch_autograd(self, users, items, negatives, fused):
        net = self._net
        n_neg = self._n_neg()
        epoch_loss = torch.zeros((), dtype=torch.float64, device=users.device)
        lo = 0
        minibatch_num = -1
        for minibatch_num, (batch_user, batch_item) in enumerate(
                minibatch(users, items, batch_size=self._batch_size)):
            B = batch_user.numel()
            batch_neg = negatives[lo * n_neg:(lo + B) * n_neg]
            lo += B
            self._optimizer.zero_grad()
            if fused == 'fused':
                loss = ops.fused_mf_loss(net.user_embeddings.weight, net.item_embeddings.weight,
                                         net.user_biases.weight, net.item_biases.weight,
                                         batch_user, batch_item, batch_neg, self._loss, n_neg)
            elif fused == 'bloom':
                spec = net.fused_spec()
                loss = ops.fused_bloom_loss(spec['Wu'], spec['Wi'], net.user_biases.weight,
                                            net.item_biases.weight, batch_user, batch_item, batch_neg,
                                            self._loss, n_neg, spec)
            else:
                positive_prediction = net(batch_user, batch_item)
                if self._loss == 'adaptive_hinge':
                    rep_users = batch_user.view(B, 1).expand(B, n_neg).reshape(B * n_neg)
                    negative_prediction = net(rep_users, batch_neg).view(n_neg, B)
                else:
                    negative_prediction = net(batch_user, batch_neg)
                loss = self._loss_func(positive_prediction, negative_prediction)
            epoch_loss += loss.detach().double()
            loss.backward()
            self._optimizer.step()
        return float(epoch_loss.item()) / (minibatch_num + 1)

    def _get_negative_prediction(self, user_ids):
        negative_items = sample_items(self._num_items, len(user_ids),
                                      random_state=self._random_state, device=user_ids.device)
        return self._net(user_ids, negative_items)

    def _get_multiple_negative_predictions(self, user_ids, n=5):
        batch_size = user_ids.size(0)
        negative_prediction = self._get_negative_prediction(
            user_ids.view(batch_size, 1).expand(batch_size, n).reshape(batch_size * n))
        return negative_prediction.view(n, len(user_ids))

    def predict(self, user_ids, item_ids=None):
        self._check_input(user_ids, item_ids, allow_items_none=True)
        self._net.train(False)
        user_ids, item_ids = _predict_process_ids(user_ids, item_ids, self._num_items,
                                                  self._use_cuda)
        with torch.no_grad():
            out = self._net(user_ids, item_ids)
        return cpu(out).detach().numpy().flatten()
```

Before: 1.551 billion.

## Restructure plan kernels: precomputed slots, fused scan, merged long/short sort

Reworks the batch planning pipeline. The count pass records per-interaction slots, so the fill pass no longer needs atomicSub on counters. A dedicated plan scan kernel builds a list of multi-entry segments, so the sort pass only visits segments with two or more entries, and the long-segment sort is folded into the same launch. It also adds workspace-capacity helpers, layout/plan-copy exports, profiling scripts, and drops the plan stream to normal priority. In exchange it uses more workspace for the slot and multi arrays and adds new kernel logic whose correctness depends on the slot bookkeeping.

```diff
diff --git a/include/spotlight_b200.h b/include/spotlight_b200.h
--- a/include/spotlight_b200.h
+++ b/include/spotlight_b200.h
@@ -145,6 +145,12 @@
 
 int slb_mf_train_step_phases(const slb_mf_step_args* args, int32_t phases, slb_stream_t stream);
 
+int32_t slb_mf_fused_layout(const slb_mf_step_args* args, int64_t* out, int32_t max_arrays);
+
+int slb_mf_plan_copy(const slb_mf_step_args* args, int32_t slot, int64_t batch, int32_t* totals,
+                     int32_t* seg_row, int32_t* seg_start, int32_t* sid, int32_t* long_list, void* mu,
+                     void* mi, slb_stream_t stream);
+
 typedef struct slb_mf_bloom_args {
     slb_mf_step_args base;
     int64_t user_rows, item_rows;
diff --git a/profiles/plan_kernels.py b/profiles/plan_kernels.py
--- /dev/null
+++ b/profiles/plan_kernels.py
@@ -0,0 +1,71 @@
+
+import argparse
+import ctypes
+import json
+import os
+import re
+import sys
+
+ROOT = os.path.dirname(os.path.dirname(os.path.abspath(__file__)))
+if ROOT not in sys.path:
+    sys.path.insert(0, ROOT)
+
+
+def main():
+    ap = argparse.ArgumentParser()
+    ap.add_argument('--iters', type=int, default=50)
+    ap.add_argument('--label', default='')
+    cli = ap.parse_args()
+
+    import torch
+    from torch.profiler import ProfilerActivity, profile
+    from spotlight_b200 import _lib, ops
+    sys.path.insert(0, os.path.join(ROOT, 'profiles'))
+    import plan_overlap
+
+    U, I, D, B = 1_000_000, 100_000, 64, 524288
+    dev = torch.device('cuda', 0)
+    torch.cuda.set_device(dev)
+    g = torch.Generator(device=dev).manual_seed(1234)
+    users, items, negs = (torch.randint(0, n, (B,), device=dev, generator=g) for n in (U, I, I))
+    Wu, Wi = torch.zeros((U, D), device=dev), torch.zeros((I, D), device=dev)
+    bu, bi = torch.zeros((U, 1), device=dev), torch.zeros((I, 1), device=dev)
+    lib = _lib.load()
+    a = ops.mf_step_args(Wu, Wi, bu, bi, users, items, negs, 'bpr', 1, batch=B)
+    a.grad_mode, a.opt, a.lr, a.eps = _lib.GRAD_COMPACT, _lib.OPT_ADAGRAD, 0.05, 1e-10
+    a.state_Wu, a.state_Wi, a.state_bu, a.state_bi = Wu.data_ptr(), Wi.data_ptr(), bu.data_ptr(), bi.data_ptr()
+    loss = torch.zeros(1, device=dev)
+    a.loss_out = loss.data_ptr()
+    fws = torch.zeros(lib.slb_mf_fused_workspace_bytes(B, U, I, D), dtype=torch.uint8, device=dev)
+    a.fused_workspace, a.fused_workspace_bytes = fws.data_ptr(), fws.numel()
+    ws = torch.zeros(lib.slb_mf_step_workspace_bytes(B, 1, a.loss, U, I), dtype=torch.uint8, device=dev)
+    a.workspace, a.workspace_bytes = ws.data_ptr(), ws.numel()
+    stream = ops._stream()
+    for _ in range(5):
+        _lib.check(lib.slb_mf_train_step_phases(ctypes.byref(a), 1, stream), 'plan')
+    torch.cuda.synchronize()
+    e0, e1 = torch.cuda.Event(enable_timing=True), torch.cuda.Event(enable_timing=True)
+    e0.record()
+    for _ in range(cli.iters):
+        _lib.check(lib.slb_mf_train_step_phases(ctypes.byref(a), 1, stream), 'plan')
+    e1.record()
+    torch.cuda.synchronize()
+    with profile(activities=[ProfilerActivity.CUDA]) as prof:
+        for _ in range(cli.iters):
+            _lib.check(lib.slb_mf_train_step_phases(ctypes.byref(a), 1, stream), 'plan')
+        torch.cuda.synchronize()
+    per = {}
+    for e in prof.events():
+        if e.device_type.name != 'CUDA':
+            continue
+        m = re.search(r'(\w+_kernel)', e.name)
+        name = m.group(1) if m else e.name
+        per[name] = per.get(name, 0.0) + e.device_time_total / cli.iters
+    print(json.dumps({'label': cli.label, 'card': plan_overlap.card(), 'batch': B, 'iters': cli.iters,
+                      'events_us_per_plan': e0.elapsed_time(e1) * 1e3 / cli.iters,
+                      'kernel_us_per_plan': {k: round(v, 2) for k, v in sorted(per.items(), key=lambda t: -t[1])},
+                      'kernel_sum_us': round(sum(per.values()), 2)}))
+
+
+if __name__ == '__main__':
+    main()
diff --git a/profiles/plan_overlap.py b/profiles/plan_overlap.py
--- /dev/null
+++ b/profiles/plan_overlap.py
@@ -0,0 +1,168 @@
+
+import argparse
+import ctypes
+import json
+import os
+import subprocess
+import sys
+
+import numpy as np
+
+ROOT = os.path.dirname(os.path.dirname(os.path.abspath(__file__)))
+if ROOT not in sys.path:
+    sys.path.insert(0, ROOT)
+
+
+def card():
+    try:
+        out = subprocess.run(['nvidia-smi', '--query-gpu=name,power.limit', '--format=csv,noheader'],
+                             capture_output=True, text=True, timeout=30).stdout.strip().splitlines()
+        return out[0] if out else None
+    except (OSError, subprocess.SubprocessError):
+        return None
+
+
+def floor_args(model, users, items, negs, a):
+    import torch
+    from spotlight_b200 import _lib, ops
+    lib = _lib.load()
+    net, opt = model._net, model._optimizer
+    dev = users.device
+    B = a.batch
+    params = [p.detach().clone() for p in (net.user_embeddings.weight, net.item_embeddings.weight,
+                                            net.user_biases.weight, net.item_biases.weight)]
+    states = [opt.fused_state(p).clone() for p in (net.user_embeddings.weight, net.item_embeddings.weight,
+                                                   net.user_biases.weight, net.item_biases.weight)]
+    Wu, Wi, bu, bi = params
+    st = ops.mf_step_args(Wu, Wi, bu, bi, users[:B], items[:B], negs[:B], a.loss, 1, batch=B)
+    st.grad_mode = _lib.GRAD_COMPACT
+    keep = [torch.empty(64, device=dev)] + params + states
+    need = lib.slb_mf_fused_workspace_bytes(B, a.users, a.items, a.dim)
+    assert need, 'the planned step is not available at this shape'
+    keep.append(ops.workspace('mfv2_%d_%d_%d' % (a.users, a.items, a.dim), need, dev))
+    st.fused_workspace, st.fused_workspace_bytes = keep[-1].data_ptr(), keep[-1].numel()
+    st.loss_out = keep[0].data_ptr()
+    hp = opt.fused_hparams()
+    st.opt, st.lr, st.weight_decay, st.eps = opt.fused_kind, hp['lr'], hp['weight_decay'], hp['eps']
+    st.state_Wu, st.state_Wi, st.state_bu, st.state_bi = [s.data_ptr() for s in states]
+    wneed = lib.slb_mf_step_workspace_bytes(B, 1, st.loss, a.users, a.items)
+    keep.append(ops.workspace('mf%d_%d' % (a.users, a.items), wneed, dev))
+    st.workspace, st.workspace_bytes = keep[-1].data_ptr(), keep[-1].numel()
+    return st, keep
+
+
+def main():
+    ap = argparse.ArgumentParser()
+    ap.add_argument('--rounds', type=int, default=3)
+    ap.add_argument('--steps', type=int, default=100)
+    ap.add_argument('--warmup', type=int, default=10)
+    ap.add_argument('--label', default='')
+    cli = ap.parse_args()
+
+    import torch
+    import bench
+    from spotlight_b200 import _lib, ops
+    from spotlight_b200 import rng as _rng
+    from spotlight_b200.factorization import implicit
+    from spotlight_b200.sampling import sample_items
+
+    a = argparse.Namespace(users=1_000_000, items=100_000, dim=64, batch=524288, loss='bpr', lr=0.05)
+    model = bench.build_model(a, 0)
+    dev = torch.device('cuda', 0)
+    B, K, W = a.batch, cli.steps, cli.warmup
+    g = torch.Generator(device=dev).manual_seed(1234)
+    n = (K + W) * B
+    users = torch.randint(0, a.users, (n,), device=dev, generator=g)
+    items = torch.randint(0, a.items, (n,), device=dev, generator=g)
+    model._run_epoch_device(users[:W * B], items[:W * B])
+    _prime = torch.empty(K * B, dtype=torch.int64, device=dev)
+    with torch.cuda.stream(implicit._side_stream(dev)):
+        _rng.reserve(a.items, min(64, K) * B, dev)
+    del _prime
+    tu, ti = users[W * B:], items[W * B:]
+
+    def timed(fn):
+        torch.cuda.synchronize()
+        e0, e1 = torch.cuda.Event(enable_timing=True), torch.cuda.Event(enable_timing=True)
+        e0.record()
+        fn()
+        e1.record()
+        torch.cuda.synchronize()
+        return e0.elapsed_time(e1) * 1e3 / K
+
+    plan_stream = implicit._plan_stream(dev)
+    other = torch.cuda.Stream(device=dev, priority=0 if plan_stream.priority < 0 else -1)
+
+    def epoch():
+        model._run_epoch_device(tu, ti)
+
+    def epoch_other_priority():
+        implicit._PLAN_STREAMS[dev.index] = other
+        try:
+            model._run_epoch_device(tu, ti)
+        finally:
+            implicit._PLAN_STREAMS[dev.index] = plan_stream
+
+    def epoch_same_stream():
+        os.environ['SLB_PLAN_SAME_STREAM'] = '1'
+        try:
+            model._run_epoch_device(tu, ti)
+        finally:
+            del os.environ['SLB_PLAN_SAME_STREAM']
+
+    lib = _lib.load()
+    negs = sample_items(a.items, K * B, random_state=np.random.RandomState(1), device=dev)
+    st, keep = floor_args(model, tu, ti, negs, a)
+    stream = ops._stream()
+
+    def floor():
+        _lib.check(lib.slb_mf_train_step_phases(ctypes.byref(st), 1, stream), 'plan')
+        torch.cuda.synchronize()
+        e0, e1 = torch.cuda.Event(enable_timing=True), torch.cuda.Event(enable_timing=True)
+        e0.record()
+        for _ in range(K):
+            _lib.check(lib.slb_mf_train_step_phases(ctypes.byref(st), 6, stream), 'float phases')
+        e1.record()
+        torch.cuda.synchronize()
+        return e0.elapsed_time(e1) * 1e3 / K
+
+    side = implicit._side_stream(dev)
+
+    def sampler():
+        rs = np.random.RandomState(3)
+        out = torch.empty(K * B, dtype=torch.int64, device=dev)
+        side.wait_stream(torch.cuda.current_stream(dev))
+        with torch.cuda.stream(side):
+            ds = _rng.DeviceStream(rs, dev)
+            e0, e1 = torch.cuda.Event(enable_timing=True), torch.cuda.Event(enable_timing=True)
+            e0.record(side)
+            lo, chunk = 0, 48 * B
+            while lo < K * B:
+                cur = min(chunk, K * B - lo)
+                ds.draw(a.items, cur, out=out[lo:lo + cur])
+                lo += cur
+            e1.record(side)
+            ds.finish()
+        torch.cuda.synchronize()
+        return e0.elapsed_time(e1) * 1e3 / K
+
+    rows = {k: [] for k in ('a', 'a_prio', 'b', 'c', 'sampler')}
+    for _ in range(cli.rounds):
+        rows['a'].append(timed(epoch))
+        rows['b'].append(timed(epoch_same_stream))
+        rows['a_prio'].append(timed(epoch_other_priority))
+        rows['c'].append(floor())
+        rows['sampler'].append(sampler())
+    med = {k: float(np.median(v)) for k, v in rows.items()}
+    line = {'label': cli.label, 'card': card(), 'steps': K, 'batch': B, 'rounds': cli.rounds,
+            'plan_stream_priority': plan_stream.priority, 'a_prio_priority': other.priority,
+            'us_per_step': med, 'runs': rows,
+            'exposed_plan_us': med['a'] - med['c'] - med['sampler'],
+            'exposed_plan_us_other_priority': med['a_prio'] - med['c'] - med['sampler'],
+            'serial_plan_us': med['b'] - med['c'] - med['sampler']}
+    del keep
+    print(json.dumps(line))
+
+
+if __name__ == '__main__':
+    main()
diff --git a/spotlight_b200/_lib.py b/spotlight_b200/_lib.py
--- a/spotlight_b200/_lib.py
+++ b/spotlight_b200/_lib.py
@@ -21,7 +21,7 @@
     'slb_embedding_forward', 'slb_bloom_rows',
     'slb_embedding_backward_workspace_bytes', 'slb_embedding_backward',
     'slb_mf_scores', 'slb_mf_scores_backward', 'slb_rank_pairs', 'slb_mf_step_workspace_bytes', 'slb_mf_fused_workspace_bytes', 'slb_mf_compact_rows',
-    'slb_mf_train_step', 'slb_mf_train_step_phases', 'slb_mf_fit_epoch', 'slb_mf_fit_epoch_events', 'slb_adam_flush',
+    'slb_mf_train_step', 'slb_mf_train_step_phases', 'slb_mf_plan_copy', 'slb_mf_fused_layout', 'slb_mf_fit_epoch', 'slb_mf_fit_epoch_events', 'slb_adam_flush',
     'slb_mf_bloom_workspace_bytes', 'slb_mf_bloom_train_step',
     'slb_bias_sparse_workspace_bytes', 'slb_bias_sparse_apply',
     'slb_unique_workspace_bytes', 'slb_unique_bucket', 'slb_shard_gather_batch', 'slb_adagrad_dense',
@@ -127,6 +127,9 @@
     lib.slb_mf_compact_rows.restype = c_i64
     lib.slb_mf_train_step.argtypes = [P(MfStepArgs), c_vp]
     lib.slb_mf_train_step_phases.argtypes = [P(MfStepArgs), c_i32, c_vp]
+    lib.slb_mf_fused_layout.argtypes = [P(MfStepArgs), c_vp, c_i32]
+    lib.slb_mf_fused_layout.restype = c_i32
+    lib.slb_mf_plan_copy.argtypes = [P(MfStepArgs), c_i32, c_i64, c_vp, c_vp, c_vp, c_vp, c_vp, c_vp, c_vp, c_vp]
     lib.slb_mf_bloom_workspace_bytes.argtypes = [P(MfBloomArgs)]
     lib.slb_mf_bloom_workspace_bytes.restype = c_sz
     lib.slb_mf_bloom_train_step.argtypes = [P(MfBloomArgs), c_vp]
diff --git a/spotlight_b200/csrc/common.cuh b/spotlight_b200/csrc/common.cuh
--- a/spotlight_b200/csrc/common.cuh
+++ b/spotlight_b200/csrc/common.cuh
@@ -31,11 +31,18 @@
 struct WsCarver {
     char* base;
     size_t off;
+    int64_t* log = nullptr;
+    int n_log = 0, max_log = 0;
     explicit WsCarver(void* p) : base(static_cast<char*>(p)), off(0) {}
     template <typename T>
     T* take(size_t count) {
         off = slb_align_up(off, 256);
         T* p = base ? reinterpret_cast<T*>(base + off) : nullptr;
+        if (log && n_log < max_log) {
+            log[2 * n_log] = static_cast<int64_t>(off);
+            log[2 * n_log + 1] = static_cast<int64_t>(off + count * sizeof(T));
+        }
+        if (log) ++n_log;
         off += count * sizeof(T);
         return p;
     }
diff --git a/spotlight_b200/csrc/mf.cu b/spotlight_b200/csrc/mf.cu
--- a/spotlight_b200/csrc/mf.cu
+++ b/spotlight_b200/csrc/mf.cu
@@ -1,4 +1,6 @@
 #include <stdlib.h>
+
+#include <algorithm>
 
 #include "segindex.cuh"
 
@@ -1118,8 +1120,9 @@
     size_t bytes;
 };
 
-V2Layout v2_layout(void* base, int64_t B, int64_t U, int64_t I, int D) {
-    WsCarver ws(base);
+V2Layout v2_layout(void* base, int64_t B, int64_t U, int64_t I, int D, WsCarver* log = nullptr) {
+    WsCarver own(base);
+    WsCarver& ws = log ? *log : own;
     V2Layout l;
     const int64_t R = U + I;
     const int64_t Rpad = (R + SEG_SCAN_TILE - 1) / SEG_SCAN_TILE * SEG_SCAN_TILE;
@@ -1149,6 +1152,9 @@
         p.mi_tmp = ws.take<IRec>(2 * B + 1);
         p.words = (2 * B + 31) / 32;
         p.bits = ws.take<uint32_t>(static_cast<size_t>(SEG_LONG_CTAS) * 2 * p.words);
+        p.slot = ws.take<int32_t>(3 * B);
+        p.multi = ws.take<int32_t>(3 * B / 2 + 1);
+        p.nmulti = ws.take<int32_t>(8);
         p.B = B; p.U = U; p.I = I;
         p.err = nullptr; p.users = nullptr; p.items = nullptr; p.negs = nullptr;
     }
@@ -1175,21 +1181,18 @@
                    const int64_t* negs, int64_t B, cudaStream_t st) {
     p.B = B; p.users = users; p.items = items; p.negs = negs; p.err = err;
     p.seg.long_cap = seg_sort_cap(lpr_for_dim(x->dim));
-    const int sms = slb_sms();
-    int g = static_cast<int>((B + 255) / 256);
-    if (g > sms * 8) g = sms * 8;
+    const int64_t cap = static_cast<int64_t>(slb_sms()) * PLAN_GRID_PER_SM;
+    const int g = static_cast<int>(std::min<int64_t>((B + 255) / 256, cap));
     plan_count_kernel<<<g, 256, 0, st>>>(p);
     SLB_LAUNCH_CHECK("plan_count_kernel");
-    seg_scan_launch(p.seg, p.U, st);
-    SLB_LAUNCH_CHECK("seg_scan_kernel");
+    plan_scan_kernel<<<static_cast<unsigned>(p.seg.ntiles), SEG_SCAN_THREADS, 0, st>>>(p);
+    SLB_LAUNCH_CHECK("plan_scan_kernel");
     plan_fill_kernel<<<g, 256, 0, st>>>(p);
     SLB_LAUNCH_CHECK("plan_fill_kernel");
-    int64_t tiles = ((3 * B + 31) / 32 + 3) / 4;
-    int sg = static_cast<int>(tiles < static_cast<int64_t>(sms) * 16 ? tiles : static_cast<int64_t>(sms) * 16);
-    plan_sort_kernel<<<sg, 128, 0, st>>>(p, p.seg.long_cap);
+    const int64_t tiles = ((3 * B / 2 + 1 + 31) / 32 + PLAN_SORT_THREADS / 32 - 1) / (PLAN_SORT_THREADS / 32);
+    const int sg = SEG_LONG_CTAS + static_cast<int>(std::min<int64_t>(tiles, 2 * cap));
+    plan_sort_kernel<<<sg, PLAN_SORT_THREADS, 0, st>>>(p, p.seg.long_cap);
     SLB_LAUNCH_CHECK("plan_sort_kernel");
-    plan_sort_long_kernel<<<SEG_LONG_CTAS, 256, 0, st>>>(p);
-    SLB_LAUNCH_CHECK("plan_sort_long_kernel");
     return SLB_OK;
 }
 
@@ -1285,6 +1288,21 @@
     return SLB_OK;
 }
 
+int64_t v2_capacity(size_t bytes, int64_t U, int64_t I, int D) {
+    int64_t lo = 0, hi = static_cast<int64_t>(bytes / (4 * static_cast<size_t>(D))) + 1;
+    while (hi - lo > 1) {
+        const int64_t mid = lo + (hi - lo) / 2;
+        if (v2_layout(nullptr, mid, U, I, D).bytes <= bytes) lo = mid;
+        else hi = mid;
+    }
+    return lo;
+}
+
+V2Layout v2_layout_ws(const slb_mf_step_args* x, void* base, WsCarver* log = nullptr) {
+    return v2_layout(base, v2_capacity(x->fused_workspace_bytes, x->num_users, x->num_items, x->dim),
+                     x->num_users, x->num_items, x->dim, log);
+}
+
 }
 
 extern "C" {
@@ -1311,7 +1329,7 @@
     if (v2_eligible(x)) {
         const int r2 = v2_check_ws(x);
         if (r2 != SLB_OK) return r2;
-        const V2Layout l = v2_layout(x->fused_workspace, x->batch, x->num_users, x->num_items, x->dim);
+        const V2Layout l = v2_layout_ws(x, x->fused_workspace);
         MfLayout old = mf_layout(x->workspace, x->batch, x->num_users, x->num_items);
         return v2_launch_step(x, l, 0, old.err, x->users, x->items, x->negs, x->batch, x->loss_out,
                               static_cast<cudaStream_t>(stream), 7);
@@ -1326,13 +1344,68 @@
     if (v2_eligible(x)) {
         const int r2 = v2_check_ws(x);
         if (r2 != SLB_OK) return r2;
-        const V2Layout l = v2_layout(x->fused_workspace, x->batch, x->num_users, x->num_items, x->dim);
+        const V2Layout l = v2_layout_ws(x, x->fused_workspace);
         MfLayout old = mf_layout(x->workspace, x->batch, x->num_users, x->num_items);
         return v2_launch_step(x, l, (phases >> 8) & 1, old.err, x->users, x->items, x->negs, x->batch, x->loss_out,
                               static_cast<cudaStream_t>(stream), phases & 7);
     }
     return launch_step(x, x->users, x->items, x->negs, x->batch, x->loss_out,
                        static_cast<cudaStream_t>(stream), phases);
+}
+
+int slb_mf_plan_copy(const slb_mf_step_args* x, int32_t slot, int64_t batch, int32_t* totals, int32_t* seg_row,
+                     int32_t* seg_start, int32_t* sid, int32_t* long_list, void* mu, void* mi, slb_stream_t stream) {
+    SLB_REQUIRE(x && x->fused_workspace && v2_dim_ok(x->dim), "mf_plan_copy: needs a planned-step workspace");
+    SLB_REQUIRE(slot == 0 || slot == 1, "mf_plan_copy: slot must be 0 or 1");
+    SLB_REQUIRE(batch > 0 && batch <= x->batch, "mf_plan_copy: batch must be in [1, args.batch]");
+    SLB_REQUIRE(totals && seg_row && seg_start && sid && long_list && mu && mi, "mf_plan_copy: null output");
+    const int r = v2_check_ws(x);
+    if (r != SLB_OK) return r;
+    const PlanDev& p = v2_layout_ws(x, x->fused_workspace).plan[slot];
+    cudaStream_t st = static_cast<cudaStream_t>(stream);
+    const auto copy = [&](void* dst, const void* src, size_t n) {
+        return cudaMemcpyAsync(dst, src, n, cudaMemcpyDeviceToDevice, st) == cudaSuccess;
+    };
+    const bool ok = copy(totals, p.seg.totals, 4 * sizeof(int32_t)) &&
+                    copy(seg_row, p.seg.seg_row, (3 * batch + 1) * sizeof(int32_t)) &&
+                    copy(seg_start, p.seg.seg_start, (3 * batch + 2) * sizeof(int32_t)) &&
+                    copy(sid, p.seg.sid, (x->num_users + x->num_items) * sizeof(int32_t)) &&
+                    copy(long_list, p.seg.long_list, (3 * batch / 16 + 2) * sizeof(int32_t)) &&
+                    copy(mu, p.mu, batch * sizeof(URec)) && copy(mi, p.mi, 2 * batch * sizeof(IRec));
+    if (!ok) { slb_set_error("mf_plan_copy: cudaMemcpyAsync failed"); return SLB_ECUDA; }
+    return SLB_OK;
+}
+
+int32_t slb_mf_fused_layout(const slb_mf_step_args* x, int64_t* out, int32_t max_arrays) {
+    SLB_REQUIRE(x && v2_dim_ok(x->dim) && x->batch > 0 && x->num_users > 0 && x->num_items > 0,
+                "mf_fused_layout: needs batch, num_users, num_items and a planned-step dim");
+    SLB_REQUIRE(out || max_arrays == 0, "mf_fused_layout: null output");
+    const int r = v2_check_ws(x);
+    if (r != SLB_OK) return r;
+    char* const base = reinterpret_cast<char*>(static_cast<uintptr_t>(1) << 40);
+    int64_t log[2 * 64];
+    WsCarver ws(base);
+    ws.log = log;
+    ws.max_log = 64;
+    const V2Layout l = v2_layout_ws(x, base, &ws);
+    SLB_REQUIRE(ws.n_log <= 64, "mf_fused_layout: more arrays than expected");
+    const auto at = [&](const void* q) { return static_cast<int64_t>(static_cast<const char*>(q) - base); };
+    for (int n = 0; n < ws.n_log && n < max_arrays; ++n) {
+        int64_t group = -1;
+        for (int k = 0; k < 2; ++k) {
+            const PlanDev& p = l.plan[k];
+            const void* mine[] = {p.seg.cnt, p.seg.off, p.seg.sid, p.seg.status, p.seg.ticket, p.seg.seg_row,
+                                  p.seg.seg_start, p.seg.long_list, p.mu, p.mi, p.mu_tmp, p.mi_tmp, p.bits,
+                                  p.slot, p.multi, p.nmulti};
+            for (const void* q : mine) if (at(q) == log[2 * n]) group = k;
+        }
+        const void* step[] = {l.st.done, l.st.t_g, l.st.stash, l.st.partial, l.st.partial_long};
+        for (const void* q : step) if (at(q) == log[2 * n]) group = 2;
+        out[3 * n] = group;
+        out[3 * n + 1] = log[2 * n];
+        out[3 * n + 2] = log[2 * n + 1];
+    }
+    return ws.n_log;
 }
 
 static int fit_epoch_impl(const slb_mf_step_args* x, const int64_t* users, const int64_t* items,
@@ -1349,7 +1422,7 @@
     if (v2_eligible(&tmp)) {
         const int r2 = v2_check_ws(&tmp);
         if (r2 != SLB_OK) return r2;
-        const V2Layout l = v2_layout(x->fused_workspace, x->batch, x->num_users, x->num_items, x->dim);
+        const V2Layout l = v2_layout_ws(x, x->fused_workspace);
         MfLayout old = mf_layout(x->workspace, x->batch, x->num_users, x->num_items);
         cudaStream_t plan_st = x->plan_stream ? static_cast<cudaStream_t>(x->plan_stream) : main_st;
         const bool two = plan_st != main_st;
diff --git a/spotlight_b200/csrc/mf_v2.cuh b/spotlight_b200/csrc/mf_v2.cuh
--- a/spotlight_b200/csrc/mf_v2.cuh
+++ b/spotlight_b200/csrc/mf_v2.cuh
@@ -11,6 +11,9 @@
     IRec* mi_tmp;
     uint32_t* bits;
     int64_t words;
+    int32_t* slot;
+    int32_t* multi;
+    int32_t* nmulti;
     int32_t* err;
     int64_t B, U, I;
     const int64_t* users; const int64_t* items; const int64_t* negs;
@@ -25,15 +28,140 @@
 };
 
 
+#ifndef PLAN_GRID_PER_SM
+#define PLAN_GRID_PER_SM 4
+#endif
+
+__device__ __forceinline__ bool plan_ids_ok(const PlanDev& p, int64_t u, int64_t i, int64_t j) {
+    return u >= 0 && u < p.U && i >= 0 && i < p.I && j >= 0 && j < p.I;
+}
+
 __global__ void __launch_bounds__(256) plan_count_kernel(PlanDev p) {
+    const int64_t tid = static_cast<int64_t>(blockIdx.x) * blockDim.x + threadIdx.x;
     const int64_t nth = static_cast<int64_t>(gridDim.x) * blockDim.x;
-    if (blockIdx.x == 0 && threadIdx.x == 0) p.seg.totals[3] = 0;
-    for (int64_t b = static_cast<int64_t>(blockIdx.x) * blockDim.x + threadIdx.x; b < p.B; b += nth) {
+    for (int64_t t = tid; t < p.seg.ntiles; t += nth) p.seg.status[t] = 0ull;
+    if (tid == 0) { *p.seg.ticket = 0; p.seg.totals[3] = 0; *p.nmulti = 0; }
+    for (int64_t b = tid; b < p.B; b += nth) {
         const int64_t u = p.users[b], i = p.items[b], j = p.negs[b];
-        if (u < 0 || u >= p.U || i < 0 || i >= p.I || j < 0 || j >= p.I) { atomicExch(p.err, 1); continue; }
-        atomicAdd(p.seg.cnt + u, 1);
-        atomicAdd(p.seg.cnt + p.U + i, 1);
-        atomicAdd(p.seg.cnt + p.U + j, 1);
+        if (!plan_ids_ok(p, u, i, j)) { atomicExch(p.err, 1); continue; }
+        const int su = atomicAdd(p.seg.cnt + u, 1);
+        const int si = atomicAdd(p.seg.cnt + p.U + i, 1);
+        const int sj = atomicAdd(p.seg.cnt + p.U + j, 1);
+        p.slot[b] = su;
+        p.slot[p.B + b] = si;
+        p.slot[2 * p.B + b] = sj;
+    }
+}
+
+constexpr int PLAN_SCAN_WARPS = SEG_SCAN_THREADS / 32;
+constexpr int PLAN_SCAN_ITEMS = SEG_SCAN_TILE / SEG_SCAN_THREADS;
+
+__global__ void __launch_bounds__(SEG_SCAN_THREADS) plan_scan_kernel(PlanDev p) {
+    __shared__ uint32_t sh_w[3][PLAN_SCAN_WARPS];
+    __shared__ uint32_t sh_pre[3];
+    __shared__ int sh_tile;
+    const SegIndex& s = p.seg;
+    const int lane = threadIdx.x & 31, warp = threadIdx.x >> 5;
+    const int cap = s.long_cap;
+    if (threadIdx.x == 0) sh_tile = atomicAdd(s.ticket, 1);
+    __syncthreads();
+    const int tile = sh_tile;
+    const int64_t base = static_cast<int64_t>(tile) * SEG_SCAN_TILE + warp * (32 * PLAN_SCAN_ITEMS) + lane;
+
+    int32_t c[PLAN_SCAN_ITEMS];
+#pragma unroll
+    for (int k = 0; k < PLAN_SCAN_ITEMS; ++k) c[k] = s.cnt[base + 32 * k];
+    uint32_t tsum = 0, tnz = 0, tmul = 0;
+#pragma unroll
+    for (int k = 0; k < PLAN_SCAN_ITEMS; ++k) {
+        tsum += c[k]; tnz += c[k] != 0; tmul += c[k] >= 2 && c[k] <= cap;
+        if (c[k] != 0) s.cnt[base + 32 * k] = 0;
+    }
+#pragma unroll
+    for (int o = 16; o > 0; o >>= 1) {
+        tsum += __shfl_xor_sync(0xffffffffu, tsum, o);
+        tnz += __shfl_xor_sync(0xffffffffu, tnz, o);
+        tmul += __shfl_xor_sync(0xffffffffu, tmul, o);
+    }
+    if (lane == 0) { sh_w[0][warp] = tsum; sh_w[1][warp] = tnz; sh_w[2][warp] = tmul; }
+    __syncthreads();
+    if (warp == 0) {
+        uint32_t v[3];
+#pragma unroll
+        for (int q = 0; q < 3; ++q) v[q] = lane < PLAN_SCAN_WARPS ? sh_w[q][lane] : 0u;
+        uint32_t inc[3] = {v[0], v[1], v[2]};
+#pragma unroll
+        for (int o = 1; o < PLAN_SCAN_WARPS; o <<= 1)
+#pragma unroll
+            for (int q = 0; q < 3; ++q) {
+                const uint32_t t = __shfl_up_sync(0xffffffffu, inc[q], o);
+                if (lane >= o) inc[q] += t;
+            }
+        uint32_t agg[3];
+#pragma unroll
+        for (int q = 0; q < 3; ++q) agg[q] = __shfl_sync(0xffffffffu, inc[q], PLAN_SCAN_WARPS - 1);
+        if (lane < PLAN_SCAN_WARPS)
+#pragma unroll
+            for (int q = 0; q < 3; ++q) sh_w[q][lane] = inc[q] - v[q];
+        volatile unsigned long long* st = s.status;
+        if (lane == 0) st[tile] = seg_pack(tile == 0 ? SEG_FLAG_INC : SEG_FLAG_AGG, agg[0], agg[1]);
+        unsigned long long pre = 0;
+        for (int hi = tile - 1; hi >= 0; hi -= 32) {
+            const int j = hi - lane;
+            unsigned long long w = seg_pack(SEG_FLAG_INC, 0u, 0u);
+            if (j >= 0) do { w = st[j]; } while (seg_flag(w) == 0);
+            const unsigned incm = __ballot_sync(0xffffffffu, seg_flag(w) == SEG_FLAG_INC);
+            const int last = incm ? __ffs(incm) - 1 : 31;
+            unsigned long long mine = lane <= last ? (static_cast<unsigned long long>(seg_nz(w)) << 32) | seg_sum(w) : 0ull;
+#pragma unroll
+            for (int o = 16; o > 0; o >>= 1) mine += __shfl_xor_sync(0xffffffffu, mine, o);
+            pre += mine;
+            if (incm) break;
+        }
+        if (lane == 0) {
+            const uint32_t psum = static_cast<uint32_t>(pre & 0xffffffffull), pnz = static_cast<uint32_t>(pre >> 32);
+            if (tile > 0) st[tile] = seg_pack(SEG_FLAG_INC, psum + agg[0], pnz + agg[1]);
+            sh_pre[0] = psum;
+            sh_pre[1] = pnz;
+            sh_pre[2] = agg[2] ? static_cast<uint32_t>(atomicAdd(p.nmulti, static_cast<int>(agg[2]))) : 0u;
+        }
+    }
+    __syncthreads();
+    uint32_t run = sh_pre[0] + sh_w[0][warp], seg = sh_pre[1] + sh_w[1][warp], mpos = sh_pre[2] + sh_w[2][warp];
+    const unsigned below = (1u << lane) - 1u;
+    const int64_t RA = p.U;
+#pragma unroll
+    for (int k = 0; k < PLAN_SCAN_ITEMS; ++k) {
+        const int64_t row = base + 32 * k;
+        uint32_t inc = c[k];
+#pragma unroll
+        for (int o = 1; o < 32; o <<= 1) {
+            const uint32_t t = __shfl_up_sync(0xffffffffu, inc, o);
+            if (lane >= o) inc += t;
+        }
+        const bool mul = c[k] >= 2 && c[k] <= cap;
+        const unsigned nzm = __ballot_sync(0xffffffffu, c[k] != 0);
+        const unsigned mm = __ballot_sync(0xffffffffu, mul);
+        const uint32_t my_seg = seg + __popc(nzm & below);
+        if (row == RA) s.totals[2] = static_cast<int32_t>(my_seg);
+        if (c[k] != 0) {
+            const uint32_t my_run = run + inc - c[k];
+            s.off[row] = static_cast<int32_t>(my_run);
+            s.sid[row] = static_cast<int32_t>(my_seg);
+            s.seg_row[my_seg] = static_cast<int32_t>(row);
+            s.seg_start[my_seg] = static_cast<int32_t>(my_run);
+            if (cap > 0 && c[k] > cap) s.long_list[atomicAdd(s.totals + 3, 1)] = static_cast<int32_t>(my_seg);
+            if (mul) p.multi[mpos + __popc(mm & below)] = static_cast<int32_t>(my_seg);
+        }
+        run += __shfl_sync(0xffffffffu, inc, 31);
+        seg += __popc(nzm);
+        mpos += __popc(mm);
+    }
+    if (tile == s.ntiles - 1 && threadIdx.x == SEG_SCAN_THREADS - 1) {
+        s.totals[0] = static_cast<int32_t>(seg);
+        s.totals[1] = static_cast<int32_t>(run);
+        s.seg_start[seg] = static_cast<int32_t>(run);
+        if (RA >= s.Rpad) s.totals[2] = static_cast<int32_t>(seg);
     }
 }
 
@@ -42,14 +170,14 @@
     const int ubase = p.seg.seg_start[p.seg.totals[2]];
     for (int64_t b = static_cast<int64_t>(blockIdx.x) * blockDim.x + threadIdx.x; b < p.B; b += nth) {
         const int64_t u = p.users[b], i = p.items[b], j = p.negs[b];
-        if (u < 0 || u >= p.U || i < 0 || i >= p.I || j < 0 || j >= p.I) continue;
-        const int su = p.seg.off[u] + atomicSub(p.seg.cnt + u, 1) - 1;
+        if (!plan_ids_ok(p, u, i, j)) continue;
+        const int su = p.seg.off[u] + p.slot[b];
+        const int useg = p.seg.sid[u];
+        const int si = p.seg.off[p.U + i] + p.slot[p.B + b] - ubase;
+        const int sj = p.seg.off[p.U + j] + p.slot[2 * p.B + b] - ubase;
         URec r;
         r.b = static_cast<int32_t>(b); r.i = static_cast<int32_t>(i); r.j = static_cast<int32_t>(j); r.pad = 0;
         p.mu[su] = r;
-        const int useg = p.seg.sid[u];
-        const int si = p.seg.off[p.U + i] + atomicSub(p.seg.cnt + p.U + i, 1) - 1 - ubase;
-        const int sj = p.seg.off[p.U + j] + atomicSub(p.seg.cnt + p.U + j, 1) - 1 - ubase;
         IRec a; a.t = static_cast<int32_t>(2 * b); a.useg = useg;
         IRec c; c.t = static_cast<int32_t>(2 * b + 1); c.useg = useg;
         p.mi[si] = a;
@@ -127,27 +255,13 @@
     }
 }
 
-__global__ void __launch_bounds__(128) plan_sort_kernel(PlanDev p, int cap) {
-    const int nseg = p.seg.totals[0], nsegA = p.seg.totals[2];
-    const int ubase = p.seg.seg_start[nsegA];
-    const int lane = threadIdx.x & 31;
-    const int ntiles = (nseg + 31) / 32;
-    for (int tile = blockIdx.x * 4 + (threadIdx.x >> 5); tile < ntiles; tile += gridDim.x * 4) {
-        const int s = tile * 32 + lane;
-        int start = 0, len = 0;
-        if (s < nseg) { start = p.seg.seg_start[s]; len = p.seg.seg_start[s + 1] - start; }
-        plan_sort_tile<URec>(p.mu, start, (s < nsegA) ? len : 0, cap, p.mu_tmp);
-        plan_sort_tile<IRec>(p.mi, start - ubase, (s >= nsegA && s < nseg) ? len : 0, cap, p.mi_tmp);
-    }
-}
-
-template <typename Rec>
+template <int NT, typename Rec>
 __device__ void plan_sort_long_one(Rec* base, Rec* tmp, int start, int len, uint32_t* bits, uint32_t* pre,
                                    int W, uint32_t* sh_scan) {
-    const int per = (W + 255) / 256;
-    for (int w = threadIdx.x; w < W; w += 256) bits[w] = 0u;
-    __syncthreads();
-    for (int i = threadIdx.x; i < len; i += 256) {
+    const int per = (W + NT - 1) / NT;
+    for (int w = threadIdx.x; w < W; w += NT) bits[w] = 0u;
+    __syncthreads();
+    for (int i = threadIdx.x; i < len; i += NT) {
         const int t = rec_key(base[start + i]);
         atomicOr(bits + (t >> 5), 1u << (t & 31));
     }
@@ -157,7 +271,7 @@
     for (int w = lo; w < hi; ++w) sum += __popc(bits[w]);
     sh_scan[threadIdx.x] = sum;
     __syncthreads();
-    for (int o = 1; o < 256; o <<= 1) {
+    for (int o = 1; o < NT; o <<= 1) {
         const uint32_t v = threadIdx.x >= o ? sh_scan[threadIdx.x - o] : 0u;
         __syncthreads();
         sh_scan[threadIdx.x] += v;
@@ -166,30 +280,51 @@
     uint32_t run = sh_scan[threadIdx.x] - sum;
     for (int w = lo; w < hi; ++w) { pre[w] = run; run += __popc(bits[w]); }
     __syncthreads();
-    for (int i = threadIdx.x; i < len; i += 256) {
+    for (int i = threadIdx.x; i < len; i += NT) {
         const Rec x = base[start + i];
         const int t = rec_key(x);
         const uint32_t r = pre[t >> 5] + __popc(bits[t >> 5] & ((1u << (t & 31)) - 1u));
         tmp[start + r] = x;
     }
     __syncthreads();
-    for (int i = threadIdx.x; i < len; i += 256) base[start + i] = tmp[start + i];
-    __syncthreads();
-}
-
-__global__ void __launch_bounds__(256) plan_sort_long_kernel(PlanDev p) {
-    __shared__ uint32_t sh_scan[256];
-    const int nlong = p.seg.totals[3];
+    for (int i = threadIdx.x; i < len; i += NT) base[start + i] = tmp[start + i];
+    __syncthreads();
+}
+
+constexpr int PLAN_SORT_THREADS = 128;
+
+__global__ void __launch_bounds__(PLAN_SORT_THREADS) plan_sort_kernel(PlanDev p, int cap) {
+    __shared__ uint32_t sh_scan[PLAN_SORT_THREADS];
     const int nsegA = p.seg.totals[2];
     const int ubase = p.seg.seg_start[nsegA];
-    uint32_t* bits = p.bits + static_cast<size_t>(blockIdx.x) * 2 * p.words;
-    uint32_t* pre = bits + p.words;
-    for (int li = blockIdx.x; li < nlong; li += gridDim.x) {
-        const int s = p.seg.long_list[li];
-        const int start = p.seg.seg_start[s];
-        const int len = p.seg.seg_start[s + 1] - start;
-        if (s < nsegA) plan_sort_long_one<URec>(p.mu, p.mu_tmp, start, len, bits, pre, static_cast<int>((p.B + 31) / 32), sh_scan);
-        else plan_sort_long_one<IRec>(p.mi, p.mi_tmp, start - ubase, len, bits, pre, static_cast<int>((2 * p.B + 31) / 32), sh_scan);
+    if (blockIdx.x < SEG_LONG_CTAS) {
+        const int nlong = p.seg.totals[3];
+        uint32_t* bits = p.bits + static_cast<size_t>(blockIdx.x) * 2 * p.words;
+        uint32_t* pre = bits + p.words;
+        for (int li = blockIdx.x; li < nlong; li += SEG_LONG_CTAS) {
+            const int s = p.seg.long_list[li];
+            const int start = p.seg.seg_start[s];
+            const int len = p.seg.seg_start[s + 1] - start;
+            if (s < nsegA)
+                plan_sort_long_one<PLAN_SORT_THREADS, URec>(p.mu, p.mu_tmp, start, len, bits, pre,
+                                                            static_cast<int>((p.B + 31) / 32), sh_scan);
+            else
+                plan_sort_long_one<PLAN_SORT_THREADS, IRec>(p.mi, p.mi_tmp, start - ubase, len, bits, pre,
+                                                            static_cast<int>((2 * p.B + 31) / 32), sh_scan);
+        }
+        return;
+    }
+    constexpr int WARPS = PLAN_SORT_THREADS / 32;
+    const int nmul = *p.nmulti;
+    const int lane = threadIdx.x & 31;
+    const int ntiles = (nmul + 31) / 32;
+    const int wstride = (gridDim.x - SEG_LONG_CTAS) * WARPS;
+    for (int tile = (blockIdx.x - SEG_LONG_CTAS) * WARPS + (threadIdx.x >> 5); tile < ntiles; tile += wstride) {
+        const int k = tile * 32 + lane;
+        int s = -1, start = 0, len = 0;
+        if (k < nmul) { s = p.multi[k]; start = p.seg.seg_start[s]; len = p.seg.seg_start[s + 1] - start; }
+        plan_sort_tile<URec>(p.mu, start, (s >= 0 && s < nsegA) ? len : 0, cap, p.mu_tmp);
+        plan_sort_tile<IRec>(p.mi, start - ubase, s >= nsegA ? len : 0, cap, p.mi_tmp);
     }
 }
 
diff --git a/spotlight_b200/factorization/implicit.py b/spotlight_b200/factorization/implicit.py
--- a/spotlight_b200/factorization/implicit.py
+++ b/spotlight_b200/factorization/implicit.py
@@ -32,7 +32,7 @@
 def _plan_stream(device):
     key = torch.device(device).index
     if key not in _PLAN_STREAMS:
-        _PLAN_STREAMS[key] = torch.cuda.Stream(device=device, priority=-1)
+        _PLAN_STREAMS[key] = torch.cuda.Stream(device=device, priority=0)
     return _PLAN_STREAMS[key]
 
 
```

Result: faster. 1.603 billion, median of 6 (+3.4%).
